# fxslava/tiny_mp2v_dec

Measured on AMD Instinct MI355X. Metric: decoded frames/sec + GB/s vs HBM roofline, 1080p 4:2:0 @1/2/4/8 GPU; bit-exact YUV, higher is better.
Workload: dtype u8

## Files before the change

include/mp2vg.h:

```cpp
#ifndef MP2VG_H
#define MP2VG_H

#include <stddef.h>
#include <stdint.h>

#ifdef __cplusplus
extern "C" {
#endif

#define MP2VG_ABI_VERSION 2

enum {
    MP2VG_OK = 0,
    MP2VG_E_INVALID = -1,
    MP2VG_E_UNSUPPORTED = -2,
    MP2VG_E_HIP = -3,
    MP2VG_E_NOMEM = -4,
    MP2VG_E_STATE = -5,
    MP2VG_E_BITSTREAM = -6
};

enum {
    MP2VG_MB_INTRA = 1u << 0,
    MP2VG_MB_FWD = 1u << 1,
    MP2VG_MB_BWD = 1u << 2,
    MP2VG_MB_FIELD_MC = 1u << 3,
    MP2VG_MB_DCT_FIELD = 1u << 4
};
#define MP2VG_MB_FS_BIT(r, s) (1u << (8 + 2 * (r) + (s)))

typedef struct mp2vg_mb {
    uint16_t x, y;
    uint16_t flags;
    uint16_t cbp;
    uint8_t  qscale;
    uint8_t  reserved;
    uint16_t ncoef;
    uint32_t coef_off;
    int16_t  mv[2][2][2];
} mp2vg_mb_t;

#define MP2VG_COEF_LEVEL(w) ((int16_t)((w) & 0xffffu))
#define MP2VG_COEF_POS(w) (((w) >> 16) & 63u)
#define MP2VG_COEF_BLOCK(w) (((w) >> 22) & 15u)
#define MP2VG_COEF_FIRST1S (1u << 29)
#define MP2VG_COEF_DC (1u << 30)
#define MP2VG_COEF_MBX(x) (((uint32_t)(x) & 7u) << 26)
#define MP2VG_COEF_PACK(level, pos, block, fl) \
    ((uint32_t)(uint16_t)(int16_t)(level) | ((uint32_t)(pos) << 16) | ((uint32_t)(block) << 22) | (uint32_t)(fl))

typedef struct mp2vg_picture {
    int32_t  dst_slot;
    int32_t  fwd_slot;
    int32_t  bwd_slot;
    int32_t  picture_coding_type;
    uint32_t mb_first;
    uint16_t mb_width, mb_height;
    uint8_t  alternate_scan;
    uint8_t  reserved0[3];
    int32_t  temporal_reference;
    uint8_t  W[4][64];
} mp2vg_picture_t;

typedef struct mp2vg_config {
    int32_t width, height;
    int32_t chroma_format;
    int32_t pictures_pool_size;
    int32_t num_threads;
    int32_t reordering;
    int32_t device;
    int32_t reserved;
} mp2vg_config_t;

#define MP2VG_DECODER_DEVICE_FRAMES 1
#define MP2VG_CTX_ONE_STREAM 2
#define MP2VG_DECODER_DEVICE_PARSE 4

typedef struct mp2vg_ctx mp2vg_ctx_t;

int  mp2vg_abi_version(void);
const char* mp2vg_status_string(int status);
const char* mp2vg_last_error(void);

int  mp2vg_create(const mp2vg_config_t* cfg, mp2vg_ctx_t** out);
int  mp2vg_destroy(mp2vg_ctx_t* ctx);
int  mp2vg_frame_geometry(const mp2vg_config_t* cfg, int32_t width[3], int32_t height[3],
                          int32_t stride[3], uint64_t* slot_bytes);
int  mp2vg_reserve_slots(mp2vg_ctx_t* ctx, int32_t nslots);

int  mp2vg_batch_upload(mp2vg_ctx_t* ctx, const mp2vg_picture_t* pics, int32_t npics,
                        const mp2vg_mb_t* mbs, uint64_t nmbs, const uint32_t* coefs,
                        uint64_t ncoefs);
int  mp2vg_batch_validate(const mp2vg_config_t* cfg, int32_t nslots, const mp2vg_picture_t* pics,
                          int32_t npics, const mp2vg_mb_t* mbs, uint64_t nmbs,
                          const uint32_t* coefs, uint64_t ncoefs, int32_t* nlaunches,
                          int32_t* launch_of_pic, int32_t* launch_mode, int32_t max_launches);
typedef struct mp2vg_plan {
    uint32_t* slices;
    int32_t*  launches;
    int32_t*  writes;
    int32_t*  ext_reads;
    int32_t*  post;
    int32_t*  foot;
    int32_t   max_slices, max_launches, max_writes, max_ext_reads, max_post, max_foot;
    int32_t   nslices, nlaunches, nwrites, next_reads, npost, nfoot;
    int32_t   nsets;
    int32_t   reserved;
} mp2vg_plan_t;
int  mp2vg_batch_plan(const mp2vg_config_t* cfg, int32_t nslots, const mp2vg_picture_t* pics,
                      int32_t npics, const mp2vg_mb_t* mbs, uint64_t nmbs,
                      const uint32_t* coefs, uint64_t ncoefs, mp2vg_plan_t* plan);
int  mp2vg_batch_decode(mp2vg_ctx_t* ctx);
int  mp2vg_synchronize(mp2vg_ctx_t* ctx);
int  mp2vg_last_launch_times(mp2vg_ctx_t* ctx, float* ms, int32_t max, int32_t* count);
int  mp2vg_last_batch_time(mp2vg_ctx_t* ctx, float* ms);
int  mp2vg_batch_times(mp2vg_ctx_t* ctx, int32_t back, float* batch_ms, float* launch_ms, int32_t max,
                       int32_t* count);
int  mp2vg_batches_span(mp2vg_ctx_t* ctx, int32_t back_first, int32_t back_last, float* ms);
int  mp2vg_download_slot(mp2vg_ctx_t* ctx, int32_t slot, uint8_t* dst_planes[3],
                         const int32_t dst_stride[3]);
int  mp2vg_copy_slot_packed(mp2vg_ctx_t* ctx, int32_t slot, void* dst, int32_t dst_on_device);
int  mp2vg_slot_device_ptr(mp2vg_ctx_t* ctx, int32_t slot, void** dptr);
int  mp2vg_invalidate_slot(mp2vg_ctx_t* ctx, int32_t slot);
int  mp2vg_pool_placement(mp2vg_ctx_t* ctx, float* ms, int32_t max, int32_t* n, int32_t* kept);
int  mp2vg_sink_device_ptr(mp2vg_ctx_t* ctx, void** dptr);
int  mp2vg_clock_probe(int32_t device, double* ghz);
int  mp2vg_cpu_budget(void);
int  mp2vg_pool_probe(mp2vg_ctx_t* ctx, int32_t rw, int32_t reps, double* gbps, int32_t max, int32_t* nblocks);
int  mp2vg_slot_digests(mp2vg_ctx_t* ctx, const int32_t* slots, int32_t n, uint64_t* out);

enum { MP2VG_EXPORT_RGB_PLANAR = 0 , MP2VG_EXPORT_RGB_PACKED = 1  };
enum { MP2VG_EXPORT_CHROMA_NEAREST = 0, MP2VG_EXPORT_CHROMA_LINEAR = 1 };
typedef struct mp2vg_export {
    int32_t layout, matrix, chroma;
    int32_t width, height;
    int32_t reserved[3];
} mp2vg_export_t;

int  mp2vg_export_coefficients(int32_t matrix, int32_t out[5]);
int  mp2vg_export_bytes(const mp2vg_config_t* cfg, const mp2vg_export_t* exp, int32_t n, uint64_t* bytes);
int  mp2vg_export_slots(mp2vg_ctx_t* ctx, const int32_t* slots, int32_t n, const mp2vg_export_t* exp,
                        void* dst_device, uint64_t dst_bytes);
int  mp2vg_export_planes(int32_t device, const uint8_t* const planes[3], const int32_t stride[3],
                         int32_t chroma_format, int32_t coded_w, int32_t coded_h, const mp2vg_export_t* exp,
                         void* dst_device, uint64_t dst_bytes);

enum { MP2VG_TENSOR_U8 = 0, MP2VG_TENSOR_F16 = 1, MP2VG_TENSOR_BF16 = 2, MP2VG_TENSOR_F32 = 3 };
enum { MP2VG_FIELD_PROGRESSIVE = 0, MP2VG_FIELD_TOP = 1, MP2VG_FIELD_BOTTOM = 2, MP2VG_FIELD_WEAVE = 3 };
#define MP2VG_TENSOR_MAX_TAPS 65
typedef struct mp2vg_tensor {
    int32_t layout, matrix, chroma;
    int32_t src_x, src_y, src_w, src_h;
    int32_t out_w, out_h;
    int32_t dtype;
    float   scale[3], bias[3];
    int32_t reserved[4];
} mp2vg_tensor_t;

int  mp2vg_tensor_weights(int32_t src, int32_t out, int32_t* first, int32_t* count, int32_t* weights,
                          int32_t max_taps);
int  mp2vg_tensor_bytes(const mp2vg_config_t* cfg, const mp2vg_tensor_t* t, int32_t n, uint64_t* bytes);
int  mp2vg_tensor_slots(mp2vg_ctx_t* ctx, const int32_t* slots, int32_t n, const mp2vg_tensor_t* t,
                        void* dst_device, uint64_t dst_bytes);
int  mp2vg_tensor_planes(int32_t device, const uint8_t* const planes[3], const int32_t stride[3],
                         int32_t chroma_format, int32_t coded_w, int32_t coded_h, const mp2vg_tensor_t* t,
                         void* dst_device, uint64_t dst_bytes);
int  mp2vg_tensor_slots_fields(mp2vg_ctx_t* ctx, const int32_t* slots, const int32_t* fields, int32_t n,
                               const mp2vg_tensor_t* t, void* dst_device, uint64_t dst_bytes);
int  mp2vg_tensor_planes_field(int32_t device, const uint8_t* const planes[3], const int32_t stride[3],
                               int32_t chroma_format, int32_t coded_w, int32_t coded_h, int32_t field,
                               const mp2vg_tensor_t* t, void* dst_device, uint64_t dst_bytes);

typedef struct mp2vg_sequence_header {
    uint32_t sequence_header_code, horizontal_size_value, vertical_size_value, aspect_ratio_information,
             frame_rate_code, bit_rate_value, vbv_buffer_size_value, constrained_parameters_flag,
             load_intra_quantiser_matrix;
    uint8_t  intra_quantiser_matrix[64];
    uint32_t load_non_intra_quantiser_matrix;
    uint8_t  non_intra_quantiser_matrix[64];
} mp2vg_sequence_header_t;
typedef struct mp2vg_sequence_extension {
    uint32_t extension_start_code, extension_start_code_identifier, profile_and_level_indication,
             progressive_sequence, chroma_format, horizontal_size_extension, vertical_size_extension,
             bit_rate_extension, vbv_buffer_size_extension, low_delay, frame_rate_extension_n,
             frame_rate_extension_d;
} mp2vg_sequence_extension_t;
typedef struct mp2vg_sequence_display_extension {
    uint32_t extension_start_code_identifier, video_format, colour_description, colour_primaries,
             transfer_characteristics, matrix_coefficients, display_horizontal_size, display_vertical_size;
} mp2vg_sequence_display_extension_t;
typedef struct mp2vg_sequence_scalable_extension {
    uint32_t extension_start_code_identifier, scalable_mode, layer_id, lower_layer_prediction_horizontal_size,
             lower_layer_prediction_vertical_size, horizontal_subsampling_factor_m,
             horizontal_subsampling_factor_n, vertical_subsampling_factor_m, vertical_subsampling_factor_n,
             picture_mux_enable, mux_to_progressive_sequence, picture_mux_order, picture_mux_factor;
} mp2vg_sequence_scalable_extension_t;
typedef struct mp2vg_group_of_pictures_header {
    uint32_t group_start_code, time_code, closed_gop, broken_link;
} mp2vg_group_of_pictures_header_t;
typedef struct mp2vg_stream_headers {
    int32_t have_sequence_display_extension;
    int32_t have_group_of_pictures_header;
    mp2vg_sequence_header_t sequence_header;
    mp2vg_sequence_extension_t sequence_extension;
    mp2vg_sequence_display_extension_t sequence_display_extension;
    mp2vg_group_of_pictures_header_t group_of_pictures_header;
} mp2vg_stream_headers_t;

int  mp2vg_export_matrix(const mp2vg_stream_headers_t* headers, int32_t* matrix);

typedef struct mp2vg_parsed mp2vg_parsed_t;

int  mp2vg_parse_es(const uint8_t* buf, uint64_t len, const mp2vg_config_t* cfg,
                    mp2vg_parsed_t** out);
int  mp2vg_parsed_counts(const mp2vg_parsed_t* p, int32_t* npics, uint64_t* nmbs,
                         uint64_t* ncoefs);
const mp2vg_picture_t* mp2vg_parsed_pictures(const mp2vg_parsed_t* p);
const mp2vg_mb_t*      mp2vg_parsed_mbs(const mp2vg_parsed_t* p);
const uint32_t*        mp2vg_parsed_coefs(const mp2vg_parsed_t* p);
int  mp2vg_parsed_display_order(const mp2vg_parsed_t* p, int32_t* order, int32_t n);
int  mp2vg_parsed_gop_index(const mp2vg_parsed_t* p, int32_t* gop, int32_t n);
enum { MP2VG_PIC_PROGRESSIVE_FRAME = 1, MP2VG_PIC_TOP_FIELD_FIRST = 2, MP2VG_PIC_REPEAT_FIRST_FIELD = 4 };
int  mp2vg_parsed_picture_flags(const mp2vg_parsed_t* p, uint32_t* flags, int32_t n);
int  mp2vg_parsed_stream_headers(const mp2vg_parsed_t* p, mp2vg_stream_headers_t* out);
int  mp2vg_parsed_shards(const mp2vg_parsed_t* p, int32_t* shard, int32_t n);
void mp2vg_parsed_free(mp2vg_parsed_t* p);

typedef struct mp2vg_scan mp2vg_scan_t;
int  mp2vg_scan_es(const uint8_t* buf, uint64_t len, const mp2vg_config_t* cfg, mp2vg_scan_t** out);
int  mp2vg_scan_counts(const mp2vg_scan_t* s, int32_t* npics, uint64_t* nslices);
const mp2vg_picture_t* mp2vg_scan_pictures(const mp2vg_scan_t* s);
int  mp2vg_scan_display_order(const mp2vg_scan_t* s, int32_t* order, int32_t n);
int  mp2vg_scan_gop_index(const mp2vg_scan_t* s, int32_t* gop, int32_t n);
int  mp2vg_scan_picture_flags(const mp2vg_scan_t* s, uint32_t* flags, int32_t n);
int  mp2vg_scan_shards(const mp2vg_scan_t* s, int32_t* shard, int32_t n);
int  mp2vg_scan_stream_headers(const mp2vg_scan_t* s, mp2vg_stream_headers_t* out);
void mp2vg_scan_free(mp2vg_scan_t* s);
int  mp2vg_scan_parse_host(const mp2vg_scan_t* s, int32_t first, int32_t npics, mp2vg_mb_t* mbs, uint64_t nmbs,
                           uint32_t* coefs, uint64_t ncoefs, uint64_t* nmbs_out, uint64_t* ncoefs_out);
int  mp2vg_batch_upload_es(mp2vg_ctx_t* ctx, const mp2vg_scan_t* scan, const mp2vg_picture_t* pics,
                           int32_t first, int32_t npics);
int  mp2vg_batch_record_counts(mp2vg_ctx_t* ctx, uint64_t* nmbs, uint64_t* ncoefs);
int  mp2vg_batch_download_records(mp2vg_ctx_t* ctx, mp2vg_mb_t* mbs, uint64_t nmbs, uint32_t* coefs,
                                  uint64_t ncoefs);
int  mp2vg_last_parse_times(mp2vg_ctx_t* ctx, float ms[3]);

enum {
    MP2VG_VLC_MBA = 0, MP2VG_VLC_MBTYPE_I = 1, MP2VG_VLC_MBTYPE_P = 2, MP2VG_VLC_MBTYPE_B = 3,
    MP2VG_VLC_CBP = 4, MP2VG_VLC_MOTION = 5, MP2VG_VLC_DC_LUMA = 6, MP2VG_VLC_DC_CHROMA = 7,
    MP2VG_VLC_COEF_B14 = 8, MP2VG_VLC_COEF_B15 = 9
};
int  mp2vg_vlc_decode(int32_t table, uint64_t bits, int32_t* value, int32_t* aux, int32_t* consumed);

typedef struct mp2vg_gen_params {
    int32_t width, height, chroma_format;
    int32_t n_gops;
    int32_t gop_n, gop_m;
    uint32_t seed;
    int32_t frame_pred_frame_dct;
    int32_t alternate_scan;
    int32_t q_scale_type;
    int32_t intra_dc_precision;
    int32_t coefs_min, coefs_max;
    int32_t intra_coefs_min, intra_coefs_max;
    int32_t big_level_permille;
    int32_t escape_permille;
    int32_t quant_permille;
    int32_t f_code;
    int32_t mix;
    int32_t leading_b;
    int32_t big_matrix_permille;
    int32_t top_field_first;
    int32_t reserved[4];
} mp2vg_gen_params_t;

void mp2vg_gen_default_params(mp2vg_gen_params_t* p);
int  mp2vg_generate_es(const mp2vg_gen_params_t* p, uint8_t** out, uint64_t* len);
void mp2vg_free(void* ptr);

typedef struct mp2vg_frame {
    uint8_t* planes[3];
    int32_t  width[3], height[3], stride[3];
    int32_t  picture_coding_type;
    int32_t  decode_index;
    int32_t  device;
} mp2vg_frame_t;
typedef void (*mp2vg_render_fn)(void* user, const mp2vg_frame_t* frame);
typedef struct mp2vg_decoder mp2vg_decoder_t;

int  mp2vg_decoder_create(const mp2vg_config_t* cfg, mp2vg_render_fn fn, void* user,
                          mp2vg_decoder_t** out);
int  mp2vg_decoder_create_multi(const mp2vg_config_t* cfg, const int32_t* devices, int32_t ndevices,
                                mp2vg_render_fn fn, void* user, mp2vg_decoder_t** out);
int  mp2vg_decoder_decode(mp2vg_decoder_t* dec, const uint8_t* buf, uint64_t len);
int  mp2vg_decoder_stream_headers(const mp2vg_decoder_t* dec, mp2vg_stream_headers_t* out);
int  mp2vg_decoder_lane_frames(const mp2vg_decoder_t* dec, int32_t* frames, int32_t n);
int  mp2vg_decoder_frames_allocated(const mp2vg_decoder_t* dec);
int  mp2vg_decoder_handoff_stats(const mp2vg_decoder_t* dec, int32_t* in_flight, int32_t* blocks, int32_t* landed,
                                 int32_t* changes);
int  mp2vg_decoder_destroy(mp2vg_decoder_t* dec);

#ifdef __cplusplus
}
#endif
#endif
```

tiny_mp2v_dec_amd/_lib.py:

```python
import ctypes
import os

import numpy as np

PKG = os.path.dirname(os.path.abspath(__file__))
LIB_PATH = os.environ.get("MP2VG_LIB") or os.path.join(PKG, "_build", "libmp2vg.so")

MB_DTYPE = np.dtype([("x", "<u2"), ("y", "<u2"), ("flags", "<u2"), ("cbp", "<u2"), ("qscale", "u1"),
                     ("reserved", "u1"), ("ncoef", "<u2"), ("coef_off", "<u4"), ("mv", "<i2", (2, 2, 2))])
assert MB_DTYPE.itemsize == 32
PIC_DTYPE = np.dtype([("dst_slot", "<i4"), ("fwd_slot", "<i4"), ("bwd_slot", "<i4"),
                      ("picture_coding_type", "<i4"), ("mb_first", "<u4"), ("mb_width", "<u2"),
                      ("mb_height", "<u2"), ("alternate_scan", "u1"), ("reserved0", "u1", (3,)),
                      ("temporal_reference", "<i4"), ("W", "u1", (4, 64))])
assert PIC_DTYPE.itemsize == 288

MB_INTRA, MB_FWD, MB_BWD, MB_FIELD_MC, MB_DCT_FIELD = 1, 2, 4, 8, 16
COEF_FIRST1S, COEF_DC = 1 << 29, 1 << 30


def mb_fs_bit(r, s):
    return 1 << (8 + 2 * r + s)


def coef_pack(level, pos, block, flags=0, mbx=0):
    return (np.uint32(np.int64(level) & 0xFFFF) | np.uint32(pos << 16) | np.uint32(block << 22) |
            np.uint32(flags) | np.uint32((int(mbx) & 7) << 26))


STATUS = {0: "ok", -1: "invalid argument", -2: "unsupported stream", -3: "HIP error", -4: "out of memory",
          -5: "call out of order", -6: "bitstream error"}


class Mp2vgError(RuntimeError):
    def __init__(self, status, what, detail=""):
        self.status = status
        super().__init__(f"{what}: {STATUS.get(status, status)} ({detail})")


class Config(ctypes.Structure):
    _fields_ = [("width", ctypes.c_int32), ("height", ctypes.c_int32), ("chroma_format", ctypes.c_int32),
                ("pictures_pool_size", ctypes.c_int32), ("num_threads", ctypes.c_int32),
                ("reordering", ctypes.c_int32), ("device", ctypes.c_int32), ("reserved", ctypes.c_int32)]


class GenParams(ctypes.Structure):
    _fields_ = [(n, ctypes.c_int32) for n in (
        "width", "height", "chroma_format", "n_gops", "gop_n", "gop_m")] + [("seed", ctypes.c_uint32)] + [
        (n, ctypes.c_int32) for n in (
            "frame_pred_frame_dct", "alternate_scan", "q_scale_type", "intra_dc_precision", "coefs_min",
            "coefs_max", "intra_coefs_min", "intra_coefs_max", "big_level_permille", "escape_permille",
            "quant_permille", "f_code", "mix", "leading_b", "big_matrix_permille", "top_field_first")] + [
        ("reserved", ctypes.c_int32 * 4)]


class Frame(ctypes.Structure):
    _fields_ = [("planes", ctypes.POINTER(ctypes.c_uint8) * 3), ("width", ctypes.c_int32 * 3),
                ("height", ctypes.c_int32 * 3), ("stride", ctypes.c_int32 * 3),
                ("picture_coding_type", ctypes.c_int32), ("decode_index", ctypes.c_int32),
                ("device", ctypes.c_int32)]


class SequenceHeader(ctypes.Structure):
    _fields_ = [(n, ctypes.c_uint32) for n in (
        "sequence_header_code", "horizontal_size_value", "vertical_size_value", "aspect_ratio_information",
        "frame_rate_code", "bit_rate_value", "vbv_buffer_size_value", "constrained_parameters_flag",
        "load_intra_quantiser_matrix")] + [("intra_quantiser_matrix", ctypes.c_uint8 * 64),
                                           ("load_non_intra_quantiser_matrix", ctypes.c_uint32),
                                           ("non_intra_quantiser_matrix", ctypes.c_uint8 * 64)]


class SequenceExtension(ctypes.Structure):
    _fields_ = [(n, ctypes.c_uint32) for n in (
        "extension_start_code", "extension_start_code_identifier", "profile_and_level_indication",
        "progressive_sequence", "chroma_format", "horizontal_size_extension", "vertical_size_extension",
        "bit_rate_extension", "vbv_buffer_size_extension", "low_delay", "frame_rate_extension_n",
        "frame_rate_extension_d")]


class SequenceDisplayExtension(ctypes.Structure):
    _fields_ = [(n, ctypes.c_uint32) for n in (
        "extension_start_code_identifier", "video_format", "colour_description", "colour_primaries",
        "transfer_characteristics", "matrix_coefficients", "display_horizontal_size", "display_vertical_size")]


class GopHeader(ctypes.Structure):
    _fields_ = [(n, ctypes.c_uint32) for n in ("group_start_code", "time_code", "closed_gop", "broken_link")]


class StreamHeaders(ctypes.Structure):
    _fields_ = [("have_sequence_display_extension", ctypes.c_int32),
                ("have_group_of_pictures_header", ctypes.c_int32),
                ("sequence_header", SequenceHeader), ("sequence_extension", SequenceExtension),
                ("sequence_display_extension", SequenceDisplayExtension),
                ("group_of_pictures_header", GopHeader)]


class Export(ctypes.Structure):
    _fields_ = [("layout", ctypes.c_int32), ("matrix", ctypes.c_int32), ("chroma", ctypes.c_int32),
                ("width", ctypes.c_int32), ("height", ctypes.c_int32), ("reserved", ctypes.c_int32 * 3)]


class Plan(ctypes.Structure):
    _fields_ = [("slices", ctypes.POINTER(ctypes.c_uint32))] + [
        (n, ctypes.POINTER(ctypes.c_int32)) for n in ("launches", "writes", "ext_reads", "post", "foot")] + [
        (n, ctypes.c_int32) for n in (
            "max_slices", "max_launches", "max_writes", "max_ext_reads", "max_post", "max_foot",
            "nslices", "nlaunches", "nwrites", "next_reads", "npost", "nfoot", "nsets", "reserved")]


EXPORT_RGB_PLANAR, EXPORT_RGB_PACKED = 0, 1
EXPORT_CHROMA_NEAREST, EXPORT_CHROMA_LINEAR = 0, 1

class Tensor(ctypes.Structure):
    _fields_ = [("layout", ctypes.c_int32), ("matrix", ctypes.c_int32), ("chroma", ctypes.c_int32),
                ("src_x", ctypes.c_int32), ("src_y", ctypes.c_int32), ("src_w", ctypes.c_int32),
                ("src_h", ctypes.c_int32), ("out_w", ctypes.c_int32), ("out_h", ctypes.c_int32),
                ("dtype", ctypes.c_int32), ("scale", ctypes.c_float * 3), ("bias", ctypes.c_float * 3),
                ("reserved", ctypes.c_int32 * 4)]


TENSOR_U8, TENSOR_F16, TENSOR_BF16, TENSOR_F32 = 0, 1, 2, 3
TENSOR_MAX_TAPS = 65
FIELD_PROGRESSIVE, FIELD_TOP, FIELD_BOTTOM, FIELD_WEAVE = 0, 1, 2, 3
FIELDS = {"progressive": FIELD_PROGRESSIVE, "top": FIELD_TOP, "bottom": FIELD_BOTTOM, "weave": FIELD_WEAVE}
PIC_PROGRESSIVE_FRAME, PIC_TOP_FIELD_FIRST, PIC_REPEAT_FIRST_FIELD = 1, 2, 4
TENSOR_DTYPES = {"uint8": (TENSOR_U8, 1), "float16": (TENSOR_F16, 2), "bfloat16": (TENSOR_BF16, 2),
                 "float32": (TENSOR_F32, 4)}

RENDER_FN = ctypes.CFUNCTYPE(None, ctypes.c_void_p, ctypes.POINTER(Frame))

EXPORTS = [
    "mp2vg_abi_version", "mp2vg_status_string", "mp2vg_last_error", "mp2vg_create", "mp2vg_destroy",
    "mp2vg_frame_geometry", "mp2vg_reserve_slots", "mp2vg_batch_upload", "mp2vg_batch_validate", "mp2vg_batch_plan", "mp2vg_batch_decode",
    "mp2vg_synchronize", "mp2vg_last_launch_times", "mp2vg_last_batch_time", "mp2vg_batch_times", "mp2vg_batches_span", "mp2vg_download_slot", "mp2vg_copy_slot_packed", "mp2vg_slot_device_ptr", "mp2vg_sink_device_ptr", "mp2vg_clock_probe", "mp2vg_pool_probe", "mp2vg_pool_placement", "mp2vg_cpu_budget", "mp2vg_invalidate_slot",
    "mp2vg_slot_digests", "mp2vg_parse_es", "mp2vg_parsed_counts", "mp2vg_parsed_pictures", "mp2vg_parsed_mbs",
    "mp2vg_parsed_coefs", "mp2vg_parsed_display_order", "mp2vg_parsed_gop_index", "mp2vg_parsed_stream_headers",
    "mp2vg_parsed_shards", "mp2vg_parsed_free", "mp2vg_vlc_decode",
    "mp2vg_gen_default_params", "mp2vg_generate_es", "mp2vg_free", "mp2vg_decoder_create",
    "mp2vg_decoder_create_multi", "mp2vg_decoder_decode", "mp2vg_decoder_stream_headers",
    "mp2vg_decoder_lane_frames", "mp2vg_decoder_frames_allocated", "mp2vg_decoder_handoff_stats",
    "mp2vg_decoder_destroy",
    "mp2vg_export_coefficients", "mp2vg_export_matrix", "mp2vg_export_bytes", "mp2vg_export_slots",
    "mp2vg_export_planes",
    "mp2vg_tensor_weights", "mp2vg_tensor_bytes", "mp2vg_tensor_slots", "mp2vg_tensor_planes",
    "mp2vg_tensor_slots_fields", "mp2vg_tensor_planes_field", "mp2vg_parsed_picture_flags", "mp2vg_scan_picture_flags",
    "mp2vg_scan_es", "mp2vg_scan_counts", "mp2vg_scan_pictures", "mp2vg_scan_display_order",
    "mp2vg_scan_gop_index", "mp2vg_scan_shards", "mp2vg_scan_stream_headers", "mp2vg_scan_free",
    "mp2vg_scan_parse_host", "mp2vg_batch_upload_es", "mp2vg_batch_record_counts",
    "mp2vg_batch_download_records", "mp2vg_last_parse_times",
]

_lib = None


def lib():
    global _lib
    if _lib is not None:
        return _lib
    if not os.path.exists(LIB_PATH):
        raise RuntimeError(f"native library {LIB_PATH} is missing: run `python tiny_mp2v_dec_amd/build.py` "
                           "(there is no CPU fallback for the reconstruct path)")
    L = ctypes.CDLL(LIB_PATH)
    P, I32, U64, VP = ctypes.POINTER, ctypes.c_int32, ctypes.c_uint64, ctypes.c_void_p
    sig = {
        "mp2vg_abi_version": ([], ctypes.c_int),
        "mp2vg_status_string": ([ctypes.c_int], ctypes.c_char_p),
        "mp2vg_last_error": ([], ctypes.c_char_p),
        "mp2vg_create": ([P(Config), P(VP)], ctypes.c_int),
        "mp2vg_destroy": ([VP], ctypes.c_int),
        "mp2vg_frame_geometry": ([P(Config), P(I32), P(I32), P(I32), P(U64)], ctypes.c_int),
        "mp2vg_reserve_slots": ([VP, I32], ctypes.c_int),
        "mp2vg_batch_upload": ([VP, VP, I32, VP, U64, VP, U64], ctypes.c_int),
        "mp2vg_batch_validate": ([P(Config), I32, VP, I32, VP, U64, VP, U64, P(I32), P(I32), P(I32), I32],
                                 ctypes.c_int),
        "mp2vg_batch_plan": ([P(Config), I32, VP, I32, VP, U64, VP, U64, P(Plan)], ctypes.c_int),
        "mp2vg_batch_decode": ([VP], ctypes.c_int),
        "mp2vg_synchronize": ([VP], ctypes.c_int),
        "mp2vg_last_launch_times": ([VP, P(ctypes.c_float), I32, P(I32)], ctypes.c_int),
        "mp2vg_last_batch_time": ([VP, P(ctypes.c_float)], ctypes.c_int),
        "mp2vg_batch_times": ([VP, I32, P(ctypes.c_float), P(ctypes.c_float), I32, P(I32)], ctypes.c_int),
        "mp2vg_batches_span": ([VP, I32, I32, P(ctypes.c_float)], ctypes.c_int),
        "mp2vg_download_slot": ([VP, I32, P(ctypes.c_void_p), P(I32)], ctypes.c_int),
        "mp2vg_copy_slot_packed": ([VP, I32, VP, I32], ctypes.c_int),
        "mp2vg_slot_device_ptr": ([VP, I32, P(VP)], ctypes.c_int),
        "mp2vg_sink_device_ptr": ([VP, P(VP)], ctypes.c_int),
        "mp2vg_clock_probe": ([I32, P(ctypes.c_double)], ctypes.c_int),
        "mp2vg_pool_probe": ([VP, I32, I32, P(ctypes.c_double), I32, P(I32)], ctypes.c_int),
        "mp2vg_pool_placement": ([VP, P(ctypes.c_float), I32, P(I32), P(I32)], ctypes.c_int),
        "mp2vg_cpu_budget": ([], ctypes.c_int),
        "mp2vg_invalidate_slot": ([VP, I32], ctypes.c_int),
        "mp2vg_slot_digests": ([VP, P(I32), I32, P(ctypes.c_uint64)], ctypes.c_int),
        "mp2vg_parse_es": ([VP, U64, P(Config), P(VP)], ctypes.c_int),
        "mp2vg_parsed_counts": ([VP, P(I32), P(U64), P(U64)], ctypes.c_int),
        "mp2vg_parsed_pictures": ([VP], VP),
        "mp2vg_parsed_mbs": ([VP], VP),
        "mp2vg_parsed_coefs": ([VP], VP),
        "mp2vg_parsed_display_order": ([VP, P(I32), I32], ctypes.c_int),
        "mp2vg_parsed_gop_index": ([VP, P(I32), I32], ctypes.c_int),
        "mp2vg_parsed_stream_headers": ([VP, P(StreamHeaders)], ctypes.c_int),
        "mp2vg_parsed_shards": ([VP, P(I32), I32], ctypes.c_int),
        "mp2vg_parsed_free": ([VP], None),
        "mp2vg_vlc_decode": ([I32, U64, P(I32), P(I32), P(I32)], ctypes.c_int),
        "mp2vg_gen_default_params": ([P(GenParams)], None),
        "mp2vg_generate_es": ([P(GenParams), P(VP), P(U64)], ctypes.c_int),
        "mp2vg_free": ([VP], None),
        "mp2vg_decoder_create": ([P(Config), RENDER_FN, VP, P(VP)], ctypes.c_int),
        "mp2vg_decoder_create_multi": ([P(Config), P(I32), I32, RENDER_FN, VP, P(VP)], ctypes.c_int),
        "mp2vg_decoder_decode": ([VP, VP, U64], ctypes.c_int),
        "mp2vg_decoder_stream_headers": ([VP, P(StreamHeaders)], ctypes.c_int),
        "mp2vg_decoder_lane_frames": ([VP, P(I32), I32], ctypes.c_int),
        "mp2vg_decoder_frames_allocated": ([VP], ctypes.c_int),
        "mp2vg_decoder_handoff_stats": ([VP, P(I32), P(I32), P(I32), P(I32)], ctypes.c_int),
        "mp2vg_decoder_destroy": ([VP], ctypes.c_int),
        "mp2vg_export_coefficients": ([I32, P(I32)], ctypes.c_int),
        "mp2vg_export_matrix": ([P(StreamHeaders), P(I32)], ctypes.c_int),
        "mp2vg_export_bytes": ([P(Config), P(Export), I32, P(U64)], ctypes.c_int),
        "mp2vg_export_slots": ([VP, P(I32), I32, P(Export), VP, U64], ctypes.c_int),
        "mp2vg_export_planes": ([I32, P(VP), P(I32), I32, I32, I32, P(Export), VP, U64], ctypes.c_int),
        "mp2vg_tensor_weights": ([I32, I32, P(I32), P(I32), P(I32), I32], ctypes.c_int),
        "mp2vg_tensor_bytes": ([P(Config), P(Tensor), I32, P(U64)], ctypes.c_int),
        "mp2vg_tensor_slots": ([VP, P(I32), I32, P(Tensor), VP, U64], ctypes.c_int),
        "mp2vg_tensor_planes": ([I32, P(VP), P(I32), I32, I32, I32, P(Tensor), VP, U64], ctypes.c_int),
        "mp2vg_tensor_slots_fields": ([VP, P(I32), P(I32), I32, P(Tensor), VP, U64], ctypes.c_int),
        "mp2vg_tensor_planes_field": ([I32, P(VP), P(I32), I32, I32, I32, I32, P(Tensor), VP, U64], ctypes.c_int),
        "mp2vg_parsed_picture_flags": ([VP, P(ctypes.c_uint32), I32], ctypes.c_int),
        "mp2vg_scan_picture_flags": ([VP, P(ctypes.c_uint32), I32], ctypes.c_int),
        "mp2vg_scan_es": ([VP, U64, P(Config), P(VP)], ctypes.c_int),
        "mp2vg_scan_counts": ([VP, P(I32), P(U64)], ctypes.c_int),
        "mp2vg_scan_pictures": ([VP], VP),
        "mp2vg_scan_display_order": ([VP, P(I32), I32], ctypes.c_int),
        "mp2vg_scan_gop_index": ([VP, P(I32), I32], ctypes.c_int),
        "mp2vg_scan_shards": ([VP, P(I32), I32], ctypes.c_int),
        "mp2vg_scan_stream_headers": ([VP, P(StreamHeaders)], ctypes.c_int),
        "mp2vg_scan_free": ([VP], None),
        "mp2vg_scan_parse_host": ([VP, I32, I32, VP, U64, VP, U64, P(U64), P(U64)], ctypes.c_int),
        "mp2vg_batch_upload_es": ([VP, VP, VP, I32, I32], ctypes.c_int),
        "mp2vg_batch_record_counts": ([VP, P(U64), P(U64)], ctypes.c_int),
        "mp2vg_batch_download_records": ([VP, VP, U64, VP, U64], ctypes.c_int),
        "mp2vg_last_parse_times": ([VP, P(ctypes.c_float)], ctypes.c_int),
    }
    for name, (args, res) in sig.items():
        fn = getattr(L, name)
        fn.argtypes = args
        fn.restype = res
    _lib = L
    return L


def check(status, what):
    if status != 0:
        detail = lib().mp2vg_last_error().decode(errors="replace")
        raise Mp2vgError(status, what, detail)
    return status


MP2VG_DECODER_DEVICE_FRAMES, MP2VG_CTX_ONE_STREAM = 1, 2
MP2VG_DECODER_DEVICE_PARSE = 4


def make_config(width, height, chroma_format, pool=10, threads=0, reordering=True, device=0, flags=0):
    return Config(width, height, chroma_format, pool, threads, 1 if reordering else 0, device, flags)


def make_export(layout="nchw", chroma="linear", matrix=1, size=None):
    layouts = {"nchw": EXPORT_RGB_PLANAR, "nhwc": EXPORT_RGB_PACKED}
    modes = {"nearest": EXPORT_CHROMA_NEAREST, "linear": EXPORT_CHROMA_LINEAR}
    if layout not in layouts:
        raise ValueError(f"layout {layout!r}: expected 'nchw' or 'nhwc'")
    if chroma not in modes:
        raise ValueError(f"chroma {chroma!r}: expected 'linear' or 'nearest'")
    w, h = (0, 0) if size is None else (int(size[0]), int(size[1]))
    return Export(layouts[layout], int(matrix), modes[chroma], w, h, (ctypes.c_int32 * 3)())


def export_shape(exp, n, coded_w, coded_h):
    w, h = exp.width or coded_w, exp.height or coded_h
    return (n, 3, h, w) if exp.layout == EXPORT_RGB_PLANAR else (n, h, w, 3)


def export_out(out, shape, device):
    import torch
    dev = torch.device("cuda", device)
    if out is None:
        return torch.empty(shape, dtype=torch.uint8, device=dev)
    if not isinstance(out, torch.Tensor) or out.device != dev or out.dtype != torch.uint8:
        raise ValueError(f"out must be a torch.uint8 tensor on {dev}")
    if tuple(out.shape) != tuple(shape) or not out.is_contiguous():
        raise ValueError(f"out must be contiguous with shape {tuple(shape)}, got {tuple(out.shape)}")
    return out


def tensor_dtype_name(dtype):
    name = str(dtype).replace("torch.", "")
    if name not in TENSOR_DTYPES:
        raise ValueError(f"dtype {dtype!r}: expected uint8, float16, bfloat16 or float32")
    return name


def make_tensor(size, crop=None, dtype="float16", mean=None, std=None, layout="nchw", chroma="linear", matrix=1):
    e = make_export(layout, chroma, matrix)
    name = tensor_dtype_name(dtype)
    if (mean is None) != (std is None):
        raise ValueError("mean and std go together")
    if name == "uint8":
        if mean is not None:
            raise ValueError("uint8 output takes no mean / std")
        scale, bias = [1.0] * 3, [0.0] * 3
    elif mean is None:
        scale, bias = [1.0 / 255.0] * 3, [0.0] * 3
    else:
        mean, std = [float(v) for v in mean], [float(v) for v in std]
        if len(mean) != 3 or len(std) != 3:
            raise ValueError("mean and std have one entry per channel")
        scale, bias = [1.0 / (255.0 * s) for s in std], [-m / s for m, s in zip(mean, std)]
    x, y, w, h = (0, 0, 0, 0) if crop is None else (int(v) for v in crop)
    return Tensor(e.layout, e.matrix, e.chroma, x, y, w, h, int(size[0]), int(size[1]), TENSOR_DTYPES[name][0],
                  (ctypes.c_float * 3)(*scale), (ctypes.c_float * 3)(*bias), (ctypes.c_int32 * 4)())


def field_mode(field):
    if isinstance(field, str):
        if field not in FIELDS:
            raise ValueError(f"field {field!r}: expected 'progressive', 'top', 'bottom' or 'weave'")
        return FIELDS[field]
    if int(field) not in FIELDS.values():
        raise ValueError(f"field {field!r}: expected 0..3 (MP2VG_FIELD_*)")
    return int(field)


def field_modes(fields, n):
    if fields is None:
        return None
    if isinstance(fields, (str, int, np.integer)):
        return np.full(n, field_mode(fields), np.int32)
    out = np.array([field_mode(f) for f in fields], np.int32)
    if len(out) != n:
        raise ValueError("fields must hold one mode per slot")
    return out


def tensor_shape(t, n):
    return (n, 3, t.out_h, t.out_w) if t.layout == EXPORT_RGB_PLANAR else (n, t.out_h, t.out_w, 3)


def tensor_out(out, shape, dtype, device):
    import torch
    dev, want = torch.device("cuda", device), getattr(torch, tensor_dtype_name(dtype))
    if out is None:
        return torch.empty(shape, dtype=want, device=dev)
    if not isinstance(out, torch.Tensor) or out.device != dev or out.dtype != want:
        raise ValueError(f"out must be a {want} tensor on {dev}")
    if tuple(out.shape) != tuple(shape) or not out.is_contiguous():
        raise ValueError(f"out must be contiguous with shape {tuple(shape)}, got {tuple(out.shape)}")
    return out


def tensor_weights(src, out):
    first, count = np.zeros(out, np.int32), np.zeros(out, np.int32)
    w = np.zeros((out, TENSOR_MAX_TAPS), np.int32)
    i32p = ctypes.POINTER(ctypes.c_int32)
    check(lib().mp2vg_tensor_weights(src, out, first.ctypes.data_as(i32p), count.ctypes.data_as(i32p),
                                     w.ctypes.data_as(i32p), TENSOR_MAX_TAPS), "tensor_weights")
    return first, count, w[:, :int(count.max())]


def geometry(width, height, chroma_format):
    c = make_config(width, height, chroma_format)
    w, h, s = (ctypes.c_int32 * 3)(), (ctypes.c_int32 * 3)(), (ctypes.c_int32 * 3)()
    sb = ctypes.c_uint64()
    check(lib().mp2vg_frame_geometry(ctypes.byref(c), w, h, s, ctypes.byref(sb)), "frame_geometry")
    return list(w), list(h), list(s), sb.value
```

tiny_mp2v_dec_amd/csrc/recon.hip:

```cpp
#include <hip/hip_runtime.h>

#include <cstdlib>
#include <stdint.h>
#include <stdlib.h>

#include "recon_kernel.h"

namespace mp2vg {

typedef short short2_t __attribute__((ext_vector_type(2)));

__device__ __forceinline__ short2_t adds2(short2_t a, short2_t b) { return __builtin_elementwise_add_sat(a, b); }
__device__ __forceinline__ short2_t subs2(short2_t a, short2_t b) { return __builtin_elementwise_sub_sat(a, b); }
__device__ __forceinline__ short2_t shl2(short2_t a, int n) {
    return __builtin_bit_cast(short2_t, __builtin_bit_cast(ushort2, a) << (unsigned short)n);
}
__device__ __forceinline__ short2_t mulhi2(short2_t a, int c) {
    const uint32_t u = __builtin_bit_cast(uint32_t, a);
    const int lo = (int)(short)(u & 0xffffu) * c, hi = ((int)u >> 16) * c;
    return __builtin_bit_cast(short2_t, __builtin_amdgcn_perm((uint32_t)hi, (uint32_t)lo, 0x07060302u));
}
__device__ __forceinline__ short2_t mulhi2_x2(short2_t a, int c) {
    const short2_t h = mulhi2(a, 2 * c);
    return __builtin_bit_cast(short2_t, __builtin_bit_cast(uint32_t, h) & 0xfffefffeu);
}

template <bool P1 = false>
__device__ __forceinline__ void idct_1d(short2_t s[8]) {
    const short2_t v15 = adds2(mulhi2_x2(s[0], 27145), shl2(s[0], 1));
    const short2_t v26 = P1 ? mulhi2(s[1], -5037 + 262144) : adds2(mulhi2(s[1], -5037), shl2(s[1], 2));
    const short2_t v21 = P1 ? mulhi2(s[2], -19954 + 262144) : adds2(mulhi2(s[2], -19954), shl2(s[2], 2));
    const short2_t v28 = P1 ? mulhi2_x2(s[3], -22089 + 131072) : adds2(mulhi2_x2(s[3], -22089), shl2(s[3], 2));
    const short2_t v16 = P1 ? mulhi2_x2(s[4], 27145 + 65536) : adds2(mulhi2_x2(s[4], 27145), shl2(s[4], 1));
    const short2_t v25 = P1 ? mulhi2(s[5], 14567 + 131072) : adds2(mulhi2(s[5], 14567), shl2(s[5], 1));
    const short2_t v22 = adds2(mulhi2_x2(s[6], 17391), s[6]);
    const short2_t v27 = mulhi2_x2(s[7], 25570);
    const short2_t v19 = subs2(v25, v28);
    const short2_t v20 = subs2(v26, v27);
    const short2_t v23 = adds2(v26, v27);
    const short2_t v24 = adds2(v25, v28);
    const short2_t v7 = adds2(v23, v24);
    const short2_t v11 = adds2(v21, v22);
    const short2_t v13 = subs2(v23, v24);
    const short2_t v17 = subs2(v21, v22);
    const short2_t v8 = adds2(v15, v16);
    const short2_t v9 = subs2(v15, v16);
    const short2_t v18 = mulhi2(subs2(v19, v20), 25079);
    const short2_t v12 = subs2(v18, P1 ? mulhi2(v19, 20090 + 65536) : adds2(v19, mulhi2(v19, 20090)));
    const short2_t v14 = subs2(subs2(v20, mulhi2(v20, 30068)), v18);
    const short2_t v6 = subs2(shl2(v14, 1), v7);
    const short2_t v5 = subs2(P1 ? mulhi2(v13, 27145 + 65536) : adds2(v13, mulhi2(v13, 27145)), v6);
    const short2_t v4 = adds2(v5, shl2(v12, 1));
    const short2_t v10 = subs2(P1 ? mulhi2(v17, 27145 + 65536) : adds2(v17, mulhi2(v17, 27145)), v11);
    const short2_t v0 = adds2(v8, v11);
    const short2_t v1 = adds2(v9, v10);
    const short2_t v2 = subs2(v9, v10);
    const short2_t v3 = subs2(v8, v11);
    s[0] = adds2(v0, v7);
    s[1] = adds2(v1, v6);
    s[2] = adds2(v2, v5);
    s[3] = subs2(v3, v4);
    s[4] = adds2(v3, v4);
    s[5] = subs2(v2, v5);
    s[6] = subs2(v1, v6);
    s[7] = subs2(v0, v7);
}

__device__ __forceinline__ void interleave(const uint4& a, const uint4& b, short2_t s[8]) {
    const uint32_t av[4] = {a.x, a.y, a.z, a.w}, bv[4] = {b.x, b.y, b.z, b.w};
#pragma unroll
    for (int i = 0; i < 4; i++) {
        s[2 * i] = __builtin_bit_cast(short2_t, __builtin_amdgcn_perm(bv[i], av[i], 0x05040100u));
        s[2 * i + 1] = __builtin_bit_cast(short2_t, __builtin_amdgcn_perm(bv[i], av[i], 0x07060302u));
    }
}

__constant__ uint8_t c_scan_raster[2][64] = {
    {0,  1,  8,  16, 9,  2,  3,  10, 17, 24, 32, 25, 18, 11, 4,  5,  12, 19, 26, 33, 40, 48,
     41, 34, 27, 20, 13, 6,  7,  14, 21, 28, 35, 42, 49, 56, 57, 50, 43, 36, 29, 22, 15, 23,
     30, 37, 44, 51, 58, 59, 52, 45, 38, 31, 39, 46, 53, 60, 61, 54, 47, 55, 62, 63},
    {0,  8,  16, 24, 1,  9,  2,  10, 17, 25, 32, 40, 48, 56, 57, 49, 41, 33, 26, 18, 3,  11,
     4,  12, 19, 27, 34, 42, 50, 58, 35, 43, 51, 59, 20, 28, 5,  13, 6,  14, 21, 29, 36, 44,
     52, 60, 37, 45, 53, 61, 22, 30, 7,  15, 23, 31, 38, 46, 54, 62, 39, 47, 55, 63}};

__device__ __forceinline__ void wave_sync() {
    __builtin_amdgcn_fence(__ATOMIC_RELEASE, "wavefront");
    __builtin_amdgcn_wave_barrier();
    __builtin_amdgcn_fence(__ATOMIC_ACQUIRE, "wavefront");
}

__device__ __forceinline__ uint32_t sat_pk_u8(short2_t v) {
    uint32_t r;
    asm("v_sat_pk_u8_i16 %0, %1" : "=v"(r) : "v"(__builtin_bit_cast(uint32_t, v)));
    return r;
}

__device__ __forceinline__ uint32_t avg4(uint32_t a, uint32_t b) { return __builtin_amdgcn_lerp(a, b, 0x01010101u); }

__device__ __forceinline__ uint32_t mul24_asm(uint32_t a, uint32_t b) {
    uint32_t r;
    asm("v_mul_u32_u24 %0, %1, %2" : "=v"(r) : "v"(a), "v"(b));
    return r;
}

template <int CF>
struct Fmt {
    static constexpr int NB = CF == 1 ? 6 : (CF == 2 ? 8 : 12);
    static constexpr int CW = CF == 3 ? 16 : 8;
    static constexpr int CH = CF == 1 ? 8 : 16;
};

template <int CF>
__device__ __forceinline__ void block_origin(int b, bool dctf, int& plane, int& x0, int& y0, int& ys) {
    ys = 1;
    if (b < 4) {
        plane = 0;
        x0 = (b & 1) * 8;
        if (dctf) {
            y0 = b >> 1;
            ys = 2;
        } else {
            y0 = (b >> 1) * 8;
        }
        return;
    }
    plane = (b & 1) ? 2 : 1;
    const int k = (b - 4) >> 1;
    x0 = k >= 2 ? 8 : 0;
    const bool lower = (k & 1);
    if (dctf && CF != 1) {
        y0 = lower ? 1 : 0;
        ys = 2;
    } else {
        y0 = lower ? 8 : 0;
    }
}

template <int CF>
__device__ __forceinline__ int left_block(int plane, int py, bool dctf) {
    const int lower = dctf ? (py & 1) : (py >> 3);
    if (plane == 0) return lower * 2;
    const int base = plane == 1 ? 4 : 5;
    if (CF == 1) return base;
    return base + 2 * lower;
}


constexpr int WAVES = 4;
constexpr int G = 4;
#ifndef MP2VG_I_WAVES
#define MP2VG_I_WAVES 4
#endif
#ifndef MP2VG_I_KBTAB
#define MP2VG_I_KBTAB 1
#endif
template <int MCM, int ABL>
constexpr int kernel_waves() { return (MCM == 0 || MCM == 4) && ABL == 0 ? MP2VG_I_WAVES : WAVES; }

template <int CF>
struct ResLayout {
    using F = Fmt<CF>;
    static constexpr int SIZE = 256 + 2 * F::CW * F::CH;
#ifndef MP2VG_RES_PAD
#define MP2VG_RES_PAD 0
#endif
    static constexpr int MBS = SIZE + MP2VG_RES_PAD;
    __device__ static constexpr int base(int plane) { return plane == 0 ? 0 : 256 + (plane - 1) * F::CW * F::CH; }
    __device__ static constexpr int width(int plane) { return plane == 0 ? 16 : F::CW; }
    __device__ static int pos(int x) { return (x & ~3) | ((x & 1) << 1) | ((x >> 1) & 1); }
};

template <class T>
__device__ __forceinline__ T gsel(const T (&v)[3], int plane) {
    return plane == 0 ? v[0] : (plane == 1 ? v[1] : v[2]);
}

#ifndef MP2VG_REC_NT
#define MP2VG_REC_NT 0
#endif
__device__ __forceinline__ uint32_t ld_rec(const uint32_t* p) {
    if (MP2VG_REC_NT) return __builtin_nontemporal_load(p);
    return *p;
}
__device__ __forceinline__ uint32_t rec_load(const uint32_t* __restrict__ mbrec, uint32_t g, uint32_t mb_last, int lane) {
    const uint32_t mb = min(g + (uint32_t)(lane & 3), mb_last);
    return ld_rec(&mbrec[(size_t)mb * 8 + ((lane >> 2) & 7)]);
}
__device__ __forceinline__ uint32_t rec_get(uint32_t rv, int f, int k) {
    return (uint32_t)__builtin_amdgcn_ds_bpermute((f * 4 + k) * 4, (int)rv);
}
template <int F, int K>
__device__ __forceinline__ uint32_t rec_uni(uint32_t rv) {
    return (uint32_t)__builtin_amdgcn_readlane((int)rv, F * 4 + K);
}

struct Group {
    uint32_t fl8;
    uint32_t qs8;
    uint32_t sb8;
    uint32_t cbp01, cbp23;
    int nslots, ncoef;
    uint32_t coef0;
};

__device__ __forceinline__ uint32_t pick8(uint32_t v, int k) { return __builtin_amdgcn_ubfe(v, (uint32_t)k * 8, 8); }
__device__ __forceinline__ uint32_t pick16(uint32_t lo, uint32_t hi, int k) {
    return __builtin_amdgcn_ubfe((k & 2) ? hi : lo, (uint32_t)(k & 1) * 16, 16);
}

template <int NB, int K>
__device__ __forceinline__ void group_mb(Group& S, uint32_t rv, int ng, int& sb, int& cr) {
    const uint32_t r1 = rec_uni<1, K>(rv), r2 = rec_uni<2, K>(rv);
    const bool live = K < ng;
    const uint32_t cbpk = live ? ((r1 >> 16) & ((1u << NB) - 1)) : 0u;
    S.fl8 |= (live ? (r1 & 0xff) : (uint32_t)MP2VG_MB_INTRA) << (8 * K);
    S.qs8 |= (r2 & 0xff) << (8 * K);
    S.sb8 |= (uint32_t)sb << (8 * K);
    if (K == 0) S.cbp01 = cbpk;
    if (K == 1) S.cbp01 |= cbpk << 16;
    if (K == 2) S.cbp23 = cbpk;
    if (K == 3) S.cbp23 |= cbpk << 16;
    sb += __builtin_popcount(cbpk);
    cr += live ? (int)(r2 >> 16) : 0;
}

template <int NB>
__device__ __forceinline__ Group group_state(uint32_t rv, int ng) {
    Group S;
    S.fl8 = S.qs8 = S.sb8 = 0;
    int sb = 0, cr = 0;
    group_mb<NB, 0>(S, rv, ng, sb, cr);
    group_mb<NB, 1>(S, rv, ng, sb, cr);
    group_mb<NB, 2>(S, rv, ng, sb, cr);
    group_mb<NB, 3>(S, rv, ng, sb, cr);
    S.nslots = sb;
    S.ncoef = cr;
    S.coef0 = rec_uni<3, 0>(rv);
    return S;
}

template <int CF>
struct Passes {
    static constexpr int N = CF == 1 ? 2 : 3;
};
template <int CF, int J>
__device__ __forceinline__ void pass_row(int lane, int& k, int& plane, int& py) {
    k = lane & 3;
    py = lane >> 2;
    if (J == 0) {
        plane = 0;
    } else if (CF == 1) {
        plane = 1 + (lane >> 5);
        py = (lane & 31) >> 2;
    } else {
        plane = J;
    }
}

template <int W>
__device__ __forceinline__ uint32_t tile_off(uint32_t x, uint32_t y, uint32_t ncol) {
    if (W == 16) return (mul24_asm(y >> 2, ncol) + (x >> 4)) * 128u + (y & 3u) * 32u + (x & 12u);
    return (mul24_asm(y >> 3, ncol) + (x >> 3)) * 128u + (y & 7u) * 16u + (x & 4u);
}
template <int W>
__device__ __forceinline__ uint32_t tile_row(uint32_t mx, uint32_t y, uint32_t ncol) {
    if (W == 16) return (mul24_asm(y >> 2, ncol) + mx) * 128u + (y & 3u) * 32u;
    return (mul24_asm(y >> 3, ncol) + mx) * 128u + (y & 7u) * 16u;
}

template <int NW>
struct Tap {
    static constexpr int ND = NW + 1;
    uint32_t a[ND], b[ND];
    uint32_t ctl;
};

typedef uint32_t u3v __attribute__((ext_vector_type(3)));
typedef uint32_t u4v __attribute__((ext_vector_type(4)));
constexpr uint32_t kNoTap = 0xFFFFFF00u;
__device__ __forceinline__ __amdgpu_buffer_rsrc_t slot_rsrc(const uint8_t* base, uint32_t bytes) {
    return __builtin_amdgcn_make_buffer_rsrc((void*)base, (short)0, (int)bytes, 0x00020000);
}
template <int NW, int ABL = 0>
__device__ __forceinline__ void load_row(uint32_t (&d)[NW + 1], __amdgpu_buffer_rsrc_t r, uint32_t off) {
    if (NW == 4) {
        const u4v v = __builtin_amdgcn_raw_buffer_load_b128(r, (int)off, 0, 0);
        d[0] = v.x; d[1] = v.y; d[2] = v.z; d[3] = v.w;
        d[4] = __builtin_amdgcn_raw_buffer_load_b32(r, (ABL & 128) ? (int)kNoTap : (int)(off + 16), 0, 0);
    } else if (NW == 2) {
        const u3v v = __builtin_amdgcn_raw_buffer_load_b96(r, (int)off, 0, 0);
        d[0] = v.x; d[1] = v.y; d[2] = v.z;
    } else {
#pragma unroll
        for (int i = 0; i < NW + 1; i++) d[i] = __builtin_amdgcn_raw_buffer_load_b32(r, (int)(off + 4 * i), 0, 0);
    }
}

#ifndef MP2VG_CHROMA_TILES
#define MP2VG_CHROMA_TILES 1
#endif
constexpr bool kChromaTiles = MP2VG_CHROMA_TILES;

__device__ __forceinline__ uint32_t mad24s_asm(uint32_t a, uint32_t b_uniform, uint32_t c) {
    uint32_t r;
    asm("v_mad_u32_u24 %0, %1, %2, %3" : "=v"(r) : "v"(a), "s"(b_uniform), "v"(c));
    return r;
}

// ... 77 lines not shown
    for (int d = 0; d < NW; d++) {
        const uint32_t r0 = avg4(A[d], __builtin_amdgcn_alignbyte(A[d + 1], A[d], hx));
        const uint32_t r1 = avg4(C[d], __builtin_amdgcn_alignbyte(C[d + 1], C[d], hx));
        p[d] = avg4(r0, r1);
    }
}

template <int MCM, int NW, int ABL = 0>
__device__ __forceinline__ void predict(Tap<NW>& tf, Tap<NW>& tb, int lane, uint32_t (&p)[NW]) {
    if (ABL & 64) {
#pragma unroll
        for (int d = 0; d < NW; d++) p[d] = tf.a[d] ^ tf.b[d] ^ (MCM == 2 ? tb.a[d] ^ tb.b[d] : 0u);
        return;
    }
    if (!(MP2VG_ROW2_LOAD && MCM == 2)) {
        tap_rows<NW>(tf, lane);
        if (MCM == 2) tap_rows<NW>(tb, lane);
    }
    const bool uf = tf.ctl & 16, ub = MCM == 2 && (tb.ctl & 16);
    uint32_t pf[NW], pb[NW];
#pragma unroll
    for (int d = 0; d < NW; d++) pf[d] = pb[d] = 0;
    if (uf) tap_finish<NW>(tf, pf);
    if (MCM == 2 && ub) tap_finish<NW>(tb, pb);
#pragma unroll
    for (int d = 0; d < NW; d++) p[d] = (uf && ub) ? avg4(pf[d], pb[d]) : (uf ? pf[d] : pb[d]);
}

struct LaneRec {
    uint32_t r0, r1, mvf, mvb;
};
__device__ __forceinline__ LaneRec lane_rec(uint32_t rv, int lane) {
    LaneRec L;
    const int k = lane & 3;
    L.r0 = rec_get(rv, 0, k);
    L.r1 = rec_get(rv, 1, k);
    const int r = (L.r1 & MP2VG_MB_FIELD_MC) ? ((lane >> 2) & 1) : 0;
    L.mvf = rec_get(rv, 4 + 2 * r, k);
    L.mvb = rec_get(rv, 5 + 2 * r, k);
    return L;
}

template <int CF, int MCM, int J, int NW, int ABL = 0>
__device__ __forceinline__ void issue_pass(const LaneRec& L, bool live, int lane, const Geo& geo,
                                           __amdgpu_buffer_rsrc_t ref_fwd, __amdgpu_buffer_rsrc_t ref_bwd,
                                           Tap<NW>& tf, Tap<NW>& tb, int dir = 0) {
    using F = Fmt<CF>;
    int k, plane, py;
    pass_row<CF, J>(lane, k, plane, py);
    const uint32_t fl = L.r1 & 0xffff;
    const bool none = !live || (fl & MP2VG_MB_INTRA);
    const bool bwd = fl & MP2VG_MB_BWD;
    const bool fwd = !none && (MCM == 1 || (fl & MP2VG_MB_FWD) || !bwd);
    const bool field = fl & MP2VG_MB_FIELD_MC;
    const int pw = plane == 0 ? 16 : F::CW;
    const int phm = plane == 0 ? 16 : F::CH;
    const int gx = (int)(L.r0 & 0xffff) * pw;
    const int mbyb = (int)(L.r0 >> 16) * phm;
    const int r = field ? (py & 1) : 0;
    const int stride = J == 0 ? geo.stride[0] : geo.stride[1];
    const int ph = J == 0 ? geo.ph[0] : geo.ph[1];
    constexpr bool TL = J == 0 || kChromaTiles;
    const uint32_t off = (TL ? 2u : 1u) * (uint32_t)gsel(geo.plane_off, plane);
    const uint32_t mv1 = (MCM == 1 && dir) ? L.mvb : L.mvf;
    const int fsh = 8 + 2 * r + (MCM == 1 ? dir : 0);
    constexpr bool R2 = MP2VG_ROW2_LOAD && MCM == 2;
    tap_issue<CF, NW, ABL, TL, R2>(tf, fwd, ref_fwd, off, mv1, plane, gx, py, phm, mbyb, field, (fl >> fsh) & 1, stride, ph);
    if (MCM == 2)
        tap_issue<CF, NW, ABL, TL, R2>(tb, !none && bwd, ref_bwd, off, L.mvb, plane, gx, py, phm, mbyb, field,
                                       (fl >> (9 + 2 * r)) & 1, stride, ph);
}

__device__ __forceinline__ void row_store16(uint8_t* d, uint32_t a, uint32_t b, uint32_t c, uint32_t e) {
    *(uint4*)d = make_uint4(a, b, c, e);
}
__device__ __forceinline__ void row_store8(uint8_t* d, uint32_t a, uint32_t b) { *(uint2*)d = make_uint2(a, b); }

#ifndef MP2VG_ROW_POL
#define MP2VG_ROW_POL 16
#endif
#ifndef MP2VG_TILE_POL
#define MP2VG_TILE_POL 2
#endif
template <int POL>
__device__ __forceinline__ void pol_store16(__amdgpu_buffer_rsrc_t r, uint32_t off, uint4 v) {
    __builtin_amdgcn_raw_buffer_store_b128(u4v{v.x, v.y, v.z, v.w}, r, (int)off, 0, POL);
}
template <int POL>
__device__ __forceinline__ void pol_store8(__amdgpu_buffer_rsrc_t r, uint32_t off, uint2 v) {
    typedef uint32_t u2v __attribute__((ext_vector_type(2)));
    __builtin_amdgcn_raw_buffer_store_b64(u2v{v.x, v.y}, r, (int)off, 0, POL);
}


template <int CF, int J, int NW, int ABL>
__device__ __forceinline__ void store_pass(uint32_t r0, uint32_t r1, bool live, int lane, const Geo& geo, uint8_t* wsink,
                                           uint8_t* dst_slot, __amdgpu_buffer_rsrc_t dst_rsrc, bool tiles,
                                           const short* s_res_wave, const uint32_t (&p)[NW]) {
    using F = Fmt<CF>;
    using RL = ResLayout<CF>;
    int k, plane, py;
    pass_row<CF, J>(lane, k, plane, py);
    const uint32_t fl = r1 & 0xffff, cbpk = r1 >> 16;
    const int lb = left_block<CF>(plane, py, fl & MP2VG_MB_DCT_FIELD);
    const int rb = (plane == 0) ? lb + 1 : lb + 4;
    const bool cl = cbpk & (1u << lb);
    const bool cr = NW == 4 && (cbpk & (1u << rb));
    uint32_t out[4] = {0, 0, 0, 0};
#pragma unroll
    for (int d = 0; d < NW; d++) out[d] = p[d];
    if (cl || cr) {
        const short* res = s_res_wave + k * RL::MBS + RL::base(plane) + py * RL::width(plane);
        uint32_t rv[8];
        const uint4 q0 = *(const uint4*)&res[0];
        rv[0] = q0.x; rv[1] = q0.y; rv[2] = q0.z; rv[3] = q0.w;
        if (NW == 4) {
            const uint4 q1 = *(const uint4*)&res[8];
            rv[4] = q1.x; rv[5] = q1.y; rv[6] = q1.z; rv[7] = q1.w;
        }
#pragma unroll
        for (int d = 0; d < NW; d++) {
            if (!(d < 2 ? cl : cr)) continue;
            const uint32_t lo = __builtin_amdgcn_perm(0u, out[d], 0x0c020c00u);
            const uint32_t hi = __builtin_amdgcn_perm(0u, out[d], 0x0c030c01u);
            const short2_t a = __builtin_bit_cast(short2_t, lo) + __builtin_bit_cast(short2_t, rv[2 * d]);
            const short2_t c = __builtin_bit_cast(short2_t, hi) + __builtin_bit_cast(short2_t, rv[2 * d + 1]);
            out[d] = __builtin_amdgcn_perm(sat_pk_u8(c), sat_pk_u8(a), 0x05010400u);
        }
    }
    const int pw = plane == 0 ? 16 : F::CW;
    const int phm = plane == 0 ? 16 : F::CH;
    const uint32_t doff = gsel(geo.plane_off, plane) + mul24_asm((r0 >> 16) * phm + py, (uint32_t)gsel(geo.stride, plane)) +
                          (r0 & 0xffff) * (uint32_t)pw;
    uint8_t* dst = dst_slot + doff;
    dst = live ? dst : wsink;
    if (ABL & 8192)
        dst = dst_slot + ((((r0 & 0xffff) + (r0 >> 16) * 128u) * 3u + (uint32_t)J) * 1024u + (uint32_t)lane * 16u) %
                             (uint32_t)(geo.plane_off[1] - 1024);
    if (tiles) {
        uint8_t* img = (uint8_t*)(s_res_wave + k * RL::MBS + RL::base(plane) + py * RL::width(plane));
        if (NW == 4)
            *(uint4*)img = make_uint4(out[0], out[1], out[2], out[3]);
        else
            *(uint2*)img = make_uint2(out[0], out[1]);
    }
    if (ABL & 8) {
        asm volatile("" ::"v"(out[0]), "v"(out[1]), "v"(out[2]), "v"(out[3]), "v"(dst));
    } else if (ABL & 4096) {
        asm volatile("" ::"v"(out[0]), "v"(out[1]), "v"(out[2]), "v"(out[3]));
        *(uint32_t*)dst = out[0] ^ out[1] ^ (NW == 4 ? out[2] ^ out[3] : 0u);
    } else if (MP2VG_ROW_POL != 0) {
        if (NW == 4)
            pol_store16<MP2VG_ROW_POL>(dst_rsrc, live ? doff : kNoTap, make_uint4(out[0], out[1], out[2], out[3]));
        else
            pol_store8<MP2VG_ROW_POL>(dst_rsrc, live ? doff : kNoTap, make_uint2(out[0], out[1]));
    } else if (NW == 4) {
        row_store16(dst, out[0], out[1], out[2], out[3]);
    } else {
        row_store8(dst, out[0], out[1]);
    }
}

template <int CF, int J, int NW>
__device__ __forceinline__ void store_pass_put8(uint32_t r0, bool live, int lane, const Geo& geo, uint8_t* wsink,
                                                uint8_t* dst_slot, __amdgpu_buffer_rsrc_t dst_rsrc,
                                                const uint8_t* res8_wave) {
    using F = Fmt<CF>;
    using RL = ResLayout<CF>;
    int k, plane, py;
    pass_row<CF, J>(lane, k, plane, py);
    const uint8_t* row = &res8_wave[k * RL::SIZE + RL::base(plane) + py * RL::width(plane)];
    const int pw = plane == 0 ? 16 : F::CW;
    const int phm = plane == 0 ? 16 : F::CH;
    const uint32_t doff = gsel(geo.plane_off, plane) + mul24_asm((r0 >> 16) * phm + py, (uint32_t)gsel(geo.stride, plane)) +
                          (r0 & 0xffff) * (uint32_t)pw;
    uint8_t* dst = live ? dst_slot + doff : wsink;
    if (NW == 4) {
        const uint4 q = *(const uint4*)row;
        const uint4 o = make_uint4(__builtin_amdgcn_perm(q.x, q.x, 0x03010200u), __builtin_amdgcn_perm(q.y, q.y, 0x03010200u),
                                   __builtin_amdgcn_perm(q.z, q.z, 0x03010200u), __builtin_amdgcn_perm(q.w, q.w, 0x03010200u));
        if (MP2VG_ROW_POL != 0)
            pol_store16<MP2VG_ROW_POL>(dst_rsrc, live ? doff : kNoTap, o);
        else
            row_store16(dst, o.x, o.y, o.z, o.w);
    } else {
        const uint2 q = *(const uint2*)row;
        const uint2 o = make_uint2(__builtin_amdgcn_perm(q.x, q.x, 0x03010200u), __builtin_amdgcn_perm(q.y, q.y, 0x03010200u));
        if (MP2VG_ROW_POL != 0)
            pol_store8<MP2VG_ROW_POL>(dst_rsrc, live ? doff : kNoTap, o);
        else
            row_store8(dst, o.x, o.y);
    }
}

template <int CF, bool NAT>
__device__ __forceinline__ const uint8_t* img_row(const uint8_t* img, int k, int plane, int py) {
    using RL = ResLayout<CF>;
    return &img[(NAT ? 2 : 1) * (k * (NAT ? RL::MBS : RL::SIZE) + RL::base(plane) + py * RL::width(plane))];
}
__device__ __forceinline__ uint32_t unswz(uint32_t v, bool nat) { return nat ? v : __builtin_amdgcn_perm(v, v, 0x03010200u); }
template <int CF, bool NAT>
__device__ __forceinline__ uint4 img_row16(const uint8_t* img, int k, int plane, int py) {
    const uint4 q = *(const uint4*)img_row<CF, NAT>(img, k, plane, py);
    return make_uint4(unswz(q.x, NAT), unswz(q.y, NAT), unswz(q.z, NAT), unswz(q.w, NAT));
}
template <int CF, bool NAT>
__device__ __forceinline__ uint2 img_row8(const uint8_t* img, int k, int plane, int py) {
    const uint2 q = *(const uint2*)img_row<CF, NAT>(img, k, plane, py);
    return make_uint2(unswz(q.x, NAT), unswz(q.y, NAT));
}
template <int CF, bool NAT, int ABL = 0>
__device__ __forceinline__ void tile_group(uint32_t mx0, uint32_t mby, int lane, const Geo& geo, uint8_t* wsink,
                                           uint8_t* dst_tiles, __amdgpu_buffer_rsrc_t tile_rsrc, const uint8_t* res8) {
    using F = Fmt<CF>;
    constexpr bool POL = MP2VG_TILE_POL != 0;
    for (int plane = 0; plane < (CF == 3 && kChromaTiles ? 3 : 1); plane++) {
        uint8_t* tp = dst_tiles + 2u * gsel(geo.plane_off, plane);
        const uint32_t ncol = (uint32_t)gsel(geo.stride, plane) >> 4;
#pragma nounroll
        for (int i = 0; i < 2; i++) {
            const int u = lane + 64 * i;
            int j, r, h;
            if (u < 96) {
                j = u >> 5, r = ((u >> 3) & 3) * 4 + ((u & 7) >> 1), h = u & 1;
            } else {
                const int side = (u - 96) >> 4;
                r = u & 15, h = side, j = side ? -1 : 3;
            }
            const uint4 v = img_row16<CF, NAT>(res8, j + h, plane, r);
            const bool none = j < 0 && mx0 == 0;
            const uint32_t o = tile_row<16>(mx0 + (uint32_t)j, mby * 16u + (uint32_t)r, ncol) + (uint32_t)h * 16u;
            if (POL)
                pol_store16<MP2VG_TILE_POL>(tile_rsrc, none ? kNoTap : 2u * gsel(geo.plane_off, plane) + o, v);
            else
                *(uint4*)(none ? wsink : ((ABL & 65536) ? dst_tiles + (o & 0xFFF0u) : tp + o)) = v;
        }
    }
    if constexpr (CF != 3 && kChromaTiles) {
        constexpr int RPM = F::CH;
        constexpr int N16 = 2 * 3 * RPM, N8 = 2 * 2 * RPM;
        const uint32_t ncol = (uint32_t)geo.stride[1] >> 3;
#pragma nounroll
        for (int i = 0; i < (N16 + 63) / 64; i++) {
            const int u = lane + 64 * i;
            const int plane = 1 + (u >= 3 * RPM ? 1 : 0), rem = u - (plane - 1) * 3 * RPM;
            const int j = rem / RPM, r = rem % RPM;
            const uint2 a = img_row8<CF, NAT>(res8, j, plane, r), b = img_row8<CF, NAT>(res8, min(j + 1, 3), plane, r);
            const uint32_t o = tile_row<8>(mx0 + (uint32_t)j, mby * (uint32_t)RPM + (uint32_t)r, ncol);
            if (POL) {
                pol_store16<MP2VG_TILE_POL>(tile_rsrc, u < N16 ? 2u * gsel(geo.plane_off, plane) + o : kNoTap,
                                            make_uint4(a.x, a.y, b.x, b.y));
            } else {
                uint8_t* d = (ABL & 65536) ? dst_tiles + (o & 0xFFF0u) : dst_tiles + 2u * gsel(geo.plane_off, plane) + o;
                *(uint4*)(u < N16 ? d : wsink) = make_uint4(a.x, a.y, b.x, b.y);
            }
        }
#pragma nounroll
        for (int i = 0; i < (N8 + 63) / 64; i++) {
            const int u = lane + 64 * i;
            const int plane = 1 + (u >= 2 * RPM ? 1 : 0), rem = u - (plane - 1) * 2 * RPM;
            const int side = rem / RPM, r = rem % RPM;
            const int j = side ? -1 : 3, h = side;
            const uint2 v = img_row8<CF, NAT>(res8, side ? 0 : 3, plane, r);
            const uint32_t o = tile_row<8>(mx0 + (uint32_t)j, mby * (uint32_t)RPM + (uint32_t)r, ncol) + (uint32_t)h * 8u;
            const bool none = u >= N8 || (side && mx0 == 0);
            if (POL) {
                pol_store8<MP2VG_TILE_POL>(tile_rsrc, none ? kNoTap : 2u * gsel(geo.plane_off, plane) + o, v);
            } else {
                uint8_t* d = (ABL & 65536) ? dst_tiles + (o & 0xFFF8u) : dst_tiles + 2u * gsel(geo.plane_off, plane) + o;
                *(uint2*)(none ? wsink : d) = v;
            }
        }
    }
}

constexpr int kAblCompact = 16 | 32768 | 65536;
template <int MCM, int ABL>
constexpr bool compact_layout() { return (MCM == 0 || MCM == 4) && (ABL & ~kAblCompact) == 0; }
constexpr int lds_sets(int cf, bool c8) { return c8 ? 1 : (cf == 3 ? 2 : 4); }
template <int CF, int MCM, int ABL>
constexpr uint32_t slices_per_wg(uint32_t mates) {
    return !compact_layout<MCM, ABL>() && kernel_waves<MCM, ABL>() == 4 && (mates == 2 || mates == 4) &&
                   mates <= (uint32_t)lds_sets(CF, false)
               ? mates
               : 1u;
}
constexpr int BLKS = 72;
template <int CF, bool C8 = false, int NWV = WAVES>
struct Lds {
    static constexpr bool COMPACT = C8;
    static constexpr bool X64 = C8;
    static constexpr int NBUF = 1;
    static constexpr int NWAVES = NWV;
    static constexpr int STEP = NWV * G;
    static constexpr int MAXS = G * Fmt<CF>::NB;
    static constexpr int BLK = X64 ? 64 : BLKS;
    short blk[NWV * NBUF][MAXS][BLK];
    short res[NWV][C8 ? G * ResLayout<CF>::SIZE / 2 : G * ResLayout<CF>::MBS];
    uint8_t map[NWV * NBUF][MAXS];
    uint32_t dq[NWV][64];
    static constexpr int NH = lds_sets(CF, C8);
    uint8_t W[4 * NH][64];
    static constexpr bool WB = C8;
    uint8_t scan[64 * NH];
    uint8_t Wb[WB && CF != 1 ? Fmt<CF>::NB : 0][64];
    uint32_t kbtab[WB ? 64 : 0];
    __device__ static int bofs(int slot, int idx) { return slot * BLK + (X64 ? (idx ^ ((slot & 7) << 3)) : idx); }
};

template <int MCM, int NB, class LT>
__device__ __forceinline__ int slot_kb(const LT& L, int wave, int slot, int buf = 0) {
    if constexpr (MCM == 0) {
        static_assert(NB == 6 || NB == 8 || NB == 12, "blocks per MB");
        const int k = NB == 8 ? slot >> 3 : (int)(__umul24((uint32_t)slot, 43u) >> (NB == 6 ? 8 : 9));
        return (k << 4) | (slot - k * NB);
    } else {
        return L.map[wave * LT::NBUF + buf][slot];
    }
}

typedef __attribute__((address_space(3))) short2_t lds_short2_t;
typedef __attribute__((address_space(3))) u4v lds_uint4_t;
__device__ __forceinline__ uint4 ld16(const lds_uint4_t* p) {
    const u4v v = *p;
    return make_uint4(v.x, v.y, v.z, v.w);
}
__device__ __forceinline__ void zero16(lds_uint4_t* p) { *p = u4v{0u, 0u, 0u, 0u}; }
template <class LT>
__device__ __forceinline__ void pass1_store(short* bw, int slot, int v, const short2_t (&s)[8]) {
    if constexpr (LT::X64) {
        const uint32_t b0 = (uint32_t)(uintptr_t)(lds_short2_t*)(bw + LT::bofs(slot, v));
#pragma unroll
        for (int x = 0; x < 8; x++) *(lds_short2_t*)(uintptr_t)(b0 ^ (uint32_t)(x << 4)) = s[x];
    } else {
#pragma unroll
        for (int x = 0; x < 8; x++) *(short2_t*)&bw[LT::bofs(slot, x * 8 + v)] = s[x];
    }
}

typedef __attribute__((address_space(3))) uint16_t lds_u16_t;

template <class LT>
__device__ __forceinline__ void slot_chunks(short* bw, int slot, int ca, int cb, lds_uint4_t*& pa, lds_uint4_t*& pb) {
    if constexpr (LT::X64) {
        const uint32_t b0 = (uint32_t)(uintptr_t)(lds_short2_t*)(bw + LT::bofs(slot, 0));
        pa = (lds_uint4_t*)(uintptr_t)(b0 ^ (uint32_t)(ca << 4));
        pb = (lds_uint4_t*)(uintptr_t)(b0 ^ (uint32_t)(cb << 4));
    } else {
        const uint32_t b0 = (uint32_t)(uintptr_t)(lds_short2_t*)(bw + slot * LT::BLK);
        pa = (lds_uint4_t*)(uintptr_t)(b0 + (uint32_t)(ca << 4));
        pb = (lds_uint4_t*)(uintptr_t)(b0 + (uint32_t)(cb << 4));
    }
}
__device__ __forceinline__ void put8_rows(uint32_t a0, uint32_t step, const short2_t (&s)[8]) {
#pragma unroll
    for (int y = 0; y < 8; y++) *(lds_u16_t*)(uintptr_t)(a0 + (uint32_t)y * step) = (uint16_t)sat_pk_u8(s[y] >> (short)6);
}

struct SliceCtx {
    const uint32_t* mbrec;
    const uint32_t* coefs;
    uint8_t* dst_slot;
    uint8_t* dst_tiles;
    __amdgpu_buffer_rsrc_t dst_rsrc, tile_rsrc;
    bool tiles;
    int dir;
    uint8_t* wsink;
    __amdgpu_buffer_rsrc_t ref_fwd, ref_bwd;
    __amdgpu_buffer_rsrc_t cref_fwd, cref_bwd;
    __amdgpu_buffer_rsrc_t coef_rsrc;
    uint32_t mb_begin, mb_end;
    uint32_t wpos, step;
    int half;
};

template <int CF>
__device__ __forceinline__ uint32_t dq_entry(const Group& S, int lane) {
    constexpr int NB = Fmt<CF>::NB;
    const int k = lane >> 4, bb = lane & 15;
    const uint32_t cbpk = pick16(S.cbp01, S.cbp23, k);
    const bool coded = bb < NB && ((cbpk >> bb) & 1);
    const uint32_t slot = pick8(S.sb8, k) + (uint32_t)__builtin_popcount(cbpk & ((1u << bb) - 1));
    const uint32_t intra = pick8(S.fl8, k) & MP2VG_MB_INTRA;
    const uint32_t wsel = (bb < 6 ? 0u : 2u) + (intra ? 0u : 1u);
    return (slot & 0xff) | (pick8(S.qs8, k) << 8) | (wsel << 16) | (intra << 18) | ((uint32_t)coded << 19);
}

__device__ __forceinline__ int mul24i_asm(int a, int b) {
    int r;
    asm("v_mul_i32_i24 %0, %1, %2" : "=v"(r) : "v"(a), "v"(b));
    return r;
}

template <class LT, bool INTRA_ONLY = false, int NB = 6>
__device__ __forceinline__ void dequant_word(LT& L, int wave, uint32_t w, uint32_t qs8, bool live = true, int h = 0,
                                             int buf = 0) {
    if constexpr (INTRA_ONLY) {
        const uint32_t k = (w >> 26) & 3u, b = (w >> 22) & 15u;
        const int slot = (int)(k * NB + b);
        const int i = (w >> 16) & 63;
        const int level = (short)(w & 0xffff);
        const int Wi = NB == 6 ? L.W[4 * h][i]
                               : (LT::WB ? ((const uint8_t*)L.Wb)[(w >> 16) & 0x3ffu] : L.W[4 * h + (b < 6 ? 0 : 2)][i]);
        uint32_t kb = 0;
        if constexpr (LT::WB && MP2VG_I_KBTAB) kb = L.kbtab[(w >> 22) & 63u];
        const uint32_t qsk = (LT::WB && MP2VG_I_KBTAB) ? __builtin_amdgcn_ubfe(qs8, kb, 8) : pick8(qs8, (int)k);
        const uint32_t wq = __umul24((uint32_t)Wi, qsk);
        const int p = mul24i_asm(level, (int)wq);
        const int val = (p + ((p >> 31) & 15)) >> 4;
        const int v = min(max((int)(short)val, -2048), 2047);
        short o;
        if constexpr (LT::WB) {
            const uint32_t dcm = (uint32_t)__builtin_amdgcn_sbfe((int)w, 30, 1);
            uint32_t ov;
            asm("v_bfi_b32 %0, %1, %2, %3" : "=v"(ov) : "v"(dcm), "v"(w), "v"((uint32_t)v));
            o = (short)ov;
        } else {
            o = (w & MP2VG_COEF_DC) ? (short)level : (short)v;
        }
        if constexpr (LT::WB) {
            const uint32_t a = MP2VG_I_KBTAB
                                   ? (uint32_t)(uintptr_t)(lds_short2_t*)L.blk[wave] + ((kb >> 8) ^ (uint32_t)L.scan[64 * h + i])
                                   : (uint32_t)(uintptr_t)(lds_short2_t*)L.blk[wave] + ((uint32_t)slot << 7) +
                                         ((((uint32_t)slot << 4) & 0x70u) ^ (uint32_t)L.scan[64 * h + i]);
            const uint32_t d = (uint32_t)(uintptr_t)(lds_short2_t*)L.res[wave];
            *(__attribute__((address_space(3))) short*)(uintptr_t)(live ? a : d) = o;
        } else {
            short* const dst = live ? &((short*)L.blk[wave])[LT::bofs(slot, L.scan[64 * h + i])] : (short*)L.res[wave];
            *dst = o;
        }
        return;
    }
    const uint32_t e = L.dq[wave][(w >> 22) & 63u];
    const int slot = (int)(e & 0xff);
    const bool intra = INTRA_ONLY || ((e >> 18) & 1);
    const int qs = (int)((e >> 8) & 0xff);
    const int i = (w >> 16) & 63;
    const int level = (short)(w & 0xffff);
    const bool dc = w & MP2VG_COEF_DC;
    const bool s1 = !INTRA_ONLY && (w & MP2VG_COEF_FIRST1S);
    const int Wi = L.W[4 * h + ((e >> 16) & 3)][i];
    const int sign = level < 0 ? -1 : 0;
    const int mag = level < 0 ? -level : level;
    const uint32_t wq = __umul24((uint32_t)Wi, (uint32_t)qs);
    int val = intra ? (int)mul24_asm((uint32_t)mag, wq) >> 4 : (int)mul24_asm((uint32_t)(2 * mag + 1), wq) >> 5;
    val = (val ^ sign) - sign;
    const int t = (short)val;
    short v = (short)min(max(t, -2048), 2047);
    if (!INTRA_ONLY) {
        const short t1 = (short)((int)(3u * wq) >> 5);
        v = s1 ? (short)((t1 ^ sign) - sign) : v;
    }
    v = dc ? (short)level : v;
    ((short*)L.blk[wave * LT::NBUF + buf])[LT::bofs(slot, L.scan[64 * h + i])] = v;
}

template <int NW>
__device__ __forceinline__ void touch(const Tap<NW>& t) {
#pragma unroll
    for (int i = 0; i <= NW; i++) asm volatile("" ::"v"(t.a[i]), "v"(t.b[i]));
}

struct Stamps {
    uint64_t t, acc[7];
};
template <int ABL>
__device__ __forceinline__ void stamp(Stamps& st, int i) {
    if (!(ABL & 16)) return;
    uint64_t t;
    __builtin_amdgcn_sched_barrier(0);
    asm volatile("s_memtime %0 ; stage stamp %1\n\ts_waitcnt lgkmcnt(0)" : "=s"(t) : "i"(i) : "memory");
    __builtin_amdgcn_sched_barrier(0);
    if (i >= 0) st.acc[i] += t - st.t;
    st.t = t;
}

template <int MCM, int NCW>
__device__ __forceinline__ void prefetch_words(uint32_t (&cw)[NCW], const SliceCtx& c, uint32_t coef0, int ncoef,
                                               int lane) {
    if (MCM != 0) {
#pragma unroll
        for (int j = 0; j < NCW; j++) cw[j] = ld_rec(&c.coefs[coef0 + 64 * j + lane]);
    } else {
        const uint32_t off = (coef0 + (uint32_t)lane) * 4u;
#pragma unroll
        for (int j = 0; j < NCW; j++)
            cw[j] = __builtin_amdgcn_raw_buffer_load_b32(c.coef_rsrc, 64 * j < ncoef ? (int)(off + 256u * j) : (int)kNoTap,
                                                         0, MP2VG_REC_NT ? 2 : 0);
    }
}

template <int CF, int MCM, int ABL, class LT, bool TILES = true>
__device__ __forceinline__ void run_slice(const SliceCtx& c, const Geo& geo, LT& L, int lane, int wave) {
    using F = Fmt<CF>;
    using RL = ResLayout<CF>;
    constexpr int NB = F::NB;
    const uint32_t STEP = c.step;
    constexpr int NWC = F::CW / 4;
    constexpr bool UNI = LT::COMPACT && CF == 1;
    const uint32_t mb_end = c.mb_end, mb_last = c.mb_end - 1;
    uint32_t g = c.mb_begin + c.wpos * G;
    if (g >= mb_end) return;
    const int kl = lane & 3;

    Tap<4> t0f, t0b;
    Tap<NWC> t1f, t1b;
    Tap<NWC> t2f, t2b;
    Group S;
    constexpr int NCW = MCM == 0 ? (CF == 3 ? 24 : (CF == 2 ? 12 : 8)) : 2;
    uint32_t gr0, gr1, rvN, cw[NCW];
    bool glive;
    {
        const uint32_t rv = rec_load(c.mbrec, g, mb_last, lane);
        const int ng = (int)min(mb_end - g, (uint32_t)G);
        glive = kl < ng;
        const LaneRec R = lane_rec(rv, lane);
        if (MCM) issue_pass<CF, MCM, 0, 4, ABL>(R, glive, lane, geo, c.ref_fwd, c.ref_bwd, t0f, t0b, c.dir);
        S = group_state<NB>(rv, ng);
        gr0 = R.r0;
        gr1 = R.r1;
        __builtin_amdgcn_sched_barrier(0);
        rvN = rec_load(c.mbrec, g + STEP < mb_end ? g + STEP : g, mb_last, lane);
        prefetch_words<MCM, NCW>(cw, c, S.coef0, S.ncoef, lane);
        __builtin_amdgcn_sched_barrier(0);
        if (MCM) {
            issue_pass<CF, MCM, 1, NWC, ABL>(R, glive, lane, geo, c.cref_fwd, c.cref_bwd, t1f, t1b, c.dir);
            if (CF != 1) issue_pass<CF, MCM, 2, NWC, ABL>(R, glive, lane, geo, c.cref_fwd, c.cref_bwd, t2f, t2b, c.dir);
        }
        __builtin_amdgcn_sched_barrier(0);
        if (!(ABL & 8)) {
#pragma unroll
            for (int j = 0; j < Passes<CF>::N; j++) ((uint32_t*)c.wsink)[j * 4] = 0u;
        }
    }

    Stamps st;
#pragma unroll
    for (int i = 0; i < 7; i++) st.acc[i] = 0;
    stamp<ABL>(st, -1);
    for (; g < mb_end; g += STEP) {
        stamp<ABL>(st, 6);
        uint32_t p0[4] = {0, 0, 0, 0}, p1[NWC], p2[NWC];
#pragma unroll
        for (int d = 0; d < NWC; d++) p1[d] = p2[d] = 0;
        if (MCM) {
            touch(t0f), touch(t1f);
            if (MCM == 2) touch(t0b), touch(t1b);
            if (CF != 1) touch(t2f);
            if (CF != 1 && MCM == 2) touch(t2b);
            predict<MCM, 4, ABL>(t0f, t0b, lane, p0);
            predict<MCM, NWC, ABL>(t1f, t1b, lane, p1);
            if (CF != 1) predict<MCM, NWC, ABL>(t2f, t2b, lane, p2);
        }

        stamp<ABL>(st, 0);
        const uint32_t gn = g + STEP < mb_end ? g + STEP : g;
        const int ngN = (int)min(mb_end - gn, (uint32_t)G);
        const bool gliveN = kl < ngN;
        const LaneRec R = lane_rec(rvN, lane);
        if (MCM) issue_pass<CF, MCM, 0, 4, ABL>(R, gliveN, lane, geo, c.ref_fwd, c.ref_bwd, t0f, t0b, c.dir);
        const Group SN = group_state<NB>(rvN, ngN);
        __builtin_amdgcn_sched_barrier(0);
        rvN = rec_load(c.mbrec, g + 2 * STEP < mb_end ? g + 2 * STEP : g, mb_last, lane);

        stamp<ABL>(st, 1);
        if constexpr (MCM != 0) {
            const uint32_t e = dq_entry<CF>(S, lane);
            L.dq[wave][lane] = e;
            if (e & (1u << 19)) L.map[wave][e & 0xff] = (uint8_t)lane;
            wave_sync();
        }
        if (!(ABL & 4)) {
            if constexpr (MCM == 0) {
#pragma unroll
                for (int j = 0; j < NCW; j++) {
                    if (64 * j >= S.ncoef) break;
                    dequant_word<LT, true, NB>(L, wave, cw[j], S.qs8, 64 * j + lane < S.ncoef, c.half);
                }
            } else {
#pragma unroll
                for (int j = 0; j < NCW; j++)
                    if (64 * j + lane < S.ncoef) dequant_word<LT, false, NB>(L, wave, cw[j], S.qs8, true, c.half);
            }
            constexpr int XW = MCM == 0 ? 8 : 2;
            if (S.ncoef > 64 * NCW) {
                for (int base = 64 * NCW; base < S.ncoef; base += 64 * XW) {
                    uint32_t xw[XW];
#pragma unroll
                    for (int j = 0; j < XW; j++) {
                        const int wi = base + 64 * j + lane;
                        xw[j] = wi < S.ncoef ? ld_rec(&c.coefs[S.coef0 + wi]) : 0u;
                    }
#pragma unroll
                    for (int j = 0; j < XW; j++)
                        if (base + 64 * j + lane < S.ncoef) dequant_word<LT, MCM == 0, NB>(L, wave, xw[j], S.qs8, true, c.half);
                }
                __builtin_amdgcn_s_waitcnt(0x0f70);
            }
        }
        __builtin_amdgcn_sched_barrier(0);
        prefetch_words<MCM, NCW>(cw, c, SN.coef0, SN.ncoef, lane);
        __builtin_amdgcn_sched_barrier(0);
        wave_sync();

        stamp<ABL>(st, 2);
        bool odd = false;
        if constexpr ((ABL & (131072 | 262144)) != 0) odd = ((g - c.mb_begin) / STEP) & 1;
        if constexpr (!UNI) {
            for (int t = lane; t < (((ABL & 1) || ((ABL & 262144) && odd)) ? 0 : S.nslots * 4); t += 64) {
                const int slot = t >> 2, v = (t & 3) * 2;
                short* const bw = (short*)L.blk[wave];
                lds_uint4_t *pa, *pb;
                slot_chunks<LT>(bw, slot, v, v + 1, pa, pb);
                uint4 ra = ld16(pa);
                uint4 rb = ld16(pb);
                const int k = slot_kb<MCM, NB>(L, wave, slot) >> 4;
                const bool intra = MCM == 0 || (pick8(S.fl8, k) & MP2VG_MB_INTRA);
                uint32_t par = (ra.x ^ ra.y ^ ra.z ^ ra.w ^ rb.x ^ rb.y ^ rb.z ^ rb.w) & 0x00010001u;
                if (v == 0 && intra) par ^= ra.x & 1u;
                par = (par ^ (par >> 16)) & 1u;
                par ^= (uint32_t)__builtin_amdgcn_ds_swizzle((int)par, 0x041F);
                par ^= (uint32_t)__builtin_amdgcn_ds_swizzle((int)par, 0x081F);
                if (v == 6) rb.w ^= (par ^ 1u) << 16;
                short2_t s[8] = {__builtin_bit_cast(short2_t, ra.x), __builtin_bit_cast(short2_t, ra.y),
                                 __builtin_bit_cast(short2_t, ra.z), __builtin_bit_cast(short2_t, ra.w),
                                 __builtin_bit_cast(short2_t, rb.x), __builtin_bit_cast(short2_t, rb.y),
                                 __builtin_bit_cast(short2_t, rb.z), __builtin_bit_cast(short2_t, rb.w)};
                idct_1d<true>(s);
                pass1_store<LT>(bw, slot, v, s);
            }
            wave_sync();
            __builtin_amdgcn_sched_barrier(0);
            if (MCM) {
                issue_pass<CF, MCM, 1, NWC, ABL>(R, gliveN, lane, geo, c.cref_fwd, c.cref_bwd, t1f, t1b, c.dir);
                if (CF != 1) issue_pass<CF, MCM, 2, NWC, ABL>(R, gliveN, lane, geo, c.cref_fwd, c.cref_bwd, t2f, t2b, c.dir);
            }
            __builtin_amdgcn_sched_barrier(0);
            stamp<ABL>(st, 3);
            for (int t = lane; t < (((ABL & 1) || ((ABL & (131072 | 262144)) && odd)) ? 0 : S.nslots * 4); t += 64) {
                const int slot = t >> 2, xq = t & 3;
                const int x = (xq & 1) | ((xq & 2) << 1);
                short* const bw = (short*)L.blk[wave];
                lds_uint4_t *pa, *pb;
                slot_chunks<LT>(bw, slot, x, x + 2, pa, pb);
                const uint4 ra = ld16(pa);
                const uint4 rb = ld16(pb);
                zero16(pa);
                zero16(pb);
                short2_t s[8];
                interleave(ra, rb, s);
                idct_1d(s);
                const int kb = slot_kb<MCM, NB>(L, wave, slot);
                const int k = kb >> 4, bb = kb & 15;
                const bool dctf = pick8(S.fl8, k) & MP2VG_MB_DCT_FIELD;
                int plane, x0, y0, ys;
                block_origin<CF>(bb, dctf, plane, x0, y0, ys);
                const int rw = RL::width(plane);
                const int xp = RL::pos(x0 + x);
                if constexpr (LT::COMPACT) {
                    const uint32_t a0 = (uint32_t)(uintptr_t)(lds_u16_t*)((uint8_t*)L.res[wave] + RL::base(plane)) +
                                        mul24_asm((uint32_t)k, (uint32_t)RL::SIZE) + (uint32_t)(y0 * rw + xp);
                    put8_rows(a0, (uint32_t)(ys * rw), s);
                } else {
                    const uint32_t a0 = (uint32_t)(uintptr_t)(lds_short2_t*)(&L.res[wave][RL::base(plane)]) +
                                        2u * (mul24_asm((uint32_t)k, (uint32_t)RL::MBS) + (uint32_t)(y0 * rw + xp));
                    const uint32_t step = 2u * (uint32_t)(ys * rw);
#pragma unroll
                    for (int y = 0; y < 8; y++) *(lds_short2_t*)(uintptr_t)(a0 + (uint32_t)y * step) = s[y] >> (short)6;
                }
            }
            wave_sync();
        } else {
            const int n4 = S.nslots * 4;
            const int p2b = n4 > 64 ? n4 : 64;
            short* const bw = (short*)L.blk[wave];
            for (int base = 0; base < ((ABL & 1) ? 0 : p2b + n4); base += 64) {
                const int t = base + lane;
                const bool p1 = t < n4;
                const int u = p1 ? t : t - p2b;
                if (p1 || (t >= p2b && u < n4)) {
                    const int slot = u >> 2, q = u & 3;
                    const int v = q * 2;
                    const int x = (q & 1) | ((q & 2) << 1);
                    lds_uint4_t *pa, *pb;
                    slot_chunks<LT>(bw, slot, p1 ? v : x, p1 ? v + 1 : x + 2, pa, pb);
                    uint4 ra = ld16(pa);
                    uint4 rb = ld16(pb);
                    short2_t sv[8];
                    if (p1) {
                        uint32_t par = (ra.x ^ ra.y ^ ra.z ^ ra.w ^ rb.x ^ rb.y ^ rb.z ^ rb.w) & 0x00010001u;
                        if (v == 0) par ^= ra.x & 1u;
                        par = (par ^ (par >> 16)) & 1u;
                        par ^= (uint32_t)__builtin_amdgcn_ds_swizzle((int)par, 0x041F);
                        par ^= (uint32_t)__builtin_amdgcn_ds_swizzle((int)par, 0x081F);
                        if (v == 6) rb.w ^= (par ^ 1u) << 16;
                        sv[0] = __builtin_bit_cast(short2_t, ra.x), sv[1] = __builtin_bit_cast(short2_t, ra.y);
                        sv[2] = __builtin_bit_cast(short2_t, ra.z), sv[3] = __builtin_bit_cast(short2_t, ra.w);
                        sv[4] = __builtin_bit_cast(short2_t, rb.x), sv[5] = __builtin_bit_cast(short2_t, rb.y);
                        sv[6] = __builtin_bit_cast(short2_t, rb.z), sv[7] = __builtin_bit_cast(short2_t, rb.w);
                    } else {
                        zero16(pa);
                        zero16(pb);
                        interleave(ra, rb, sv);
                    }
                    if (base + 64 <= n4)
                        idct_1d<true>(sv);
                    else
                        idct_1d(sv);
                    if (p1) {
                        pass1_store<LT>(bw, slot, v, sv);
                    } else {
                        const int kb = slot_kb<MCM, NB>(L, wave, slot);
                        const int k = kb >> 4, bb = kb & 15;
                        const bool dctf = pick8(S.fl8, k) & MP2VG_MB_DCT_FIELD;
                        int plane, x0, y0, ys;
                        block_origin<CF>(bb, dctf, plane, x0, y0, ys);
                        const int rw = RL::width(plane);
                        const int xp = RL::pos(x0 + x);
                        const uint32_t a0 = (uint32_t)(uintptr_t)(lds_u16_t*)((uint8_t*)L.res[wave] + RL::base(plane)) +
                                            mul24_asm((uint32_t)k, (uint32_t)RL::SIZE) + (uint32_t)(y0 * rw + xp);
                        put8_rows(a0, (uint32_t)(ys * rw), sv);
                    }
                }
                wave_sync();
            }
            stamp<ABL>(st, 3);
        }

        stamp<ABL>(st, 4);
        if constexpr (LT::COMPACT) {
            const uint8_t* res8 = (const uint8_t*)L.res[wave];
            store_pass_put8<CF, 0, 4>(gr0, glive, lane, geo, c.wsink, c.dst_slot, c.dst_rsrc, res8);
            store_pass_put8<CF, 1, NWC>(gr0, glive, lane, geo, c.wsink, c.dst_slot, c.dst_rsrc, res8);
            if (CF != 1) store_pass_put8<CF, 2, NWC>(gr0, glive, lane, geo, c.wsink, c.dst_slot, c.dst_rsrc, res8);
            if (TILES && c.tiles) {
                const uint32_t r00 = (uint32_t)__builtin_amdgcn_readfirstlane((int)gr0);
                tile_group<CF, false, ABL>(r00 & 0xffff, r00 >> 16, lane, geo, c.wsink, c.dst_tiles, c.tile_rsrc, res8);
            }
        } else {
            store_pass<CF, 0, 4, ABL>(gr0, gr1, glive, lane, geo, c.wsink, c.dst_slot, c.dst_rsrc, MCM != 2 && c.tiles, L.res[wave], p0);
            store_pass<CF, 1, NWC, ABL>(gr0, gr1, glive, lane, geo, c.wsink, c.dst_slot, c.dst_rsrc, MCM != 2 && c.tiles, L.res[wave], p1);
            if (CF != 1) store_pass<CF, 2, NWC, ABL>(gr0, gr1, glive, lane, geo, c.wsink, c.dst_slot, c.dst_rsrc, MCM != 2 && c.tiles, L.res[wave], p2);
            if (MCM != 2 && c.tiles) {
                wave_sync();
                const uint32_t r00 = (uint32_t)__builtin_amdgcn_readfirstlane((int)gr0);
                tile_group<CF, true, ABL>(r00 & 0xffff, r00 >> 16, lane, geo, c.wsink, c.dst_tiles, c.tile_rsrc,
                                          (const uint8_t*)L.res[wave]);
            }
        }
        wave_sync();

        stamp<ABL>(st, 5);
        S = SN;
        gr0 = R.r0;
        gr1 = R.r1;
        glive = gliveN;
    }
    if ((ABL & 16) && lane == 0) {
        unsigned long long* out = (unsigned long long*)(geo.sink + 1024) + 8 * MCM;
#pragma unroll
        for (int i = 0; i < 7; i++) atomicAdd(&out[i], (unsigned long long)st.acc[i]);
        atomicAdd(&out[7], 1ull);
    }
}

template <int CF, int MCM, int ABL = 0>
__global__ __launch_bounds__((64 * kernel_waves<MCM, ABL>())) __attribute__((amdgpu_waves_per_eu((MCM == 0 || MCM == 4) && (ABL & ~kAblCompact) == 0 ? (CF == 3 ? 4 : 6) : (CF == 3 ? 3 : 4)))) void recon_kernel(const mp2vg_picture_t* __restrict__ pics,
                                                    const uint32_t* __restrict__ mbrec,
                                                    const uint32_t* __restrict__ coefs,
                                                    const SliceDesc* __restrict__ slices,
                                                    const Geo geo,
                                                    const uint32_t slice_base, const uint32_t nslices,
                                                    const uint32_t mates) {
    using LT = Lds<CF, compact_layout<MCM, ABL>(), kernel_waves<MCM, ABL>()>;
    __shared__ __attribute__((aligned(128))) LT L;
    const int tid = threadIdx.x;
    const int lane = tid & 63;
    const int wave = __builtin_amdgcn_readfirstlane(tid >> 6);
    static_assert(slices_per_wg<CF, MCM, ABL>(4) <= (uint32_t)LT::NH, "one matrix set per slice");
    const uint32_t spw = slices_per_wg<CF, MCM, ABL>(mates);
    const bool two = spw > 1;
    const uint32_t wps = 4u / spw;
    const uint32_t nunits = (nslices + spw - 1) / spw;
    const uint32_t b = blockIdx.x, q8 = nunits / 8, r8 = nunits % 8, xcd = b % 8;
    const uint32_t unit = xcd * q8 + min(xcd, r8) + b / 8;
    const int half = two ? (int)((uint32_t)wave / wps) : 0;
    const uint32_t si = spw * unit + (uint32_t)half;
    const bool have = si < nslices;
    const SliceDesc sd = slices[slice_base + min(si, nslices - 1)];
    const mp2vg_picture_t* pic = pics + sd.pic;
    const int alt = pic->alternate_scan & 1;

    if ((uint32_t)wave % wps == 0 && (two || tid < 64)) {
        ((uint32_t*)L.W)[64 * half + lane] = ((const uint32_t*)pic->W)[lane];
        const int r = c_scan_raster[alt][lane];
        const int pos = (r >> 4) * 16 + (r & 7) * 2 + ((r >> 3) & 1);
        L.scan[64 * half + lane] = (uint8_t)(LT::WB ? 2 * pos : pos);
        if constexpr (LT::WB && MP2VG_I_KBTAB) {
            const int k = lane >> 4, bb = lane & 15;
            const uint32_t slot = (uint32_t)(k * Fmt<CF>::NB + (bb < Fmt<CF>::NB ? bb : 0));
            L.kbtab[lane] = (((slot << 7) | ((slot << 4) & 0x70u)) << 8) | ((uint32_t)k * 8u);
        }
        if constexpr (LT::WB && CF != 1) {
#pragma unroll
            for (int bb = 0; bb < Fmt<CF>::NB; bb++) L.Wb[bb][lane] = pic->W[bb < 6 ? 0 : 2][lane];
        }
    }
    for (int i = lane; i < LT::NBUF * LT::MAXS * LT::BLK / 2; i += 64) ((uint32_t*)L.blk[wave * LT::NBUF])[i] = 0;
    __syncthreads();
    if (!have) return;

    SliceCtx c;
    c.mbrec = mbrec;
    c.coefs = coefs;
    c.dst_slot = (uint8_t*)geo.ftab[pic->dst_slot];
    c.wsink = geo.sink + 2048 + ((b * LT::NWAVES + wave) & 1023) * 64;
    c.dst_tiles = (uint8_t*)geo.ttab[pic->dst_slot];
    c.dst_rsrc = slot_rsrc(c.dst_slot, (uint32_t)geo.slot_bytes);
    c.tile_rsrc = slot_rsrc(c.dst_tiles, (uint32_t)(2 * geo.slot_bytes));
    c.tiles = sd.reserved & 1u;
    const bool one_dir = sd.reserved & 2u;
    c.dir = (sd.reserved >> 2) & 1u;
    const int fs0 = pic->fwd_slot < 0 ? pic->dst_slot : pic->fwd_slot;
    const int bs = pic->bwd_slot < 0 ? pic->dst_slot : pic->bwd_slot;
    const int fs = c.dir ? bs : fs0;
    c.ref_fwd = slot_rsrc((const uint8_t*)geo.ttab[fs], (uint32_t)(2 * geo.slot_bytes));
    c.ref_bwd = slot_rsrc((const uint8_t*)geo.ttab[bs], (uint32_t)(2 * geo.slot_bytes));
    if (kChromaTiles) {
        c.cref_fwd = c.ref_fwd, c.cref_bwd = c.ref_bwd;
    } else {
        c.cref_fwd = slot_rsrc((const uint8_t*)geo.ftab[fs], (uint32_t)geo.slot_bytes);
        c.cref_bwd = slot_rsrc((const uint8_t*)geo.ftab[bs], (uint32_t)geo.slot_bytes);
    }
    c.coef_rsrc = __builtin_amdgcn_make_buffer_rsrc((void*)coefs, (short)0, (int)kNoTap, 0x00020000);
    c.mb_begin = sd.mb_begin;
    c.mb_end = sd.mb_begin + sd.mb_count;
    c.half = half;
    c.wpos = two ? (uint32_t)wave % wps : (uint32_t)wave;
    c.step = (two ? wps : (uint32_t)LT::NWAVES) * G;
    if constexpr (MCM == 4) {
        run_slice<CF, 0, ABL, LT, false>(c, geo, L, lane, wave);
    } else if constexpr (MCM < 3) {
        run_slice<CF, (ABL & 2) ? 0 : MCM, ABL, LT>(c, geo, L, lane, wave);
    } else {
        const int pct = pic->picture_coding_type;
        if (pct == 3 && !one_dir)
            run_slice<CF, (ABL & 2) ? 0 : 2, ABL, LT>(c, geo, L, lane, wave);
        else if (pct == 2 || one_dir)
            run_slice<CF, (ABL & 2) ? 0 : 1, ABL, LT>(c, geo, L, lane, wave);
        else
            run_slice<CF, 0, ABL, LT>(c, geo, L, lane, wave);
    }
}
__device__ __forceinline__ uint64_t mix64(uint64_t z) {
    z = (z ^ (z >> 30)) * 0xBF58476D1CE4E5B9ull;
    z = (z ^ (z >> 27)) * 0x94D049BB133111EBull;
    return z ^ (z >> 31);
}

__global__ void digest_kernel(const uint64_t* __restrict__ ftab, const int32_t* __restrict__ slots,
                              uint64_t o0, uint64_t o1, uint64_t o2, int s0, int s1, int w0, int w1, int h0, int h1,
                              unsigned long long* __restrict__ out) {
    const int si = blockIdx.y;
    const uint8_t* base = (const uint8_t*)ftab[slots[si]];
    const int rows = h0 + 2 * h1;
    uint64_t acc = 0;
    for (int row = blockIdx.x; row < rows; row += gridDim.x) {
        const uint8_t* p;
        int w;
        if (row < h0) {
            p = base + o0 + (uint64_t)row * s0;
            w = w0;
        } else if (row < h0 + h1) {
            p = base + o1 + (uint64_t)(row - h0) * s1;
            w = w1;
        } else {
            p = base + o2 + (uint64_t)(row - h0 - h1) * s1;
            w = w1;
        }
        for (int x = threadIdx.x * 4; x < w; x += blockDim.x * 4) {
            const uint32_t d = *(const uint32_t*)(p + x);
            acc += mix64(mix64(((uint64_t)row << 32) | (uint64_t)x) ^ (uint64_t)d);
        }
    }
    for (int off = 32; off > 0; off >>= 1) acc += __shfl_xor(acc, off);
    if ((threadIdx.x & 63) == 0) atomicAdd(&out[si], (unsigned long long)acc);
}

template <int CF, int MCM, int ABL>
static void launch_one(const KArgs& a, const Geo& g, hipStream_t stream) {
    const uint32_t spw = slices_per_wg<CF, MCM, ABL>(a.mates);
    hipLaunchKernelGGL((recon_kernel<CF, MCM, ABL>), dim3((a.nslices + spw - 1) / spw),
                       dim3(64 * kernel_waves<MCM, ABL>()), 0, stream, a.pics, (const uint32_t*)a.mbs, a.coefs,
                       a.slices, g, a.slice_base, a.nslices, spw);
}

template <int CF, int ABL>
static hipError_t launch_mcm(int mcm, const KArgs& a, const Geo& g, hipStream_t stream) {
    switch (mcm) {
    case 0: launch_one<CF, 0, ABL>(a, g, stream); break;
    case 1: launch_one<CF, 1, ABL>(a, g, stream); break;
    case 2: launch_one<CF, 2, ABL>(a, g, stream); break;
    case 3: launch_one<CF, 3, ABL>(a, g, stream); break;
    case 4: launch_one<CF, 4, ABL>(a, g, stream); break;
    default: return hipErrorInvalidValue;
    }
    return hipGetLastError();
}

hipError_t launch_recon(int cf, int mcm, const KArgs& a, hipStream_t stream) {
    Geo g;
    g.sink = a.sink;
    g.slot_bytes = a.slot_bytes;
    g.ftab = a.ftab;
    g.ttab = a.ttab;
    for (int i = 0; i < 3; i++) {
        g.plane_off[i] = (uint32_t)a.plane_off[i];
        g.stride[i] = a.stride[i];
        g.ph[i] = a.ph[i];
    }
    static const int ablate = getenv("MP2VG_ABLATE") ? atoi(getenv("MP2VG_ABLATE")) : 0;
#ifndef MP2VG_DEV_ABLATIONS
    if (ablate) return hipErrorNotSupported;
#else
    if (cf == 3 && ablate == 16) return launch_mcm<3, 16>(mcm, a, g, stream);
    if (cf == 1 && ablate) {
        switch (ablate) {
        case 1: return launch_mcm<1, 1>(mcm, a, g, stream);
        case 2: return launch_mcm<1, 2>(mcm, a, g, stream);
        case 4: return launch_mcm<1, 4>(mcm, a, g, stream);
        case 8: return launch_mcm<1, 8>(mcm, a, g, stream);
        case 15: return launch_mcm<1, 15>(mcm, a, g, stream);
        case 16: return launch_mcm<1, 16>(mcm, a, g, stream);
        case 32: return launch_mcm<1, 32>(mcm, a, g, stream);
        case 64: return launch_mcm<1, 64>(mcm, a, g, stream);
        case 96: return launch_mcm<1, 96>(mcm, a, g, stream);
        case 128: return launch_mcm<1, 128>(mcm, a, g, stream);
        case 512: return launch_mcm<1, 512>(mcm, a, g, stream);
        case 2048: return launch_mcm<1, 2048>(mcm, a, g, stream);
        case 2056: return launch_mcm<1, 2056>(mcm, a, g, stream);
        case 4096: return launch_mcm<1, 4096>(mcm, a, g, stream);
        case 8192: return launch_mcm<1, 8192>(mcm, a, g, stream);
        case 32768: return launch_mcm<1, 32768>(mcm, a, g, stream);
        case 65536: return launch_mcm<1, 65536>(mcm, a, g, stream);
        case 131072: return launch_mcm<1, 131072>(mcm, a, g, stream);
        case 262144: return launch_mcm<1, 262144>(mcm, a, g, stream);
        default: return hipErrorInvalidValue;
        }
    }
#endif
    switch (cf) {
    case 1: return launch_mcm<1, 0>(mcm, a, g, stream);
    case 2: return launch_mcm<2, 0>(mcm, a, g, stream);
    case 3: return launch_mcm<3, 0>(mcm, a, g, stream);
    default: return hipErrorInvalidValue;
    }
}

__global__ void __launch_bounds__(256) tile_convert_kernel(const Geo geo, int cw, const int32_t* __restrict__ list,
                                                           int32_t slot0) {
    const int32_t slot = list ? list[blockIdx.y] : slot0;
    const uint8_t* frame = (const uint8_t*)geo.ftab[slot];
    uint8_t* tiles = (uint8_t*)geo.ttab[slot];
#pragma unroll
    for (int plane = 0; plane < 3; plane++) {
        const int w = plane == 0 ? 16 : cw;
        const int R = w == 16 ? 4 : 8, RB = 128 / R;
        const uint32_t ncol = (uint32_t)geo.stride[plane] / w;
        const uint32_t n = (uint32_t)geo.ph[plane] / R * ncol * 8;
        for (uint32_t i = blockIdx.x * 256 + threadIdx.x; i < n; i += gridDim.x * 256) {
            const uint32_t line = i >> 3, c = i & 7;
            const uint32_t band = line / ncol, t = line % ncol;
            const uint32_t r = c / (RB / 16), o = (c % (RB / 16)) * 16;
            const uint8_t* src = frame + geo.plane_off[plane] + (size_t)(band * R + r) * geo.stride[plane] + t * w + o;
            const uint2 lo = *(const uint2*)src, hi = *(const uint2*)(src + 8);
            *(uint4*)(tiles + 2 * (size_t)geo.plane_off[plane] + (size_t)line * 128 + c * 16) =
                make_uint4(lo.x, lo.y, hi.x, hi.y);
        }
    }
}

hipError_t launch_tile_convert(const KArgs& a, int cf, const int32_t* d_list, int n, int32_t slot0, hipStream_t stream) {
    Geo g;
    g.ftab = a.ftab;
    g.ttab = a.ttab;
    for (int i = 0; i < 3; i++) {
        g.plane_off[i] = (uint32_t)a.plane_off[i];
        g.stride[i] = a.stride[i];
        g.ph[i] = a.ph[i];
    }
    const int cw = cf == 3 ? 16 : 8;
    hipLaunchKernelGGL(tile_convert_kernel, dim3(128, d_list ? n : 1), dim3(256), 0, stream, g, cw, d_list, slot0);
    return hipGetLastError();
}

__global__ void __launch_bounds__(256) frame_copy_kernel(FrameCopy fc, uint64_t bytes) {
    typedef uint32_t u4v_t __attribute__((ext_vector_type(4)));
    const int f = blockIdx.y;
    const uint8_t* __restrict__ src = fc.src[f];
    uint8_t* __restrict__ dst = fc.dst[f];
    const uint64_t n16 = bytes >> 4, step = (uint64_t)gridDim.x * 256;
    for (uint64_t i = (uint64_t)blockIdx.x * 256 + threadIdx.x; i < n16; i += step)
        ((u4v_t*)dst)[i] = ((const u4v_t*)src)[i];
    if (blockIdx.x == 0)
        for (uint64_t i = (n16 << 4) + threadIdx.x; i < bytes; i += 256) dst[i] = src[i];
}

hipError_t launch_frame_copy(const FrameCopy& fc, int n, uint64_t bytes, hipStream_t stream) {
    if (n < 1 || n > kFrameCopyMax) return hipErrorInvalidValue;
    for (int i = 0; i < n; i++)
        if (((uintptr_t)fc.src[i] | (uintptr_t)fc.dst[i]) & 15) return hipErrorInvalidValue;
    static const int wgs = getenv("MP2VG_DL_WGS") ? std::max(1, atoi(getenv("MP2VG_DL_WGS"))) : 64;
    dim3 block(256), grid(n < wgs ? wgs / n : 1, n);
    hipLaunchKernelGGL(frame_copy_kernel, grid, block, 0, stream, fc, bytes);
    return hipGetLastError();
}

__global__ void __launch_bounds__(256) clock_probe_kernel(unsigned long long* __restrict__ out, int iters) {
    uint32_t a = threadIdx.x, b = a * 2654435761u, c2 = a ^ 0x9e3779b9u, d = ~a;
    uint64_t t0, r0, t1, r1;
    asm volatile("s_memtime %0\n s_memrealtime %1\n s_waitcnt lgkmcnt(0)" : "=s"(t0), "=s"(r0)::"memory");
    for (int i = 0; i < iters; i++) {
        asm volatile("v_add_u32 %0, %0, %1\n v_xor_b32 %1, %1, %2\n v_add_u32 %2, %2, %3\n v_xor_b32 %3, %3, %0"
                     : "+v"(a), "+v"(b), "+v"(c2), "+v"(d));
    }
    asm volatile("s_memtime %0\n s_memrealtime %1\n s_waitcnt lgkmcnt(0)" : "=s"(t1), "=s"(r1)::"memory");
    if ((a ^ b ^ c2 ^ d) == 0x12345678u) out[2] = 1;
    if ((threadIdx.x & 63) == 0) {
        atomicAdd(&out[0], (unsigned long long)(t1 - t0));
        atomicAdd(&out[1], (unsigned long long)(r1 - r0));
    }
}

hipError_t launch_clock_probe(unsigned long long* d_out, int iters, int blocks, hipStream_t stream) {
    hipLaunchKernelGGL(clock_probe_kernel, dim3(blocks), dim3(256), 0, stream, d_out, iters);
    return hipGetLastError();
}

template <bool RW>
__global__ void __launch_bounds__(256) block_probe_kernel(u4v* __restrict__ p, size_t n, uint32_t zero, int reps,
                                                          u4v* __restrict__ sink) {
    u4v acc = {0, 0, 0, 0};
    for (int r = 0; r < reps; r++)
        for (size_t i = (size_t)blockIdx.x * 256 + threadIdx.x; i < n; i += (size_t)gridDim.x * 256) {
            u4v v = p[i];
            if (RW) {
                v.x ^= zero;
                p[i] = v;
            } else {
                acc ^= v;
            }
        }
    if (!RW && (acc.x ^ acc.y ^ acc.z ^ acc.w) == ~zero) sink[threadIdx.x] = acc;
}

template <bool LOCK, bool RW = false>
__global__ void __launch_bounds__(256) pool_scatter_kernel(const uint64_t* __restrict__ tab, int nslots,
                                                           uint32_t fkb, uint32_t tkb, int iters,
                                                           u4v* __restrict__ sink, uint32_t zero) {
    const uint32_t wave = blockIdx.x * 4 + (threadIdx.x >> 6), lane = threadIdx.x & 63;
    u4v acc = {0, 0, 0, 0};
    uint32_t h = wave * 2654435761u + 12345u;
    for (int i = 0; i < iters; i++) {
        uint32_t slot, tile, kb;
        if (LOCK) {
            slot = wave % nslots;
            tile = wave / nslots & 1;
            kb = (uint32_t)i * 4 % (tile ? tkb : fkb);
        } else {
            h ^= h << 13, h ^= h >> 17, h ^= h << 5;
            slot = h % nslots;
            tile = h >> 31;
            const uint32_t g = h * 0x9e3779b1u;
            kb = (g >> 8) % (tile ? tkb : fkb);
        }
        u4v* p = (u4v*)(tab[tile * nslots + slot] + (uint64_t)kb * 1024) + lane;
        u4v v = *p;
        if (RW) {
            v.x ^= zero;
            *p = v;
        } else {
            acc ^= v;
        }
    }
    if ((acc.x ^ acc.y ^ acc.z ^ acc.w) == ~zero) sink[threadIdx.x] = acc;
}

__global__ void __launch_bounds__(256) block_random_kernel(const uint8_t* __restrict__ base, uint32_t kbs, int iters,
                                                           u4v* __restrict__ sink, uint32_t zero) {
    const uint32_t wave = blockIdx.x * 4 + (threadIdx.x >> 6), lane = threadIdx.x & 63;
    u4v acc = {0, 0, 0, 0};
    uint32_t h = wave * 2654435761u + 777u;
    for (int i = 0; i < iters; i++) {
        h ^= h << 13, h ^= h >> 17, h ^= h << 5;
        const uint32_t kb = (h * 0x9e3779b1u >> 8) % kbs;
        acc ^= *((const u4v*)(base + (uint64_t)kb * 1024) + lane);
    }
    if ((acc.x ^ acc.y ^ acc.z ^ acc.w) == ~zero) sink[threadIdx.x] = acc;
}

hipError_t launch_block_random(const void* base, size_t bytes, int waves, int iters, void* sink, hipStream_t stream) {
    hipLaunchKernelGGL(block_random_kernel, dim3(waves / 4), dim3(256), 0, stream, (const uint8_t*)base,
                       (uint32_t)(bytes >> 10), iters, (u4v*)sink, 0u);
    return hipGetLastError();
}

hipError_t launch_pool_scatter(const uint64_t* tab, int nslots, uint32_t fkb, uint32_t tkb, int lock, int waves,
                               int iters, void* sink, hipStream_t stream) {
    if (lock >= 2)
        hipLaunchKernelGGL((lock == 2 ? pool_scatter_kernel<true, true> : pool_scatter_kernel<false, true>),
                           dim3(waves / 4), dim3(256), 0, stream, tab, nslots, fkb, tkb, iters, (u4v*)sink, 0u);
    else if (lock)
        hipLaunchKernelGGL(pool_scatter_kernel<true>, dim3(waves / 4), dim3(256), 0, stream, tab, nslots, fkb, tkb,
                           iters, (u4v*)sink, 0u);
    else
        hipLaunchKernelGGL(pool_scatter_kernel<false>, dim3(waves / 4), dim3(256), 0, stream, tab, nslots, fkb, tkb,
                           iters, (u4v*)sink, 0u);
    return hipGetLastError();
}

hipError_t launch_block_probe(void* p, size_t bytes, int rw, int reps, void* sink, hipStream_t stream) {
    const size_t n = bytes / 16;
    if (rw)
        hipLaunchKernelGGL(block_probe_kernel<true>, dim3(2048), dim3(256), 0, stream, (u4v*)p, n, 0u, reps, (u4v*)sink);
    else
        hipLaunchKernelGGL(block_probe_kernel<false>, dim3(2048), dim3(256), 0, stream, (u4v*)p, n, 0u, reps, (u4v*)sink);
    return hipGetLastError();
}

hipError_t launch_digest(const uint64_t* ftab, const int32_t* d_slots, int n,
                         const uint64_t off[3], const int32_t stride[3], const int32_t w[3],
                         const int32_t h[3], unsigned long long* d_out, hipStream_t stream) {
    dim3 block(256), grid(64, n);
    hipLaunchKernelGGL(digest_kernel, grid, block, 0, stream, ftab, d_slots, off[0], off[1], off[2],
                       stride[0], stride[1], w[0], w[1], h[0], h[1], d_out);
    return hipGetLastError();
}

}
```

tiny_mp2v_dec_amd/csrc/recon_kernel.h:

```cpp
#pragma once
#include <hip/hip_runtime.h>
#include <stdint.h>

#include "../../include/mp2vg.h"

namespace mp2vg {

struct SliceDesc {
    uint32_t pic;
    uint32_t mb_begin;
    uint32_t mb_count;
    uint32_t reserved;
};

struct Launch {
    uint32_t begin, end;
    int mcm;
    int mates = 0;
    int level;
    int set;
};

struct Geo {
    uint8_t* sink;
    uint64_t slot_bytes;
    const uint64_t* ftab;
    const uint64_t* ttab;
    uint32_t plane_off[3];
    int32_t stride[3];
    int32_t ph[3];
};

struct KArgs {
    const mp2vg_picture_t* pics;
    const mp2vg_mb_t* mbs;
    const uint32_t* coefs;
    const SliceDesc* slices;
    uint8_t* sink;
    uint64_t slot_bytes;
    const uint64_t *ftab, *ttab;
    uint64_t plane_off[3];
    int32_t stride[3];
    int32_t ph[3];
    uint32_t slice_base;
    uint32_t nslices;
    uint32_t mates = 0;
};

constexpr int kFrameCopyMax = 32;
struct FrameCopy {
    const uint8_t* src[kFrameCopyMax];
    uint8_t* dst[kFrameCopyMax];
};
hipError_t launch_frame_copy(const FrameCopy& fc, int n, uint64_t bytes, hipStream_t stream);

}
```

tiny_mp2v_dec_amd/csrc/runtime.cpp:

```cpp
#include <hip/hip_runtime.h>

#include <algorithm>
#include <cmath>
#include <cstdio>
#include <cstring>
#include <string>
#include <vector>
#include <atomic>
#include <thread>

#include "export_kernel.h"
#include "hipchk.h"
#include "parse_kernel.h"
#include "recon_kernel.h"
#include "syntax.h"
#include "tensor_kernel.h"

namespace mp2vg {
hipError_t launch_recon(int cf, int mcm, const KArgs& a, hipStream_t stream);
hipError_t launch_tile_convert(const KArgs& a, int cf, const int32_t* d_list, int n, int32_t slot0, hipStream_t stream);
hipError_t launch_clock_probe(unsigned long long* d_out, int iters, int blocks, hipStream_t stream);
hipError_t launch_block_probe(void* p, size_t bytes, int rw, int reps, void* sink, hipStream_t stream);
hipError_t launch_block_random(const void* base, size_t bytes, int waves, int iters, void* sink, hipStream_t stream);
hipError_t launch_pool_scatter(const uint64_t* tab, int nslots, uint32_t fkb, uint32_t tkb, int lock, int waves,
                               int iters, void* sink, hipStream_t stream);
hipError_t launch_digest(const uint64_t* ftab, const int32_t* d_slots, int n,
                         const uint64_t off[3], const int32_t stride[3], const int32_t w[3],
                         const int32_t h[3], unsigned long long* d_out, hipStream_t stream);
}

using namespace mp2vg;


static constexpr size_t kPoolPad = 4096 + 65536;
static constexpr size_t kSinkOff = 2048;
static constexpr size_t kCoefPad = 256;
static constexpr size_t kStageBytes = 32u << 20;
static constexpr size_t kMbPad = 16;
static int default_streams(const mp2vg_config_t* cfg) {
    if (cfg->reserved & MP2VG_CTX_ONE_STREAM) return 1;
    const char* e = getenv("MP2VG_STREAMS");
    return e ? std::max(1, atoi(e)) : 2;
}
static const char* dev_env(const char* name) {
#ifdef MP2VG_DEV_ABLATIONS
    return getenv(name);
#else
    (void)name;
    return nullptr;
#endif
}
static void pool_block_free(uint8_t* p, size_t bytes, uint64_t vmm);
static void free_held_pools(mp2vg_ctx_t* c);
static size_t slot_pad() {
    const char* e = dev_env("MP2VG_SLOT_PAD");
    return e ? (size_t)std::max(0, atoi(e)) & ~(size_t)255 : 0;
}
static size_t tile_pad() {
    const char* e = dev_env("MP2VG_TILE_PAD");
    return e ? (size_t)std::max(0, atoi(e)) & ~(size_t)255 : 0;
}
static int set_coupling() {
    const char* e = dev_env("MP2VG_SET_COUPLE");
    return e ? atoi(e) : 0;
}

struct TilePlan {
    std::vector<std::pair<int32_t, int32_t>> ext_reads;
    std::vector<std::pair<int32_t, uint8_t>> writes;
    std::vector<std::pair<int32_t, int32_t>> post;
};

struct Bank {
    mp2vg_picture_t* d_pics = nullptr;
    size_t cap_pics = 0;
    mp2vg_mb_t* d_mbs = nullptr;
    size_t cap_mbs = 0;
    uint32_t* d_coefs = nullptr;
    size_t cap_coefs = 0;
    SliceDesc* d_slices = nullptr;
    size_t cap_slices = 0;
    int32_t* d_post = nullptr;
    size_t cap_post = 0;
    uint8_t* h_small = nullptr;
    size_t cap_small = 0;
    std::vector<std::pair<int32_t, int32_t>> post_of;
    std::vector<Launch> launches;
    std::vector<std::vector<int32_t>> foot;
    TilePlan tiles;
    int32_t npics = 0;
    uint64_t nmbs = 0, ncoefs = 0;
    hipEvent_t uploaded = nullptr;
    hipEvent_t consumed = nullptr;
    bool decoded = false;
};

struct PoolSet;
struct mp2vg_ctx {
    mp2vg_config_t cfg{};
    Geom g{};
    hipStream_t stream = nullptr;
    hipStream_t ustream = nullptr;
    std::vector<hipStream_t> sstreams;
    std::vector<hipEvent_t> sev;
    std::vector<hipEvent_t> lev;
    std::vector<std::vector<uint8_t>> last_foot;
    uint8_t* d_pool = nullptr;
    int32_t nslots = 0;
    size_t slot_stride = 0;
    uint8_t* d_tiles = nullptr;
    std::vector<uint64_t> fptr, tptr;
    std::vector<uint8_t*> chunks;
    std::vector<size_t> chunk_bytes;
    std::vector<uint64_t> chunk_vmm;
    uint64_t* d_tab = nullptr;
    uint8_t* d_sink = nullptr;
    std::vector<uint8_t> tiles_ok;
    size_t tile_stride = 0;
    int nstreams = 2;
    int ncu = 0;

    Bank bank[2];
    int cur = -1;
    bool batch_ready = false;

    struct BatchEv {
        hipEvent_t b[2] = {nullptr, nullptr};
        std::vector<hipEvent_t> s;
        int ns = 0;
        std::vector<hipEvent_t> l;
        int nl = 0;
    };
    static constexpr int kHist = 64;
    BatchEv hist[kHist];
    uint64_t seq = 0;
    hipEvent_t up_ev[2] = {nullptr, nullptr};
    bool launch_timing = true;
    bool placed = false;
    std::vector<float> place_ms;
    int place_kept = -1;
    std::vector<PoolSet*> place_held;

    void* h_stage = nullptr;
    int32_t* d_dslots = nullptr;
    unsigned long long* d_digest = nullptr;
    size_t cap_digest = 0;

    struct ExportStage {
        int32_t* h = nullptr;
        int32_t* d = nullptr;
        size_t cap = 0;
        hipEvent_t done = nullptr;
    };
    static constexpr int kExportRing = 4;
    ExportStage estage[kExportRing];
    uint32_t eseq = 0;
    hipEvent_t export_ev = nullptr;
    std::vector<uint32_t> swaited;
    uint32_t export_synced = 0;

    void* es = nullptr;
    void (*es_free)(void*) = nullptr;
};

template <class T>
static int grow(T*& p, size_t& cap, size_t n) {
    if (n <= cap) return MP2VG_OK;
    if (p) HIPCHK(hipFree(p));
    p = nullptr;
    size_t c = std::max(n, cap * 3 / 2);
    HIPCHK(hipMalloc((void**)&p, c * sizeof(T)));
    cap = c;
    return MP2VG_OK;
}

static int upload(mp2vg_ctx_t* ctx, void* dst, const void* src, size_t bytes, bool pinned) {
    if (pinned) {
        if (bytes) HIPCHK(hipMemcpyAsync(dst, src, bytes, hipMemcpyHostToDevice, ctx->ustream));
        return MP2VG_OK;
    }
    const uint8_t* s = (const uint8_t*)src;
    uint8_t* d = (uint8_t*)dst;
    const size_t half = kStageBytes / 2;
    for (int i = 0; bytes; i++) {
        const size_t n = std::min(bytes, half);
        uint8_t* st = (uint8_t*)ctx->h_stage + (i & 1) * half;
        if (i >= 2) HIPCHK(hipEventSynchronize(ctx->up_ev[i & 1]));
        memcpy(st, s, n);
        HIPCHK(hipMemcpyAsync(d, st, n, hipMemcpyHostToDevice, ctx->ustream));
        HIPCHK(hipEventRecord(ctx->up_ev[i & 1], ctx->ustream));
        s += n;
        d += n;
        bytes -= n;
    }
    HIPCHK(hipStreamSynchronize(ctx->ustream));
    return MP2VG_OK;
}

extern "C" int mp2vg_create(const mp2vg_config_t* cfg, mp2vg_ctx_t** out) {
    if (!cfg || !out) return MP2VG_E_INVALID;
    *out = nullptr;
    if (mp2vg_frame_geometry(cfg, nullptr, nullptr, nullptr, nullptr) != MP2VG_OK) return MP2VG_E_INVALID;
    int ndev = 0;
    HIPCHK(hipGetDeviceCount(&ndev));
    if (cfg->device < 0 || cfg->device >= ndev) {
        set_error("no such HIP device");
        return MP2VG_E_HIP;
    }
    HIPCHK(hipSetDevice(cfg->device));
    if (const char* qw = dev_env("MP2VG_QUEUE_WARM")) {
        static bool warmed = false;
        if (!warmed) {
            warmed = true;
            void* buf = nullptr;
            if (hipMalloc(&buf, 4096) == hipSuccess)
                for (int i = 0; i < atoi(qw); i++) {
                    hipStream_t st;
                    if (hipStreamCreateWithFlags(&st, hipStreamNonBlocking) == hipSuccess)
                        (void)hipMemsetAsync(buf, 0, 4096, st);
                }
            (void)hipDeviceSynchronize();
        }
    }
    mp2vg_ctx_t* c = new mp2vg_ctx_t();
    c->cfg = *cfg;
    c->g.init(cfg->width, cfg->height, cfg->chroma_format);
    c->slot_stride = c->g.slot_bytes + slot_pad();
    c->tile_stride = ((2 * c->g.slot_bytes + 255) & ~(size_t)255) + tile_pad();
    c->nstreams = default_streams(cfg);
    if (hipDeviceGetAttribute(&c->ncu, hipDeviceAttributeMultiprocessorCount, cfg->device) != hipSuccess) c->ncu = 0;
    bool ok = true;
    for (Bank& b : c->bank)
        ok = ok && hipEventCreateWithFlags(&b.uploaded, hipEventDisableTiming | hipEventBlockingSync) == hipSuccess &&
             hipEventCreateWithFlags(&b.consumed, hipEventDisableTiming) == hipSuccess;
    if (!ok || hipStreamCreateWithFlags(&c->stream, hipStreamNonBlocking) != hipSuccess ||
        hipStreamCreateWithFlags(&c->ustream, hipStreamNonBlocking) != hipSuccess ||
        hipEventCreateWithFlags(&c->up_ev[0], hipEventDisableTiming) != hipSuccess ||
        hipEventCreateWithFlags(&c->up_ev[1], hipEventDisableTiming) != hipSuccess ||
        hipHostMalloc(&c->h_stage, kStageBytes, hipHostMallocDefault) != hipSuccess) {
        set_error("stream / pinned staging allocation failed");
        mp2vg_destroy(c);
        return MP2VG_E_HIP;
    }
    int rc = mp2vg_reserve_slots(c, std::max(1, cfg->pictures_pool_size));
    if (rc != MP2VG_OK) {
        mp2vg_destroy(c);
        return rc;
    }
    *out = c;
    return MP2VG_OK;
}

extern "C" int mp2vg_destroy(mp2vg_ctx_t* c) {
    if (!c) return MP2VG_E_INVALID;
    hipSetDevice(c->cfg.device);
    if (c->stream) hipStreamSynchronize(c->stream);
    if (c->ustream) hipStreamSynchronize(c->ustream);
    if (c->es && c->es_free) c->es_free(c->es);
    for (auto& h : c->hist) {
        for (auto e : h.l) hipEventDestroy(e);
        for (auto e : h.s)
            if (e) hipEventDestroy(e);
        for (auto e : h.b)
            if (e) hipEventDestroy(e);
    }
    for (auto e : c->up_ev)
        if (e) hipEventDestroy(e);

    hipFree(c->d_pool);
    hipFree(c->d_tiles);
    for (size_t i = 0; i < c->chunks.size(); i++) pool_block_free(c->chunks[i], c->chunk_bytes[i], c->chunk_vmm[i]);
    free_held_pools(c);
    hipFree(c->d_tab);
    hipFree(c->d_sink);
    for (Bank& b : c->bank) {
        hipFree(b.d_pics);
        hipFree(b.d_mbs);
        hipFree(b.d_coefs);
        hipFree(b.d_slices);
        hipFree(b.d_post);
        if (b.h_small) hipHostFree(b.h_small);
        if (b.uploaded) hipEventDestroy(b.uploaded);
        if (b.consumed) hipEventDestroy(b.consumed);
    }
    hipFree(c->d_dslots);
    hipFree(c->d_digest);
    for (auto& e : c->estage) {
        if (e.h) hipHostFree(e.h);
        hipFree(e.d);
        if (e.done) hipEventDestroy(e.done);
    }
    if (c->export_ev) hipEventDestroy(c->export_ev);
    if (c->h_stage) hipHostFree(c->h_stage);
    for (auto st : c->sstreams) hipStreamSynchronize(st);
    for (auto e : c->sev) hipEventDestroy(e);
    for (auto e : c->lev) hipEventDestroy(e);
    for (auto st : c->sstreams) hipStreamDestroy(st);
    if (c->ustream) hipStreamDestroy(c->ustream);
    if (c->stream) hipStreamDestroy(c->stream);
    delete c;
    return MP2VG_OK;
}

static int finish_reserve(mp2vg_ctx_t* c, int32_t nslots) {
    hipFree(c->d_tab);
    c->d_tab = nullptr;
    HIPCHK(hipMalloc((void**)&c->d_tab, sizeof(uint64_t) * 2 * nslots));
    HIPCHK(hipMemcpyAsync(c->d_tab, c->fptr.data(), sizeof(uint64_t) * nslots, hipMemcpyHostToDevice, c->stream));
    HIPCHK(hipMemcpyAsync(c->d_tab + nslots, c->tptr.data(), sizeof(uint64_t) * nslots, hipMemcpyHostToDevice,
                          c->stream));
    HIPCHK(hipStreamSynchronize(c->stream));
    c->tiles_ok.resize(nslots, 1);
    c->nslots = nslots;
    c->last_foot.clear();
    return MP2VG_OK;
}

static hipError_t pool_block_alloc(int device, size_t bytes, uint8_t** p, size_t* got, uint64_t* vmm) {
    *vmm = 0;
    size_t sz = bytes;
    const char* pw = dev_env("MP2VG_POOL_POW2");
    const char* vm = dev_env("MP2VG_POOL_VMM");
    if ((pw && atoi(pw)) || vm) {
        sz = 1;
        while (sz < bytes) sz <<= 1;
    }
    *got = sz;
    if (!vm) return hipMalloc((void**)p, sz);
    hipMemAllocationProp prop = {};
    prop.type = hipMemAllocationTypePinned;
    prop.location.type = hipMemLocationTypeDevice;
    prop.location.id = device;
    size_t gran = 0;
    hipError_t e = hipMemGetAllocationGranularity(&gran, &prop, hipMemAllocationGranularityRecommended);
    if (e != hipSuccess) return e;
    sz = (sz + gran - 1) / gran * gran;
    *got = sz;
    const size_t align = atoi(vm) > 0 ? (size_t)atoi(vm) << 20 : sz;
    hipMemGenericAllocationHandle_t h;
    if ((e = hipMemCreate(&h, sz, &prop, 0)) != hipSuccess) return e;
    void* va = nullptr;
    if ((e = hipMemAddressReserve(&va, sz, align, nullptr, 0)) != hipSuccess) {
        hipMemRelease(h);
        return e;
    }
    if ((e = hipMemMap(va, sz, 0, h, 0)) != hipSuccess) {
        hipMemAddressFree(va, sz);
        hipMemRelease(h);
        return e;
    }
    hipMemAccessDesc acc = {};
    acc.location = prop.location;
    acc.flags = hipMemAccessFlagsProtReadWrite;
    if ((e = hipMemSetAccess(va, sz, &acc, 1)) != hipSuccess) {
        hipMemUnmap(va, sz);
        hipMemAddressFree(va, sz);
        hipMemRelease(h);
        return e;
    }
    *p = (uint8_t*)va;
    *vmm = (uint64_t)(uintptr_t)h;
    return hipSuccess;
}

static void pool_block_free(uint8_t* p, size_t bytes, uint64_t vmm) {
    if (!vmm) {
        hipFree(p);
        return;
    }
    hipMemUnmap(p, bytes);
    hipMemAddressFree(p, bytes);
    hipMemRelease((hipMemGenericAllocationHandle_t)(uintptr_t)vmm);
}

extern "C" int mp2vg_reserve_slots(mp2vg_ctx_t* c, int32_t nslots) {
    if (!c || nslots <= 0) return MP2VG_E_INVALID;
    HIPCHK(hipSetDevice(c->cfg.device));
    if (nslots <= c->nslots) return MP2VG_OK;
    HIPCHK(hipStreamSynchronize(c->stream));
    if (!c->d_sink) {
        HIPCHK(hipMalloc((void**)&c->d_sink, kPoolPad));
        HIPCHK(hipMemsetAsync(c->d_sink, 0, kPoolPad, c->stream));
    }
    static const int chunk = getenv("MP2VG_POOL_CHUNK") ? std::max(0, atoi(getenv("MP2VG_POOL_CHUNK"))) : 16;
    if (chunk > 0) {
        std::vector<uint8_t*> blocks;
        std::vector<size_t> bsz;
        std::vector<uint64_t> fp, tp, vh;
        auto fail = [&](hipError_t e) {
            for (size_t i = 0; i < blocks.size(); i++) pool_block_free(blocks[i], bsz[i], vh[i]);
            set_error(std::string("hipMalloc (frame pool block): ") + hipGetErrorString(e));
            return MP2VG_E_HIP;
        };
        for (int s0 = c->nslots; s0 < nslots; s0 += chunk) {
            const int k = std::min(chunk, nslots - s0);
            uint8_t *f = nullptr, *t = nullptr;
            size_t got = 0;
            uint64_t h = 0;
            hipError_t e = pool_block_alloc(c->cfg.device, c->slot_stride * k + kPoolPad, &f, &got, &h);
            if (e != hipSuccess) return fail(e);
            blocks.push_back(f);
            bsz.push_back(got);
            vh.push_back(h);
            if ((e = pool_block_alloc(c->cfg.device, c->tile_stride * k, &t, &got, &h)) != hipSuccess) return fail(e);
            blocks.push_back(t);
            bsz.push_back(got);
            vh.push_back(h);
            if ((e = hipMemsetAsync(f, 0, c->slot_stride * k + kPoolPad, c->stream)) != hipSuccess ||
                (e = hipMemsetAsync(t, 0, c->tile_stride * k, c->stream)) != hipSuccess)
                return fail(e);
            for (int i = 0; i < k; i++) {
                fp.push_back((uint64_t)(uintptr_t)(f + (size_t)i * c->slot_stride));
                tp.push_back((uint64_t)(uintptr_t)(t + (size_t)i * c->tile_stride));
            }
        }
        c->chunks.insert(c->chunks.end(), blocks.begin(), blocks.end());
        c->chunk_bytes.insert(c->chunk_bytes.end(), bsz.begin(), bsz.end());
        c->chunk_vmm.insert(c->chunk_vmm.end(), vh.begin(), vh.end());
        c->fptr.insert(c->fptr.end(), fp.begin(), fp.end());
        c->tptr.insert(c->tptr.end(), tp.begin(), tp.end());
        return finish_reserve(c, nslots);
    }
    uint8_t* p = nullptr;
    uint8_t* t = nullptr;
    size_t bytes = c->slot_stride * nslots + kPoolPad;
    const size_t tbytes = c->tile_stride * nslots;
#ifdef MP2VG_DEV_ABLATIONS
    static const int pool_alloc = getenv("MP2VG_POOL_ALLOC") ? atoi(getenv("MP2VG_POOL_ALLOC")) : 0;
    if (pool_alloc == 1 && hipExtMallocWithFlags((void**)&p, bytes, hipDeviceMallocContiguous) != hipSuccess) {
        (void)hipGetLastError();
        p = nullptr;
    }
    static uint8_t* ballast = nullptr;
    static const size_t ballast_mb = getenv("MP2VG_BALLAST_MB") ? (size_t)atoll(getenv("MP2VG_BALLAST_MB")) : 0;
    if (pool_alloc == 5 && !ballast &&
        hipMalloc((void**)&ballast, ballast_mb ? ballast_mb << 20 : bytes + tbytes) != hipSuccess)
        (void)hipGetLastError(), ballast = nullptr;
#endif
    if (!p) HIPCHK(hipMalloc((void**)&p, bytes));
    if (hipMalloc((void**)&t, tbytes) != hipSuccess) {
        hipFree(p);
        set_error("out of device memory for the anchor tiles");
        return MP2VG_E_HIP;
    }
    HIPCHK(hipMemsetAsync(p, 0, bytes, c->stream));
    HIPCHK(hipMemsetAsync(t, 0, tbytes, c->stream));
    if (c->d_pool) {
        HIPCHK(hipMemcpyAsync(p, c->d_pool, c->slot_stride * c->nslots, hipMemcpyDeviceToDevice, c->stream));
        HIPCHK(hipMemcpyAsync(t, c->d_tiles, c->tile_stride * c->nslots, hipMemcpyDeviceToDevice, c->stream));
        HIPCHK(hipStreamSynchronize(c->stream));
        HIPCHK(hipFree(c->d_pool));
        HIPCHK(hipFree(c->d_tiles));
    }
    HIPCHK(hipStreamSynchronize(c->stream));
    c->d_pool = p;
    c->d_tiles = t;
    c->fptr.resize(nslots);
    c->tptr.resize(nslots);
    for (int i = 0; i < nslots; i++) {
        c->fptr[i] = (uint64_t)(uintptr_t)(p + (size_t)i * c->slot_stride);
        c->tptr[i] = (uint64_t)(uintptr_t)(t + (size_t)i * c->tile_stride);
    }
    return finish_reserve(c, nslots);
}

static int plan_from_uses(mp2vg_ctx_t* c, const mp2vg_picture_t* pics, int32_t npics, const uint8_t* uses_of,
                          const char* const* err, std::vector<SliceDesc>& slices, std::vector<Launch>& launches,
                          std::vector<std::vector<int32_t>>* foot, TilePlan* tplan);

static int plan_batch(mp2vg_ctx_t* c, const mp2vg_picture_t* pics, int32_t npics, const mp2vg_mb_t* mbs,
                      uint64_t nmbs, const uint32_t* coefs, uint64_t ncoefs, std::vector<SliceDesc>& slices,
                      std::vector<Launch>& launches, std::vector<std::vector<int32_t>>* foot = nullptr,
                      bool trusted = false, TilePlan* tplan = nullptr) {
    const int mbw = c->cfg.width / 16, mbh = c->cfg.height / 16;
    const int nb = c->g.nblocks;
    if (ncoefs + kCoefPad >= (1ull << 30)) {
        set_error("batch with 2^30 or more coefficient words (4 GB): split it");
        return MP2VG_E_INVALID;
    }
    std::vector<uint8_t> uses_of(2 * (size_t)npics, 0);
    std::vector<const char*> err(npics, nullptr);
    auto bad_type = [&](int p) { return pics[p].picture_coding_type < 1 || pics[p].picture_coding_type > 3; };
    auto uses_only = [&](int p) -> const char* {
        const mp2vg_picture_t& P = pics[p];
        if (bad_type(p)) return "picture_coding_type is not 1 (I), 2 (P) or 3 (B)";
        if (P.mb_width != mbw || P.mb_height != mbh) return "picture size differs from the context geometry";
        if (P.dst_slot < 0 || P.dst_slot >= c->nslots || P.fwd_slot >= c->nslots || P.bwd_slot >= c->nslots)
            return "frame slot out of range (mp2vg_reserve_slots)";
        const uint64_t nm = (uint64_t)mbw * mbh;
        if ((uint64_t)P.mb_first + nm > nmbs) return "picture MB range outside the batch";
        bool uses[2] = {false, false};
        for (uint64_t k = 0; k < nm; k++) {
            const mp2vg_mb_t& m = mbs[P.mb_first + k];
            if ((uint64_t)m.coef_off + m.ncoef > ncoefs) return "MB coefficient range outside the batch";
            const uint16_t f = m.flags;
            if (!(f & MP2VG_MB_INTRA)) {
                uses[0] |= (f & MP2VG_MB_FWD) || !(f & MP2VG_MB_BWD);
                uses[1] |= (f & MP2VG_MB_BWD) != 0;
            }
        }
        uses_of[2 * (size_t)p] = uses[0];
        uses_of[2 * (size_t)p + 1] = uses[1];
        return nullptr;
    };
    auto validate = [&](int p) -> const char* {
        if (trusted) return uses_only(p);
        const mp2vg_picture_t& P = pics[p];
        if (bad_type(p)) return "picture_coding_type is not 1 (I), 2 (P) or 3 (B)";
        if (P.mb_width != mbw || P.mb_height != mbh) return "picture size differs from the context geometry";
        if (P.dst_slot < 0 || P.dst_slot >= c->nslots || P.fwd_slot >= c->nslots || P.bwd_slot >= c->nslots)
            return "frame slot out of range (mp2vg_reserve_slots)";
        const uint64_t nm = (uint64_t)mbw * mbh;
        if ((uint64_t)P.mb_first + nm > nmbs) return "picture MB range outside the batch";
        bool uses[2] = {false, false};
        for (uint64_t k = 0; k < nm; k++) {
            const mp2vg_mb_t& m = mbs[P.mb_first + k];
            if (m.x != k % mbw || m.y != k / mbw) return "MB records not in raster order";
            if ((uint64_t)m.coef_off + m.ncoef > ncoefs) return "MB coefficient range outside the batch";
            const uint32_t tag = MP2VG_COEF_MBX(m.x);
            const uint32_t first = MP2VG_COEF_DC | MP2VG_COEF_FIRST1S;
            uint32_t bad = 0, blocks = 0, pos0 = 0;
            const uint32_t* w = coefs + m.coef_off;
            for (uint32_t j = 0; j < m.ncoef; j++) {
                bad |= (w[j] & 0x9C000000u) ^ tag;
                blocks |= 1u << MP2VG_COEF_BLOCK(w[j]);
                pos0 |= (w[j] & first) ? MP2VG_COEF_POS(w[j]) : 0u;
            }
            if (bad) return "coefficient word bits 26-28 are not the MB column mod 8 (or bit 31 is set)";
            if (pos0) return "DC or '1s' coefficient word with a nonzero scan position";
            if (blocks & ~(uint32_t)m.cbp) return "coefficient word of a block the MB's cbp does not code";
            if (k % mbw != 0) {
                const mp2vg_mb_t& pm = mbs[P.mb_first + k - 1];
                if ((uint64_t)pm.coef_off + pm.ncoef != m.coef_off)
                    return "coefficient words of a macroblock row are not contiguous";
            }
            if (m.cbp >> nb) return "cbp names a block the chroma format does not have";
            if (nb == 12 && (m.flags & MP2VG_MB_DCT_FIELD) && m.cbp)
                return "4:4:4 field-DCT macroblock (reference block 10/11 placement is unsupported)";
            if ((m.flags & MP2VG_MB_INTRA) && m.cbp != (1u << nb) - 1)
                return "intra macroblock whose cbp does not code every block";
            if (P.picture_coding_type == 1 && !(m.flags & MP2VG_MB_INTRA)) return "non-intra macroblock in an I picture";
            if (!(m.flags & MP2VG_MB_INTRA)) {
                const bool dir[2] = {(m.flags & MP2VG_MB_FWD) || !(m.flags & MP2VG_MB_BWD), (m.flags & MP2VG_MB_BWD) != 0};
                uses[0] |= dir[0];
                uses[1] |= dir[1];
                const bool field = m.flags & MP2VG_MB_FIELD_MC;
                for (int r = 0; r < (field ? 2 : 1); r++)
                    for (int s = 0; s < 2; s++)
                        if (dir[s] && !mc_reads_inside(c->g, m.x, m.y, m.mv[r][s][0], m.mv[r][s][1], field,
                                                       (m.flags & MP2VG_MB_FS_BIT(r, s)) ? 1 : 0, r))
                            return "motion vector reads outside the reference planes";
            }
        }
        uses_of[2 * (size_t)p] = uses[0];
        uses_of[2 * (size_t)p + 1] = uses[1];
        return nullptr;
    };
    parallel_for(npics, 16, [&](int p) { err[p] = validate(p); });
    return plan_from_uses(c, pics, npics, uses_of.data(), err.data(), slices, launches, foot, tplan);
}

static int plan_from_uses(mp2vg_ctx_t* c, const mp2vg_picture_t* pics, int32_t npics, const uint8_t* uses_of,
                          const char* const* err, std::vector<SliceDesc>& slices, std::vector<Launch>& launches,
                          std::vector<std::vector<int32_t>>* foot, TilePlan* tplan) {
    const int mbw = c->cfg.width / 16, mbh = c->cfg.height / 16;
    std::vector<int> level(npics, 0);
    std::vector<int> last_write(c->nslots, -1), max_read(c->nslots, -1);
    int maxlevel = -1;
    for (int p = 0; p < npics; p++) {
        const mp2vg_picture_t& P = pics[p];
        if (err && err[p]) {
            set_error(err[p]);
            return MP2VG_E_INVALID;
        }
        const bool uses[2] = {uses_of[2 * (size_t)p] != 0, uses_of[2 * (size_t)p + 1] != 0};
        if (P.picture_coding_type == 2 && uses[1]) {
            set_error("backward prediction in a P picture");
            return MP2VG_E_INVALID;
        }
        if ((uses[0] && P.fwd_slot < 0) || (uses[1] && P.bwd_slot < 0)) {
            set_error("picture predicts from a missing reference slot");
            return MP2VG_E_INVALID;
        }
        int lv = 0;
        if (uses[0]) lv = std::max(lv, last_write[P.fwd_slot] + 1);
        if (uses[1]) lv = std::max(lv, last_write[P.bwd_slot] + 1);
        lv = std::max(lv, last_write[P.dst_slot] + 1);
        lv = std::max(lv, max_read[P.dst_slot] + 1);
        if ((uses[0] && P.fwd_slot == P.dst_slot) || (uses[1] && P.bwd_slot == P.dst_slot)) {
            set_error("picture predicts from its own slot");
            return MP2VG_E_INVALID;
        }
        level[p] = lv;
        if (uses[0]) max_read[P.fwd_slot] = std::max(max_read[P.fwd_slot], lv);
        if (uses[1]) max_read[P.bwd_slot] = std::max(max_read[P.bwd_slot], lv);
        last_write[P.dst_slot] = lv;
        max_read[P.dst_slot] = -1;
        maxlevel = std::max(maxlevel, lv);
    }
    const int nsets = std::max(1, std::min(c->nstreams, npics));
    std::vector<int> parent(npics);
    for (int p = 0; p < npics; p++) parent[p] = p;
    auto find = [&](int x) {
        while (parent[x] != x) x = parent[x] = parent[parent[x]];
        return x;
    };
    {
        std::vector<int> owner(c->nslots, -1);
        for (int p = 0; p < npics; p++) {
            const mp2vg_picture_t& P = pics[p];
            const int sl[3] = {P.dst_slot, uses_of[2 * (size_t)p] ? P.fwd_slot : -1,
                               uses_of[2 * (size_t)p + 1] ? P.bwd_slot : -1};
            for (int s : sl) {
                if (s < 0) continue;
                if (owner[s] < 0) owner[s] = p;
                else parent[find(p)] = find(owner[s]);
            }
        }
    }
    std::vector<int> set_of(npics, 0), root_set(npics, -1);
    std::vector<size_t> load(nsets, 0);
    for (int p = 0; p < npics; p++) {
        const int r = find(p);
        if (root_set[r] < 0) root_set[r] = (int)(std::min_element(load.begin(), load.end()) - load.begin());
        set_of[p] = root_set[r];
        load[set_of[p]]++;
    }
    if (foot) {
        foot->assign(nsets, {});
        std::vector<int8_t> seen((size_t)c->nslots * nsets, 0);
        for (int p = 0; p < npics; p++) {
            const mp2vg_picture_t& P = pics[p];
            const int sl[3] = {P.dst_slot, uses_of[2 * (size_t)p] ? P.fwd_slot : -1,
                               uses_of[2 * (size_t)p + 1] ? P.bwd_slot : -1};
            for (int x : sl)
                if (x >= 0 && !seen[(size_t)set_of[p] * c->nslots + x]) {
                    seen[(size_t)set_of[p] * c->nslots + x] = 1;
                    (*foot)[set_of[p]].push_back(x);
                }
        }
    }
    std::vector<uint8_t> need(npics, 0);
    {
        std::vector<int> writer(c->nslots, -1);
        std::vector<uint8_t> ext(c->nslots, 0);
        for (int p = 0; p < npics; p++) {
            const mp2vg_picture_t& P = pics[p];
            const int rs[2] = {uses_of[2 * (size_t)p] ? P.fwd_slot : -1, uses_of[2 * (size_t)p + 1] ? P.bwd_slot : -1};
            for (int s : rs) {
                if (s < 0) continue;
                if (writer[s] >= 0) {
                    need[writer[s]] = 1;
                } else if (!ext[s]) {
                    ext[s] = 1;
                    if (tplan) tplan->ext_reads.push_back({s, set_of[p]});
                }
            }
            writer[P.dst_slot] = p;
        }
        for (int p = npics - 1, anchors = 0; p >= 0 && anchors < 2; p--)
            if (pics[p].picture_coding_type != 3) need[p] = 1, anchors++;
        if (tplan)
            for (int p = 0; p < npics; p++) tplan->writes.push_back({pics[p].dst_slot, need[p]});
    }
    slices.clear();
    launches.clear();
    static const int rows_pb = dev_env("MP2VG_SLICE_ROWS") ? std::max(1, atoi(dev_env("MP2VG_SLICE_ROWS"))) : 2;
    static const int mates = !dev_env("MP2VG_MATES") ? 2 : atoi(dev_env("MP2VG_MATES")) == 4 ? 4 : (atoi(dev_env("MP2VG_MATES")) ? 2 : 0);
    static const bool pair_order = !dev_env("MP2VG_PAIR_ORDER") || atoi(dev_env("MP2VG_PAIR_ORDER")) != 0;
    static const int rows_i_env = dev_env("MP2VG_SLICE_ROWS_I") ? std::max(1, atoi(dev_env("MP2VG_SLICE_ROWS_I"))) : 0;
    const int rows_i = rows_i_env ? rows_i_env : (c->g.cf == 3 ? 2 : 1);
    static const int i_split = dev_env("MP2VG_I_SPLIT") ? std::max(1, atoi(dev_env("MP2VG_I_SPLIT"))) : 1;
    static const int i_mbs = dev_env("MP2VG_I_SLICE_MBS") ? std::max(0, atoi(dev_env("MP2VG_I_SLICE_MBS"))) : 0;
    auto i_slice_groups = [&](size_t npic_launch) -> int {
        const int s0 = rows_i * mbw / 4;
        if (rows_i_env || i_mbs || i_split > 1 || mbw % 4) return s0;
        const double cap = (double)(c->ncu > 0 ? c->ncu : 256) * (c->g.cf == 3 ? 4 : 6) / std::max(1, nsets);
        const double gtot = (double)npic_launch * (mbw / 4) * mbh;
        auto waste = [&](int sg) {
            const double r = std::ceil(gtot / sg) / cap;
            return std::ceil(r) - r;
        };
        int best = s0;
        for (int sg = s0 + 1; sg <= s0 + s0 / 4; sg++)
            if (waste(sg) < waste(best)) best = sg;
        return waste(s0) - waste(best) >= 0.1 ? best : s0;
    };
    for (int set = 0; set < nsets; set++)
    for (int q = 0; q <= maxlevel; q++) {
        std::vector<int> lp;
        for (int p = 0; p < npics; p++)
            if (level[p] == q && set_of[p] == set) lp.push_back(p);
        if (lp.empty()) continue;
        Launch l;
        l.begin = (uint32_t)slices.size();
        static const bool route = !dev_env("MP2VG_ONE_DIR_B") || atoi(dev_env("MP2VG_ONE_DIR_B")) != 0;
        auto one_dir = [&](int p) {
            return route && pics[p].picture_coding_type == 3 && !(uses_of[2 * (size_t)p] && uses_of[2 * (size_t)p + 1]);
        };
        int types = 0;
        for (int p : lp) {
            const int pct = pics[p].picture_coding_type;
            types |= 1 << (pct == 1 ? 0 : (pct == 2 || one_dir(p) ? 1 : 2));
        }
        auto reads = [&](int p, int s) { return s >= 0 && (pics[p].fwd_slot == s || pics[p].bwd_slot == s); };
        auto sflags = [&](int p) -> uint32_t {
            const bool b = pics[p].picture_coding_type == 3;
            const bool bwd_only = !uses_of[2 * (size_t)p] && uses_of[2 * (size_t)p + 1];
            return (uint32_t)(need[p] && !b) | (one_dir(p) ? 2u : 0u) | (one_dir(p) && bwd_only ? 4u : 0u);
        };
        size_t i = 0;
        while (i < lp.size()) {
            size_t j = i + 1;
            while (j < lp.size() && j - i < 4) {
                bool share = false;
                for (size_t k = i; k < j && !share; k++)
                    share = reads(lp[j], pics[lp[k]].fwd_slot) || reads(lp[j], pics[lp[k]].bwd_slot);
                if (!share) break;
                j++;
            }
            const int slice_rows = (mbw % 4 != 0) ? 1 : (types == 1 ? rows_i : (mates ? 1 : rows_pb));
            auto push = [&](size_t k, int r) {
                slices.push_back({(uint32_t)lp[k], pics[lp[k]].mb_first + (uint32_t)(r * mbw),
                                  (uint32_t)(std::min(slice_rows, mbh - r) * mbw), sflags(lp[k])});
            };
            const bool paired = pair_order && mates == 2 && types != 1 && mbw % 4 == 0;
            if (paired && (j - i) % 2 == 1 && j - i > 1) {
                size_t o = j - 1;
                for (size_t k = i; k < j; k++)
                    if (pics[lp[k]].picture_coding_type == 2 || one_dir(lp[k])) o = k;
                for (int r = 0; r < mbh; r += 2) {
                    for (int rr = r; rr < std::min(r + 2, mbh); rr++)
                        for (size_t k = i; k < j; k++)
                            if (k != o) push(k, rr);
                    for (int rr = r; rr < std::min(r + 2, mbh); rr++) push(o, rr);
                }
            } else if (types == 1 && mbw % 4 == 0 &&
                       ((i_mbs > 0 && i_mbs % 4 == 0) || i_slice_groups(lp.size()) != rows_i * mbw / 4)) {
                const int cut = i_mbs > 0 ? i_mbs : 4 * i_slice_groups(lp.size());
                const int total = mbw * mbh;
                for (int m0 = 0; m0 < total; m0 += cut)
                    for (size_t k = i; k < j; k++)
                        slices.push_back({(uint32_t)lp[k], pics[lp[k]].mb_first + (uint32_t)m0,
                                          (uint32_t)std::min(cut, total - m0), sflags(lp[k])});
            } else if (types == 1 && slice_rows == 1 && i_split > 1 && (mbw / i_split) % 4 == 0 && mbw % i_split == 0) {
                const int pw = mbw / i_split;
                for (int r = 0; r < mbh; r++)
                    for (size_t k = i; k < j; k++)
                        for (int q = 0; q < i_split; q++)
                            slices.push_back({(uint32_t)lp[k], pics[lp[k]].mb_first + (uint32_t)(r * mbw + q * pw),
                                              (uint32_t)pw, sflags(lp[k])});
            } else {
                for (int r = 0; r < mbh; r += slice_rows)
                    for (size_t k = i; k < j; k++) push(k, r);
            }
            i = j;
        }
        l.end = (uint32_t)slices.size();
        l.mcm = types == 1 ? 0 : (types == 2 ? 1 : (types == 4 ? 2 : 3));
        static const int tilefree = dev_env("MP2VG_I_TILEFREE") ? atoi(dev_env("MP2VG_I_TILEFREE")) : 0;
        int nneed = 0;
        for (int p : lp) nneed += need[p];
        if (types == 1 && (tilefree == 2 || (tilefree && c->g.cf != 3 && nneed * 4 <= (int)lp.size()))) {
            l.mcm = 4;
            for (uint32_t k = l.begin; k < l.end; k++) slices[k].reserved = 0;
        }
        l.level = q;
        l.set = set;
        l.mates = (mates && types != 1 && l.mcm != 0 && l.mcm != 4 && mbw % 4 == 0) ? (c->g.cf == 3 ? std::min(mates, 2) : mates) : 0;
        if (tplan)
            for (int p : lp)
                if (need[p] && (pics[p].picture_coding_type == 3 || l.mcm == 4))
                    tplan->post.push_back({(int32_t)launches.size(), pics[p].dst_slot});
        launches.push_back(l);
    }
    return MP2VG_OK;
}

static int batch_upload(mp2vg_ctx_t* c, const mp2vg_picture_t* pics, int32_t npics, const mp2vg_mb_t* mbs,
                        uint64_t nmbs, const uint32_t* coefs, uint64_t ncoefs, bool pinned, bool async,
                        bool trusted = false) {
    if (!c || !pics || npics <= 0 || !mbs || (!coefs && ncoefs)) return MP2VG_E_INVALID;
    HIPCHK(hipSetDevice(c->cfg.device));
    c->batch_ready = false;
    std::vector<SliceDesc> slices;
    std::vector<Launch> lb;
    std::vector<std::vector<int32_t>> foot;
    TilePlan tplan;
    double tp = now_ms();
    int rc = plan_batch(c, pics, npics, mbs, nmbs, coefs, ncoefs, slices, lb, &foot, trusted, &tplan);
    if (rc != MP2VG_OK) return rc;
    tp = trace_phase("upload: plan", tp);
    const int k = (c->cur + 1) & 1;
    Bank& b = c->bank[k];
    if (b.decoded) HIPCHK(hipEventSynchronize(b.consumed));
    if ((rc = grow(b.d_pics, b.cap_pics, (size_t)npics)) != MP2VG_OK) return rc;
    if ((rc = grow(b.d_mbs, b.cap_mbs, (size_t)nmbs + kMbPad)) != MP2VG_OK) return rc;
    if ((rc = grow(b.d_coefs, b.cap_coefs, (size_t)ncoefs + kCoefPad)) != MP2VG_OK) return rc;
    if ((rc = grow(b.d_slices, b.cap_slices, slices.size())) != MP2VG_OK) return rc;
    std::vector<int32_t> ps;
    std::vector<std::pair<int32_t, int32_t>> post_of(lb.size(), {0, 0});
    for (size_t i = 0; i < lb.size(); i++) {
        post_of[i].first = (int32_t)ps.size();
        for (const auto& pc : tplan.post)
            if (pc.first == (int32_t)i) ps.push_back(pc.second);
        post_of[i].second = (int32_t)ps.size();
    }
    if (!ps.empty() && (rc = grow(b.d_post, b.cap_post, ps.size())) != MP2VG_OK) return rc;
    const size_t pic_bytes = sizeof(mp2vg_picture_t) * npics, sl_bytes = sizeof(SliceDesc) * slices.size(),
                 ps_bytes = sizeof(int32_t) * ps.size();
    if (async) {
        HIPCHK(hipEventSynchronize(b.uploaded));
        const size_t o1 = (pic_bytes + 255) & ~(size_t)255, o2 = o1 + ((sl_bytes + 255) & ~(size_t)255);
        const size_t need = o2 + ps_bytes;
        if (need > b.cap_small) {
            if (b.h_small) HIPCHK(hipHostFree(b.h_small));
            b.h_small = nullptr;
            b.cap_small = 0;
            const size_t cap = std::max(need, (size_t)1 << 20);
            HIPCHK(hipHostMalloc((void**)&b.h_small, cap, hipHostMallocDefault));
            b.cap_small = cap;
        }
        memcpy(b.h_small, pics, pic_bytes);
        memcpy(b.h_small + o1, slices.data(), sl_bytes);
        if (ps_bytes) memcpy(b.h_small + o2, ps.data(), ps_bytes);
        HIPCHK(hipMemcpyAsync(b.d_pics, b.h_small, pic_bytes, hipMemcpyHostToDevice, c->ustream));
        HIPCHK(hipMemcpyAsync(b.d_slices, b.h_small + o1, sl_bytes, hipMemcpyHostToDevice, c->ustream));
        if (ps_bytes) HIPCHK(hipMemcpyAsync(b.d_post, b.h_small + o2, ps_bytes, hipMemcpyHostToDevice, c->ustream));
    } else {
        if ((rc = upload(c, b.d_pics, pics, pic_bytes, false)) != MP2VG_OK) return rc;
        if ((rc = upload(c, b.d_slices, slices.data(), sl_bytes, false)) != MP2VG_OK) return rc;
        if (ps_bytes && (rc = upload(c, b.d_post, ps.data(), ps_bytes, false)) != MP2VG_OK) return rc;
    }
    if ((rc = upload(c, b.d_mbs, mbs, sizeof(mp2vg_mb_t) * nmbs, pinned)) != MP2VG_OK) return rc;
    if (ncoefs && (rc = upload(c, b.d_coefs, coefs, sizeof(uint32_t) * ncoefs, pinned)) != MP2VG_OK) return rc;
    HIPCHK(hipEventRecord(b.uploaded, c->ustream));
    if (!async) HIPCHK(hipStreamSynchronize(c->ustream));
    trace_phase("upload: copy", tp);
    b.launches = std::move(lb);
    b.foot = std::move(foot);
    b.post_of = std::move(post_of);
    b.tiles = std::move(tplan);
    b.npics = npics;
    b.nmbs = nmbs;
    b.ncoefs = ncoefs;
    c->cur = k;
    c->batch_ready = true;
    return MP2VG_OK;
}

namespace mp2vg {
int es_begin(mp2vg_ctx_t* c, const mp2vg_picture_t* pics, int32_t npics, uint64_t nmbs, EsBank* out) {
    HIPCHK(hipSetDevice(c->cfg.device));
    c->batch_ready = false;
    const int mbw = c->cfg.width / 16, mbh = c->cfg.height / 16;
    for (int p = 0; p < npics; p++) {
        const mp2vg_picture_t& P = pics[p];
        const char* e = nullptr;
        if (P.picture_coding_type < 1 || P.picture_coding_type > 3) e = "picture_coding_type is not 1 (I), 2 (P) or 3 (B)";
        else if (P.mb_width != mbw || P.mb_height != mbh) e = "picture size differs from the context geometry";
        else if (P.dst_slot < 0 || P.dst_slot >= c->nslots || P.fwd_slot >= c->nslots || P.bwd_slot >= c->nslots)
            e = "frame slot out of range (mp2vg_reserve_slots)";
        else if ((uint64_t)P.mb_first + (uint64_t)mbw * mbh > nmbs) e = "picture MB range outside the batch";
        if (e) {
            set_error(e);
            return MP2VG_E_INVALID;
        }
    }
    Bank& b = c->bank[(c->cur + 1) & 1];
    if (b.decoded) HIPCHK(hipEventSynchronize(b.consumed));
    int rc;
    if ((rc = grow(b.d_pics, b.cap_pics, (size_t)npics)) != MP2VG_OK) return rc;
    if ((rc = grow(b.d_mbs, b.cap_mbs, (size_t)nmbs + kMbPad)) != MP2VG_OK) return rc;
    out->device = c->cfg.device;
    out->stream = c->ustream;
    out->d_mbs = b.d_mbs;
    out->state = &c->es;
    out->state_free = &c->es_free;
    return MP2VG_OK;
}
int es_coefs(mp2vg_ctx_t* c, uint64_t ncoefs, uint32_t** d_coefs) {
    if (ncoefs + kCoefPad >= (1ull << 30)) {
        set_error("batch with 2^30 or more coefficient words (4 GB): split it");
        return MP2VG_E_INVALID;
    }
    Bank& b = c->bank[(c->cur + 1) & 1];
    const int rc = grow(b.d_coefs, b.cap_coefs, (size_t)ncoefs + kCoefPad);
    *d_coefs = b.d_coefs;
    return rc;
}
int es_commit(mp2vg_ctx_t* c, const mp2vg_picture_t* pics, int32_t npics, uint64_t nmbs, uint64_t ncoefs,
              const uint8_t* uses_of) {
    std::vector<SliceDesc> slices;
    std::vector<Launch> lb;
    std::vector<std::vector<int32_t>> foot;
    TilePlan tplan;
    int rc = plan_from_uses(c, pics, npics, uses_of, nullptr, slices, lb, &foot, &tplan);
    if (rc != MP2VG_OK) return rc;
    const int k = (c->cur + 1) & 1;
    Bank& b = c->bank[k];
    if ((rc = grow(b.d_slices, b.cap_slices, slices.size())) != MP2VG_OK) return rc;
    std::vector<int32_t> ps;
    std::vector<std::pair<int32_t, int32_t>> post_of(lb.size(), {0, 0});
    for (size_t i = 0; i < lb.size(); i++) {
        post_of[i].first = (int32_t)ps.size();
        for (const auto& pc : tplan.post)
            if (pc.first == (int32_t)i) ps.push_back(pc.second);
        post_of[i].second = (int32_t)ps.size();
    }
    if (!ps.empty() && (rc = grow(b.d_post, b.cap_post, ps.size())) != MP2VG_OK) return rc;
    if ((rc = upload(c, b.d_pics, pics, sizeof(mp2vg_picture_t) * npics, false)) != MP2VG_OK) return rc;
    if ((rc = upload(c, b.d_slices, slices.data(), sizeof(SliceDesc) * slices.size(), false)) != MP2VG_OK) return rc;
    if (!ps.empty() && (rc = upload(c, b.d_post, ps.data(), sizeof(int32_t) * ps.size(), false)) != MP2VG_OK) return rc;
    HIPCHK(hipEventRecord(b.uploaded, c->ustream));
    HIPCHK(hipStreamSynchronize(c->ustream));
    b.launches = std::move(lb);
    b.foot = std::move(foot);
    b.post_of = std::move(post_of);
    b.tiles = std::move(tplan);
    b.npics = npics;
    b.nmbs = nmbs;
    b.ncoefs = ncoefs;
    c->cur = k;
    c->batch_ready = true;
    return MP2VG_OK;
}
void* ctx_es_state(mp2vg_ctx_t* c) { return c->es; }
const mp2vg_config_t* ctx_config(const mp2vg_ctx_t* c) { return &c->cfg; }
}

extern "C" int mp2vg_batch_record_counts(mp2vg_ctx_t* c, uint64_t* nmbs, uint64_t* ncoefs) {
    if (!c) return MP2VG_E_INVALID;
    if (!c->batch_ready) {
        set_error("no batch uploaded");
        return MP2VG_E_STATE;
    }
    if (nmbs) *nmbs = c->bank[c->cur].nmbs;
    if (ncoefs) *ncoefs = c->bank[c->cur].ncoefs;
    return MP2VG_OK;
}

extern "C" int mp2vg_batch_download_records(mp2vg_ctx_t* c, mp2vg_mb_t* mbs, uint64_t nmbs, uint32_t* coefs,
                                            uint64_t ncoefs) {
    if (!c || !mbs || (!coefs && ncoefs)) return MP2VG_E_INVALID;
    if (!c->batch_ready) {
        set_error("no batch uploaded");
        return MP2VG_E_STATE;
    }
    const Bank& b = c->bank[c->cur];
    if (nmbs != b.nmbs || ncoefs != b.ncoefs) {
        set_error("record array sizes differ from the resident batch (mp2vg_batch_record_counts)");
        return MP2VG_E_INVALID;
    }
    HIPCHK(hipSetDevice(c->cfg.device));
    HIPCHK(hipEventSynchronize(b.uploaded));
    HIPCHK(hipMemcpy(mbs, b.d_mbs, sizeof(mp2vg_mb_t) * nmbs, hipMemcpyDeviceToHost));
    if (ncoefs) HIPCHK(hipMemcpy(coefs, b.d_coefs, sizeof(uint32_t) * ncoefs, hipMemcpyDeviceToHost));
    return MP2VG_OK;
}

static void init_shell(mp2vg_ctx_t& shell, const mp2vg_config_t* cfg, int32_t nslots) {
    shell.cfg = *cfg;
    shell.g.init(cfg->width, cfg->height, cfg->chroma_format);
    shell.nslots = nslots;
    shell.nstreams = default_streams(cfg);
}

extern "C" int mp2vg_batch_plan(const mp2vg_config_t* cfg, int32_t nslots, const mp2vg_picture_t* pics,
                                int32_t npics, const mp2vg_mb_t* mbs, uint64_t nmbs, const uint32_t* coefs,
                                uint64_t ncoefs, mp2vg_plan_t* out) {
    if (!cfg || nslots <= 0 || !pics || npics <= 0 || !mbs || (!coefs && ncoefs) || !out) return MP2VG_E_INVALID;
    if (mp2vg_frame_geometry(cfg, nullptr, nullptr, nullptr, nullptr) != MP2VG_OK) return MP2VG_E_INVALID;
    mp2vg_ctx_t shell;
    init_shell(shell, cfg, nslots);
    std::vector<SliceDesc> slices;
    std::vector<Launch> lb;
    std::vector<std::vector<int32_t>> foot;
    TilePlan tplan;
    const int rc = plan_batch(&shell, pics, npics, mbs, nmbs, coefs, ncoefs, slices, lb, &foot, false, &tplan);
    if (rc != MP2VG_OK) return rc;
    auto room = [](const void* p, int32_t i, int32_t max) { return p && i < max; };
    out->nslices = (int32_t)slices.size();
    for (int32_t i = 0; i < out->nslices && room(out->slices, i, out->max_slices); i++) {
        const uint32_t w[4] = {slices[i].pic, slices[i].mb_begin, slices[i].mb_count, slices[i].reserved};
        memcpy(out->slices + 4 * (size_t)i, w, sizeof w);
    }
    out->nlaunches = (int32_t)lb.size();
    for (int32_t i = 0; i < out->nlaunches && room(out->launches, i, out->max_launches); i++) {
        const int32_t w[6] = {(int32_t)lb[i].begin, (int32_t)lb[i].end, lb[i].mcm, lb[i].level, lb[i].set, lb[i].mates};
        memcpy(out->launches + 6 * (size_t)i, w, sizeof w);
    }
    auto pairs = [&](const std::vector<std::pair<int32_t, int32_t>>& v, int32_t* dst, int32_t max, int32_t* n) {
        *n = (int32_t)v.size();
        for (int32_t i = 0; i < *n && room(dst, i, max); i++) dst[2 * (size_t)i] = v[i].first, dst[2 * (size_t)i + 1] = v[i].second;
    };
    std::vector<std::pair<int32_t, int32_t>> wr, ft;
    for (const auto& w : tplan.writes) wr.push_back({w.first, (int32_t)w.second});
    for (size_t s = 0; s < foot.size(); s++)
        for (int32_t x : foot[s]) ft.push_back({(int32_t)s, x});
    pairs(wr, out->writes, out->max_writes, &out->nwrites);
    pairs(tplan.ext_reads, out->ext_reads, out->max_ext_reads, &out->next_reads);
    pairs(tplan.post, out->post, out->max_post, &out->npost);
    pairs(ft, out->foot, out->max_foot, &out->nfoot);
    out->nsets = (int32_t)foot.size();
    return MP2VG_OK;
}

extern "C" int mp2vg_batch_validate(const mp2vg_config_t* cfg, int32_t nslots, const mp2vg_picture_t* pics,
                                    int32_t npics, const mp2vg_mb_t* mbs, uint64_t nmbs, const uint32_t* coefs,
                                    uint64_t ncoefs, int32_t* nlaunches, int32_t* launch_of_pic,
                                    int32_t* launch_mode, int32_t max_launches) {
    if (!cfg || nslots <= 0 || !pics || npics <= 0 || !mbs || (!coefs && ncoefs)) return MP2VG_E_INVALID;
    if (mp2vg_frame_geometry(cfg, nullptr, nullptr, nullptr, nullptr) != MP2VG_OK) return MP2VG_E_INVALID;
    mp2vg_ctx_t shell;
    init_shell(shell, cfg, nslots);
    std::vector<SliceDesc> slices;
    std::vector<Launch> lb;
    const int rc = plan_batch(&shell, pics, npics, mbs, nmbs, coefs, ncoefs, slices, lb);
    if (rc != MP2VG_OK) return rc;
    if (nlaunches) *nlaunches = (int32_t)lb.size();
    for (size_t i = 0; i < lb.size(); i++) {
        if (launch_mode && (int32_t)i < max_launches) launch_mode[i] = lb[i].mcm;
        for (uint32_t k = lb[i].begin; launch_of_pic && k < lb[i].end; k++) launch_of_pic[slices[k].pic] = (int32_t)i;
    }
    return MP2VG_OK;
}

extern "C" int mp2vg_batch_upload(mp2vg_ctx_t* c, const mp2vg_picture_t* pics, int32_t npics,
                                  const mp2vg_mb_t* mbs, uint64_t nmbs, const uint32_t* coefs,
                                  uint64_t ncoefs) {
    return batch_upload(c, pics, npics, mbs, nmbs, coefs, ncoefs, false, false);
}

namespace mp2vg {
int batch_upload_pinned(mp2vg_ctx_t* c, const mp2vg_picture_t* pics, int32_t npics, const mp2vg_mb_t* mbs,
                        uint64_t nmbs, const uint32_t* coefs, uint64_t ncoefs) {
    return batch_upload(c, pics, npics, mbs, nmbs, coefs, ncoefs, true, true, true);
}
int ctx_next_bank(const mp2vg_ctx_t* c) { return (c->cur + 1) & 1; }
int ctx_wait_upload(mp2vg_ctx_t* c, int bank) {
    HIPCHK(hipEventSynchronize(c->bank[bank].uploaded));
    return MP2VG_OK;
}
hipStream_t ctx_stream(mp2vg_ctx_t* c) { return c->stream; }
void ctx_set_launch_timing(mp2vg_ctx_t* c, bool on) { c->launch_timing = on; }
}

static int batch_decode(mp2vg_ctx_t* c);

struct PoolSet {
    std::vector<uint8_t*> chunks;
    std::vector<size_t> bytes;
    std::vector<uint64_t> vmm, fptr, tptr;
};

static void pool_set_free(PoolSet& p) {
    for (size_t i = 0; i < p.chunks.size(); i++) pool_block_free(p.chunks[i], p.bytes[i], p.vmm[i]);
    p = PoolSet();
}

static void free_held_pools(mp2vg_ctx_t* c) {
    for (PoolSet* p : c->place_held) {
        pool_set_free(*p);
        delete p;
    }
    c->place_held.clear();
}

static PoolSet pool_take(mp2vg_ctx_t* c) {
    PoolSet p;
    p.chunks.swap(c->chunks);
    p.bytes.swap(c->chunk_bytes);
    p.vmm.swap(c->chunk_vmm);
    p.fptr.swap(c->fptr);
    p.tptr.swap(c->tptr);
    return p;
}

static hipError_t pool_install(mp2vg_ctx_t* c, PoolSet& p) {
    c->chunks.swap(p.chunks);
    c->chunk_bytes.swap(p.bytes);
    c->chunk_vmm.swap(p.vmm);
    c->fptr.swap(p.fptr);
    c->tptr.swap(p.tptr);
    p = PoolSet();
    hipError_t e = hipMemcpyAsync(c->d_tab, c->fptr.data(), sizeof(uint64_t) * c->nslots, hipMemcpyHostToDevice, c->stream);
    if (e == hipSuccess)
        e = hipMemcpyAsync(c->d_tab + c->nslots, c->tptr.data(), sizeof(uint64_t) * c->nslots, hipMemcpyHostToDevice,
                           c->stream);
    if (e == hipSuccess) e = hipStreamSynchronize(c->stream);
    return e;
}

static hipError_t pool_clone(mp2vg_ctx_t* c, const PoolSet& src, PoolSet& dst) {
    for (size_t i = 0; i < src.chunks.size(); i++) {
        uint8_t* q = nullptr;
        size_t got = 0;
        uint64_t h = 0;
        hipError_t e = pool_block_alloc(c->cfg.device, src.bytes[i], &q, &got, &h);
        if (e != hipSuccess) {
            pool_set_free(dst);
            return e;
        }
        dst.chunks.push_back(q);
        dst.bytes.push_back(got);
        dst.vmm.push_back(h);
        if ((e = hipMemcpyAsync(q, src.chunks[i], src.bytes[i], hipMemcpyDeviceToDevice, c->stream)) != hipSuccess) {
            pool_set_free(dst);
            return e;
        }
    }
    std::vector<std::pair<uintptr_t, size_t>> order(src.chunks.size());
    for (size_t i = 0; i < order.size(); i++) order[i] = {(uintptr_t)src.chunks[i], i};
    std::sort(order.begin(), order.end());
    auto rebase = [&](uint64_t ptr) -> uint64_t {
        auto it = std::upper_bound(order.begin(), order.end(), std::make_pair((uintptr_t)ptr, (size_t)-1));
        const size_t i = std::prev(it)->second;
        return (uint64_t)(uintptr_t)dst.chunks[i] + (ptr - (uint64_t)(uintptr_t)src.chunks[i]);
    };
    for (uint64_t f : src.fptr) dst.fptr.push_back(rebase(f));
    for (uint64_t t : src.tptr) dst.tptr.push_back(rebase(t));
    return hipStreamSynchronize(c->stream);
}

static int env_int(const char* name, int dflt) {
    const char* e = getenv(name);
    return e && *e ? atoi(e) : dflt;
}

static int calibrate_placement(mp2vg_ctx_t* c) {
    if (c->placed) return 1;
    const int k = std::max(1, std::min(6, env_int("MP2VG_PLACE_CANDIDATES", 3)));
    size_t pool = 0;
    for (size_t b : c->chunk_bytes) pool += b;
    if (k < 2 || c->chunks.empty() || pool < ((size_t)std::max(0, env_int("MP2VG_PLACE_MIN_MB", 4096)) << 20)) return 1;
    if (c->nstreams == 1 && !env_int("MP2VG_PLACE_ONE_STREAM", 1)) return 1;
    const Bank& bk = c->bank[c->cur];
    std::vector<uint8_t> written(c->nslots, 0);
    for (const auto& w : bk.tiles.writes)
        if (w.first >= 0 && w.first < c->nslots) written[w.first] = 1;
    for (const auto& r : bk.tiles.ext_reads)
        if (r.first >= 0 && r.first < c->nslots && written[r.first]) return 1;
    c->placed = true;
    size_t free_b = 0, total_b = 0;
    if (hipMemGetInfo(&free_b, &total_b) != hipSuccess) return 1;
    HIPCHK(hipStreamSynchronize(c->stream));
    std::vector<PoolSet> cand;
    cand.push_back(pool_take(c));
    const size_t reserve = std::max(total_b / 8, (size_t)8 << 30);
    for (int i = 1; i < k && free_b >= (size_t)i * pool + reserve; i++) {
        PoolSet p;
        if (pool_clone(c, cand[0], p) != hipSuccess) {
            (void)hipGetLastError();
            break;
        }
        cand.push_back(std::move(p));
    }
    const size_t n = cand.size();
    std::vector<float> ms(2 * n, 0.f);
    int rc = MP2VG_OK;
    auto run = [&](size_t i, float* t) -> int {
        if (pool_install(c, cand[i]) != hipSuccess) {
            cand[i] = pool_take(c);
            return (int)MP2VG_E_HIP;
        }
        c->last_foot.clear();
        int r = batch_decode(c);
        if (r == MP2VG_OK && t) r = mp2vg_batch_times(c, 0, t, nullptr, 0, nullptr);
        cand[i] = pool_take(c);
        return r;
    };
    const std::vector<uint8_t> tiles0 = c->tiles_ok;
    for (int w = 0; w < 2 && rc == MP2VG_OK; w++) rc = run(0, nullptr);
    for (int r = 0; r < 2 && rc == MP2VG_OK; r++)
        for (size_t i = 0; i < n && rc == MP2VG_OK; i++) {
            if (r == 0 && i > 0) c->tiles_ok = tiles0;
            rc = run(i, &ms[r * n + i]);
        }
    size_t best = 0;
    if (rc == MP2VG_OK)
        for (size_t i = 1; i < n; i++)
            if (std::min(ms[i], ms[n + i]) < std::min(ms[best], ms[n + best])) best = i;
    size_t free_now = 0, total_now = 0;
    const bool room = hipMemGetInfo(&free_now, &total_now) == hipSuccess && free_now >= total_now / 8;
    const int hold_env = env_int("MP2VG_PLACE_HOLD", -1);
    const bool hold = hold_env < 0 ? room : hold_env != 0;
    for (size_t i = 0; i < n; i++)
        if (i != best && rc == MP2VG_OK) {
            if (hold)
                c->place_held.push_back(new PoolSet(std::move(cand[i])));
            else
                pool_set_free(cand[i]);
        }
    if (rc != MP2VG_OK) {
        for (size_t i = 1; i < n; i++) pool_set_free(cand[i]);
        best = 0;
    }
    HIPCHK(pool_install(c, cand[best]));
    c->place_ms = ms;
    c->place_kept = rc == MP2VG_OK ? (int)best : -1;
    if (getenv("MP2VG_TRACE")) {
        fprintf(stderr, "[mp2vg] placement: %zu candidate pools (others %s), batch ms (two rounds)", n,
                hold ? "held" : "freed");
        for (float m : ms) fprintf(stderr, " %.3f", m);
        fprintf(stderr, ", kept %zu\n", best);
    }
    return rc;
}

extern "C" int mp2vg_batch_decode(mp2vg_ctx_t* c) {
    if (!c) return MP2VG_E_INVALID;
    if (!c->batch_ready) {
        set_error("no batch uploaded");
        return MP2VG_E_STATE;
    }
    HIPCHK(hipSetDevice(c->cfg.device));
    const int rc = calibrate_placement(c);
    return rc == 1 ? batch_decode(c) : rc;
}

static int batch_decode(mp2vg_ctx_t* c) {
    Bank& b = c->bank[c->cur];
    const std::vector<Launch>& launches = b.launches;
    int nl = (int)launches.size();
    mp2vg_ctx::BatchEv& H = c->hist[c->seq % mp2vg_ctx::kHist];
    for (auto& e : H.b)
        if (!e) HIPCHK(hipEventCreate(&e));
    while (c->launch_timing && (int)H.l.size() < 2 * nl) {
        hipEvent_t e;
        HIPCHK(hipEventCreate(&e));
        H.l.push_back(e);
    }

    KArgs a;
    memset(&a, 0, sizeof a);
    a.pics = b.d_pics;
    a.mbs = b.d_mbs;
    a.coefs = b.d_coefs;
    a.slices = b.d_slices;
    a.sink = c->d_sink + kSinkOff;
    a.ftab = c->d_tab;
    a.ttab = c->d_tab + c->nslots;
    a.slot_bytes = c->g.slot_bytes;
    for (int i = 0; i < 3; i++) {
        a.plane_off[i] = c->g.plane_off[i];
        a.stride[i] = c->g.stride[i];
        a.ph[i] = c->g.ph[i];
    }
    int nsets = 1;
    for (const Launch& L : launches) nsets = std::max(nsets, L.set + 1);
    while ((int)c->sstreams.size() < nsets) {
        hipStream_t st;
        hipEvent_t e;
        HIPCHK(hipStreamCreateWithFlags(&st, hipStreamNonBlocking));
        HIPCHK(hipEventCreateWithFlags(&e, hipEventDisableTiming));
        c->sstreams.push_back(st);
        c->sev.push_back(e);
        c->swaited.push_back(c->export_synced);
    }
    auto stream_of = [&](int set) { return c->sstreams[set]; };
// ... 563 lines not shown
```

Baseline: 388,300.

## Recode coefficient words into a pre-scaled block-position format before dequant

Coefficient words are converted, during host validation or by a new GPU recode kernel for resident batches, into an internal format. The new word carries the block position instead of the scan index and a pre-multiplied signed level (2*mag or 2*mag+1, with sign) plus DC/first-1s flags. The dequant inner loop then drops the scan-table LDS lookup and the intra/inter branching, using a single mad24 and bit-field selects. The cost is an extra host pass (or extra kernel) per batch, a pinned staging buffer, and a new overlap check on coefficient rows. Downloaded records are converted back to the public format on the host.

```diff
diff --git a/include/mp2vg.h b/include/mp2vg.h
--- a/include/mp2vg.h
+++ b/include/mp2vg.h
@@ -245,6 +245,10 @@
                                   uint64_t ncoefs);
 int  mp2vg_last_parse_times(mp2vg_ctx_t* ctx, float ms[3]);
 
+int  mp2vg_coef_recode_model(const uint32_t* words, uint64_t n, int32_t intra, int32_t alternate_scan,
+                             const uint8_t* W, int32_t qs, uint32_t* internal, uint32_t* back, int16_t* value,
+                             uint8_t* raster);
+
 enum {
     MP2VG_VLC_MBA = 0, MP2VG_VLC_MBTYPE_I = 1, MP2VG_VLC_MBTYPE_P = 2, MP2VG_VLC_MBTYPE_B = 3,
     MP2VG_VLC_CBP = 4, MP2VG_VLC_MOTION = 5, MP2VG_VLC_DC_LUMA = 6, MP2VG_VLC_DC_CHROMA = 7,
diff --git a/tiny_mp2v_dec_amd/_lib.py b/tiny_mp2v_dec_amd/_lib.py
--- a/tiny_mp2v_dec_amd/_lib.py
+++ b/tiny_mp2v_dec_amd/_lib.py
@@ -148,7 +148,7 @@
     "mp2vg_scan_es", "mp2vg_scan_counts", "mp2vg_scan_pictures", "mp2vg_scan_display_order",
     "mp2vg_scan_gop_index", "mp2vg_scan_shards", "mp2vg_scan_stream_headers", "mp2vg_scan_free",
     "mp2vg_scan_parse_host", "mp2vg_batch_upload_es", "mp2vg_batch_record_counts",
-    "mp2vg_batch_download_records", "mp2vg_last_parse_times",
+    "mp2vg_batch_download_records", "mp2vg_last_parse_times", "mp2vg_coef_recode_model",
 ]
 
 _lib = None
@@ -239,6 +239,7 @@
         "mp2vg_batch_record_counts": ([VP, P(U64), P(U64)], ctypes.c_int),
         "mp2vg_batch_download_records": ([VP, VP, U64, VP, U64], ctypes.c_int),
         "mp2vg_last_parse_times": ([VP, P(ctypes.c_float)], ctypes.c_int),
+        "mp2vg_coef_recode_model": ([VP, U64, I32, I32, VP, I32, VP, VP, VP, VP], ctypes.c_int),
     }
     for name, (args, res) in sig.items():
         fn = getattr(L, name)
diff --git a/tiny_mp2v_dec_amd/csrc/coef_word.h b/tiny_mp2v_dec_amd/csrc/coef_word.h
--- /dev/null
+++ b/tiny_mp2v_dec_amd/csrc/coef_word.h
@@ -0,0 +1,69 @@
+#pragma once
+#include <stdint.h>
+
+#include "../../include/mp2vg.h"
+
+#if defined(__HIPCC__) || defined(__CUDACC__)
+#define MP2VG_CW_HD __host__ __device__
+#else
+#define MP2VG_CW_HD
+#endif
+
+namespace mp2vg {
+
+constexpr uint32_t kCwAsIs = 1u << 0;
+constexpr uint32_t kCwOnes = 1u << 13;
+constexpr int kCwPosShift = 1;
+constexpr int kCwKbShift = 7;
+constexpr int kCwMulShift = 14;
+
+MP2VG_CW_HD static inline uint32_t cw_block_pos(uint32_t r) { return (r >> 4) * 16u + (r & 7u) * 2u + ((r >> 3) & 1u); }
+
+MP2VG_CW_HD static inline uint32_t cw_recode(uint32_t w, bool intra, const uint8_t* raster_of_scan) {
+    const int level = (int16_t)(w & 0xffffu);
+    const int mag = level < 0 ? -level : level;
+    int m;
+    uint32_t fl = 0;
+    if (w & MP2VG_COEF_DC) {
+        m = level;
+        fl = kCwAsIs;
+    } else if (w & MP2VG_COEF_FIRST1S) {
+        m = level < 0 ? -3 : 3;
+        fl = kCwOnes;
+    } else {
+        const int a = intra ? 2 * mag : 2 * mag + 1;
+        m = level < 0 ? -a : a;
+    }
+    const uint32_t pos = cw_block_pos(raster_of_scan[(w >> 16) & 63u]);
+    return fl | (pos << kCwPosShift) | (((w >> 22) & 63u) << kCwKbShift) | ((uint32_t)m << kCwMulShift);
+}
+
+static inline uint32_t cw_public(uint32_t iw, bool intra, const uint8_t* scan_of_pos, uint32_t mbx) {
+    const int m = (int32_t)iw >> kCwMulShift;
+    const int am = m < 0 ? -m : m;
+    const uint32_t block = (iw >> kCwKbShift) & 15u;
+    uint32_t fl = MP2VG_COEF_MBX(mbx);
+    int level;
+    if (iw & kCwAsIs) {
+        level = m;
+        fl |= MP2VG_COEF_DC;
+    } else if (iw & kCwOnes) {
+        level = m < 0 ? -1 : 1;
+        fl |= MP2VG_COEF_FIRST1S;
+    } else {
+        const int a = intra ? am / 2 : (am - 1) / 2;
+        level = m < 0 ? -a : a;
+    }
+    return MP2VG_COEF_PACK(level, scan_of_pos[(iw >> kCwPosShift) & 63u], block, fl);
+}
+
+static inline int16_t cw_dequant_model(uint32_t iw, uint32_t wq) {
+    const int32_t m = (int32_t)iw >> kCwMulShift;
+    const int32_t p = (int32_t)((uint32_t)m * wq + (uint32_t)((m >> 31) & 31));
+    const int32_t val = p >> 5;
+    const int16_t t = (int16_t)val;
+    const int16_t v = (int16_t)(t < -2048 ? -2048 : (t > 2047 ? 2047 : t));
+    return (iw & kCwAsIs) ? (int16_t)m : ((iw & kCwOnes) ? t : v);
+}
+
+}
diff --git a/tiny_mp2v_dec_amd/csrc/recon.hip b/tiny_mp2v_dec_amd/csrc/recon.hip
--- a/tiny_mp2v_dec_amd/csrc/recon.hip
+++ b/tiny_mp2v_dec_amd/csrc/recon.hip
@@ -4,6 +4,7 @@
 #include <stdint.h>
 #include <stdlib.h>
 
+#include "coef_word.h"
 #include "recon_kernel.h"
 
 namespace mp2vg {
@@ -687,8 +688,8 @@
     static constexpr int NH = lds_sets(CF, C8);
     uint8_t W[4 * NH][64];
     static constexpr bool WB = C8;
-    uint8_t scan[64 * NH];
-    uint8_t Wb[WB && CF != 1 ? Fmt<CF>::NB : 0][64];
+    uint8_t gap[64 * NH];
+    uint8_t Wb[WB && CF != 1 ? Fmt<CF>::NB : 0][128];
     uint32_t kbtab[WB ? 64 : 0];
     __device__ static int bofs(int slot, int idx) { return slot * BLK + (X64 ? (idx ^ ((slot & 7) << 3)) : idx); }
 };
@@ -771,73 +772,64 @@
     return (slot & 0xff) | (pick8(S.qs8, k) << 8) | (wsel << 16) | (intra << 18) | ((uint32_t)coded << 19);
 }
 
-__device__ __forceinline__ int mul24i_asm(int a, int b) {
+__device__ __forceinline__ int mad24i_asm(int a, int b, int c) {
     int r;
-    asm("v_mul_i32_i24 %0, %1, %2" : "=v"(r) : "v"(a), "v"(b));
+    asm("v_mad_i32_i24 %0, %1, %2, %3" : "=v"(r) : "v"(a), "v"(b), "v"(c));
     return r;
 }
+__device__ __forceinline__ int cw_scale(int m, uint32_t wq) { return mad24i_asm(m, (int)wq, (m >> 31) & 31) >> 5; }
 
 template <class LT, bool INTRA_ONLY = false, int NB = 6>
 __device__ __forceinline__ void dequant_word(LT& L, int wave, uint32_t w, uint32_t qs8, bool live = true, int h = 0,
                                              int buf = 0) {
+    static_assert(kCwAsIs == 1u && kCwPosShift == 1 && kCwKbShift == 7 && kCwOnes == 1u << 13, "the masks below");
+    const int m = (int)w >> kCwMulShift;
+    const uint32_t dcm = (uint32_t)__builtin_amdgcn_sbfe((int)w, 0, 1);
     if constexpr (INTRA_ONLY) {
-        const uint32_t k = (w >> 26) & 3u, b = (w >> 22) & 15u;
+        const uint32_t k = (w >> (kCwKbShift + 4)) & 3u, b = (w >> kCwKbShift) & 15u;
         const int slot = (int)(k * NB + b);
-        const int i = (w >> 16) & 63;
-        const int level = (short)(w & 0xffff);
-        const int Wi = NB == 6 ? L.W[4 * h][i]
-                               : (LT::WB ? ((const uint8_t*)L.Wb)[(w >> 16) & 0x3ffu] : L.W[4 * h + (b < 6 ? 0 : 2)][i]);
+        const uint32_t pos2 = w & 0x7eu, pos = pos2 >> 1;
+        int Wi;
+        if constexpr (LT::WB)
+            Wi = NB == 6 ? ((const uint8_t*)L.W)[pos2] : ((const uint8_t*)L.Wb)[w & 0x7feu];
+        else
+            Wi = L.W[4 * h + (NB == 6 || b < 6 ? 0 : 2)][pos];
         uint32_t kb = 0;
-        if constexpr (LT::WB && MP2VG_I_KBTAB) kb = L.kbtab[(w >> 22) & 63u];
+        if constexpr (LT::WB && MP2VG_I_KBTAB) kb = L.kbtab[(w >> kCwKbShift) & 63u];
         const uint32_t qsk = (LT::WB && MP2VG_I_KBTAB) ? __builtin_amdgcn_ubfe(qs8, kb, 8) : pick8(qs8, (int)k);
         const uint32_t wq = __umul24((uint32_t)Wi, qsk);
-        const int p = mul24i_asm(level, (int)wq);
-        const int val = (p + ((p >> 31) & 15)) >> 4;
+        const int val = cw_scale(m, wq);
         const int v = min(max((int)(short)val, -2048), 2047);
-        short o;
-        if constexpr (LT::WB) {
-            const uint32_t dcm = (uint32_t)__builtin_amdgcn_sbfe((int)w, 30, 1);
-            uint32_t ov;
-            asm("v_bfi_b32 %0, %1, %2, %3" : "=v"(ov) : "v"(dcm), "v"(w), "v"((uint32_t)v));
-            o = (short)ov;
-        } else {
-            o = (w & MP2VG_COEF_DC) ? (short)level : (short)v;
-        }
+        uint32_t ov;
+        asm("v_bfi_b32 %0, %1, %2, %3" : "=v"(ov) : "v"(dcm), "v"((uint32_t)m), "v"((uint32_t)v));
+        const short o = (short)ov;
         if constexpr (LT::WB) {
             const uint32_t a = MP2VG_I_KBTAB
-                                   ? (uint32_t)(uintptr_t)(lds_short2_t*)L.blk[wave] + ((kb >> 8) ^ (uint32_t)L.scan[64 * h + i])
+                                   ? (uint32_t)(uintptr_t)(lds_short2_t*)L.blk[wave] + ((kb >> 8) ^ pos2)
                                    : (uint32_t)(uintptr_t)(lds_short2_t*)L.blk[wave] + ((uint32_t)slot << 7) +
-                                         ((((uint32_t)slot << 4) & 0x70u) ^ (uint32_t)L.scan[64 * h + i]);
+                                         ((((uint32_t)slot << 4) & 0x70u) ^ pos2);
             const uint32_t d = (uint32_t)(uintptr_t)(lds_short2_t*)L.res[wave];
             *(__attribute__((address_space(3))) short*)(uintptr_t)(live ? a : d) = o;
         } else {
-            short* const dst = live ? &((short*)L.blk[wave])[LT::bofs(slot, L.scan[64 * h + i])] : (short*)L.res[wave];
+            short* const dst = live ? &((short*)L.blk[wave])[LT::bofs(slot, (int)pos)] : (short*)L.res[wave];
             *dst = o;
         }
         return;
     }
-    const uint32_t e = L.dq[wave][(w >> 22) & 63u];
+    const uint32_t pos = (w >> kCwPosShift) & 63u;
+    const uint32_t e = L.dq[wave][(w >> kCwKbShift) & 63u];
     const int slot = (int)(e & 0xff);
-    const bool intra = INTRA_ONLY || ((e >> 18) & 1);
     const int qs = (int)((e >> 8) & 0xff);
-    const int i = (w >> 16) & 63;
-    const int level = (short)(w & 0xffff);
-    const bool dc = w & MP2VG_COEF_DC;
-    const bool s1 = !INTRA_ONLY && (w & MP2VG_COEF_FIRST1S);
-    const int Wi = L.W[4 * h + ((e >> 16) & 3)][i];
-    const int sign = level < 0 ? -1 : 0;
-    const int mag = level < 0 ? -level : level;
+    const int Wi = L.W[4 * h + ((e >> 16) & 3)][pos];
     const uint32_t wq = __umul24((uint32_t)Wi, (uint32_t)qs);
-    int val = intra ? (int)mul24_asm((uint32_t)mag, wq) >> 4 : (int)mul24_asm((uint32_t)(2 * mag + 1), wq) >> 5;
-    val = (val ^ sign) - sign;
+    const int val = cw_scale(m, wq);
     const int t = (short)val;
-    short v = (short)min(max(t, -2048), 2047);
-    if (!INTRA_ONLY) {
-        const short t1 = (short)((int)(3u * wq) >> 5);
-        v = s1 ? (short)((t1 ^ sign) - sign) : v;
-    }
-    v = dc ? (short)level : v;
-    ((short*)L.blk[wave * LT::NBUF + buf])[LT::bofs(slot, L.scan[64 * h + i])] = v;
+    const int v = min(max(t, -2048), 2047);
+    const uint32_t s1m = (uint32_t)__builtin_amdgcn_sbfe((int)w, 13, 1);
+    uint32_t ov;
+    asm("v_bfi_b32 %0, %1, %2, %3" : "=v"(ov) : "v"(s1m), "v"((uint32_t)t), "v"((uint32_t)v));
+    asm("v_bfi_b32 %0, %1, %2, %3" : "=v"(ov) : "v"(dcm), "v"((uint32_t)m), "v"(ov));
+    ((short*)L.blk[wave * LT::NBUF + buf])[LT::bofs(slot, (int)pos)] = (short)ov;
 }
 
 template <int NW>
@@ -1177,10 +1169,13 @@
     const int alt = pic->alternate_scan & 1;
 
     if ((uint32_t)wave % wps == 0 && (two || tid < 64)) {
-        ((uint32_t*)L.W)[64 * half + lane] = ((const uint32_t*)pic->W)[lane];
-        const int r = c_scan_raster[alt][lane];
-        const int pos = (r >> 4) * 16 + (r & 7) * 2 + ((r >> 3) & 1);
-        L.scan[64 * half + lane] = (uint8_t)(LT::WB ? 2 * pos : pos);
+        const uint32_t pos = cw_block_pos(c_scan_raster[alt][lane]);
+        if constexpr (LT::WB) {
+            if constexpr (CF == 1) ((uint8_t*)L.W)[2 * pos] = pic->W[0][lane];
+        } else {
+#pragma unroll
+            for (int k = 0; k < 4; k++) L.W[4 * half + k][pos] = pic->W[k][lane];
+        }
         if constexpr (LT::WB && MP2VG_I_KBTAB) {
             const int k = lane >> 4, bb = lane & 15;
             const uint32_t slot = (uint32_t)(k * Fmt<CF>::NB + (bb < Fmt<CF>::NB ? bb : 0));
@@ -1188,7 +1183,7 @@
         }
         if constexpr (LT::WB && CF != 1) {
 #pragma unroll
-            for (int bb = 0; bb < Fmt<CF>::NB; bb++) L.Wb[bb][lane] = pic->W[bb < 6 ? 0 : 2][lane];
+            for (int bb = 0; bb < Fmt<CF>::NB; bb++) L.Wb[bb][2 * pos] = pic->W[bb < 6 ? 0 : 2][lane];
         }
     }
     for (int i = lane; i < LT::NBUF * LT::MAXS * LT::BLK / 2; i += 64) ((uint32_t*)L.blk[wave * LT::NBUF])[i] = 0;
@@ -1401,6 +1396,40 @@
     return hipGetLastError();
 }
 
+__global__ void __launch_bounds__(64) recode_kernel(const mp2vg_picture_t* __restrict__ pics,
+                                                    const mp2vg_mb_t* __restrict__ mbs, uint32_t* __restrict__ coefs,
+                                                    uint32_t chunks, uint64_t nmbs, uint64_t ncoefs) {
+    __shared__ uint8_t raster[64];
+    const int lane = threadIdx.x;
+    const uint32_t p = blockIdx.x / chunks, ch = blockIdx.x % chunks;
+    const mp2vg_picture_t* pic = pics + p;
+    raster[lane] = c_scan_raster[pic->alternate_scan & 1][lane];
+    __syncthreads();
+    const uint32_t nm = (uint32_t)pic->mb_width * pic->mb_height, k = ch * 64u + (uint32_t)lane;
+    uint32_t off = 0, n = 0, intra = 0;
+    if (k < nm && (uint64_t)pic->mb_first + k < nmbs) {
+        const mp2vg_mb_t* m = mbs + pic->mb_first + k;
+        off = m->coef_off;
+        n = (uint64_t)off + m->ncoef <= ncoefs ? m->ncoef : 0u;
+        intra = m->flags & MP2VG_MB_INTRA;
+    }
+    for (int j = 0; j < 64; j++) {
+        const uint32_t o = (uint32_t)__shfl((int)off, j), c = (uint32_t)__shfl((int)n, j);
+        const bool in = __shfl((int)intra, j) != 0;
+        for (uint32_t i = (uint32_t)lane; i < c; i += 64u) coefs[o + i] = cw_recode(coefs[o + i], in, raster);
+    }
+}
+
+static hipError_t recode_launch(const mp2vg_picture_t* d_pics, const mp2vg_mb_t* d_mbs, uint32_t* d_coefs, int32_t npics,
+                                uint32_t mbs_per_pic, uint64_t nmbs, uint64_t ncoefs, hipStream_t stream) {
+    if (npics <= 0 || !mbs_per_pic || !ncoefs) return hipSuccess;
+    const uint32_t chunks = (mbs_per_pic + 63u) / 64u;
+    hipLaunchKernelGGL(recode_kernel, dim3((uint32_t)npics * chunks), dim3(64), 0, stream, d_pics, d_mbs, d_coefs, chunks,
+                       nmbs, ncoefs);
+    return hipGetLastError();
+}
+__attribute__((used)) static const bool recode_registered =(launch_recode = &recode_launch, true);
+
 __global__ void __launch_bounds__(256) clock_probe_kernel(unsigned long long* __restrict__ out, int iters) {
     uint32_t a = threadIdx.x, b = a * 2654435761u, c2 = a ^ 0x9e3779b9u, d = ~a;
     uint64_t t0, r0, t1, r1;
diff --git a/tiny_mp2v_dec_amd/csrc/recon_kernel.h b/tiny_mp2v_dec_amd/csrc/recon_kernel.h
--- a/tiny_mp2v_dec_amd/csrc/recon_kernel.h
+++ b/tiny_mp2v_dec_amd/csrc/recon_kernel.h
@@ -54,4 +54,9 @@
 };
 hipError_t launch_frame_copy(const FrameCopy& fc, int n, uint64_t bytes, hipStream_t stream);
 
+typedef hipError_t (*RecodeLauncher)(const mp2vg_picture_t* d_pics, const mp2vg_mb_t* d_mbs, uint32_t* d_coefs,
+                                     int32_t npics, uint32_t mbs_per_pic, uint64_t nmbs, uint64_t ncoefs,
+                                     hipStream_t stream);
+extern RecodeLauncher launch_recode;
+
 }
diff --git a/tiny_mp2v_dec_amd/csrc/runtime.cpp b/tiny_mp2v_dec_amd/csrc/runtime.cpp
--- a/tiny_mp2v_dec_amd/csrc/runtime.cpp
+++ b/tiny_mp2v_dec_amd/csrc/runtime.cpp
@@ -9,6 +9,7 @@
 #include <atomic>
 #include <thread>
 
+#include "coef_word.h"
 #include "export_kernel.h"
 #include "hipchk.h"
 #include "parse_kernel.h"
@@ -27,6 +28,7 @@
 hipError_t launch_digest(const uint64_t* ftab, const int32_t* d_slots, int n,
                          const uint64_t off[3], const int32_t stride[3], const int32_t w[3],
                          const int32_t h[3], unsigned long long* d_out, hipStream_t stream);
+RecodeLauncher launch_recode = nullptr;
 }
 
 using namespace mp2vg;
@@ -142,6 +144,8 @@
     std::vector<PoolSet*> place_held;
 
     void* h_stage = nullptr;
+    uint32_t* h_icoefs = nullptr;
+    size_t cap_icoefs = 0;
     int32_t* d_dslots = nullptr;
     unsigned long long* d_digest = nullptr;
     size_t cap_digest = 0;
@@ -292,6 +296,7 @@
     }
     if (c->export_ev) hipEventDestroy(c->export_ev);
     if (c->h_stage) hipHostFree(c->h_stage);
+    if (c->h_icoefs) hipHostFree(c->h_icoefs);
     for (auto st : c->sstreams) hipStreamSynchronize(st);
     for (auto e : c->sev) hipEventDestroy(e);
     for (auto e : c->lev) hipEventDestroy(e);
@@ -471,7 +476,7 @@
 static int plan_batch(mp2vg_ctx_t* c, const mp2vg_picture_t* pics, int32_t npics, const mp2vg_mb_t* mbs,
                       uint64_t nmbs, const uint32_t* coefs, uint64_t ncoefs, std::vector<SliceDesc>& slices,
                       std::vector<Launch>& launches, std::vector<std::vector<int32_t>>* foot = nullptr,
-                      bool trusted = false, TilePlan* tplan = nullptr) {
+                      bool trusted = false, TilePlan* tplan = nullptr, uint32_t* recoded = nullptr) {
     const int mbw = c->cfg.width / 16, mbh = c->cfg.height / 16;
     const int nb = c->g.nblocks;
     if (ncoefs + kCoefPad >= (1ull << 30)) {
@@ -513,6 +518,7 @@
         const uint64_t nm = (uint64_t)mbw * mbh;
         if ((uint64_t)P.mb_first + nm > nmbs) return "picture MB range outside the batch";
         bool uses[2] = {false, false};
+        const uint8_t* const raster = kScanRaster[P.alternate_scan & 1];
         for (uint64_t k = 0; k < nm; k++) {
             const mp2vg_mb_t& m = mbs[P.mb_first + k];
             if (m.x != k % mbw || m.y != k / mbw) return "MB records not in raster order";
@@ -521,10 +527,21 @@
             const uint32_t first = MP2VG_COEF_DC | MP2VG_COEF_FIRST1S;
             uint32_t bad = 0, blocks = 0, pos0 = 0;
             const uint32_t* w = coefs + m.coef_off;
-            for (uint32_t j = 0; j < m.ncoef; j++) {
-                bad |= (w[j] & 0x9C000000u) ^ tag;
-                blocks |= 1u << MP2VG_COEF_BLOCK(w[j]);
-                pos0 |= (w[j] & first) ? MP2VG_COEF_POS(w[j]) : 0u;
+            if (recoded) {
+                uint32_t* const iw = recoded + m.coef_off;
+                const bool intra = m.flags & MP2VG_MB_INTRA;
+                for (uint32_t j = 0; j < m.ncoef; j++) {
+                    bad |= (w[j] & 0x9C000000u) ^ tag;
+                    blocks |= 1u << MP2VG_COEF_BLOCK(w[j]);
+                    pos0 |= (w[j] & first) ? MP2VG_COEF_POS(w[j]) : 0u;
+                    iw[j] = cw_recode(w[j], intra, raster);
+                }
+            } else {
+                for (uint32_t j = 0; j < m.ncoef; j++) {
+                    bad |= (w[j] & 0x9C000000u) ^ tag;
+                    blocks |= 1u << MP2VG_COEF_BLOCK(w[j]);
+                    pos0 |= (w[j] & first) ? MP2VG_COEF_POS(w[j]) : 0u;
+                }
             }
             if (bad) return "coefficient word bits 26-28 are not the MB column mod 8 (or bit 31 is set)";
             if (pos0) return "DC or '1s' coefficient word with a nonzero scan position";
@@ -557,6 +574,23 @@
         return nullptr;
     };
     parallel_for(npics, 16, [&](int p) { err[p] = validate(p); });
+    if (!trusted && std::none_of(err.begin(), err.end(), [](const char* e) { return e != nullptr; })) {
+        std::vector<std::pair<uint64_t, uint64_t>> rows;
+        rows.reserve((size_t)npics * mbh);
+        for (int p = 0; p < npics; p++)
+            for (int y = 0; y < mbh; y++) {
+                const mp2vg_mb_t& a = mbs[pics[p].mb_first + (uint64_t)y * mbw];
+                const mp2vg_mb_t& z = mbs[pics[p].mb_first + (uint64_t)y * mbw + mbw - 1];
+                const uint64_t lo = a.coef_off, hi = (uint64_t)z.coef_off + z.ncoef;
+                if (hi > lo) rows.push_back({lo, hi});
+            }
+        std::sort(rows.begin(), rows.end());
+        for (size_t i = 1; i < rows.size(); i++)
+            if (rows[i].first < rows[i - 1].second) {
+                set_error("macroblock rows share coefficient words");
+                return MP2VG_E_INVALID;
+            }
+    }
     return plan_from_uses(c, pics, npics, uses_of.data(), err.data(), slices, launches, foot, tplan);
 }
 
@@ -777,6 +811,16 @@
     return MP2VG_OK;
 }
 
+static int recode_resident(mp2vg_ctx_t* c, Bank& b, int32_t npics, uint64_t nmbs, uint64_t ncoefs) {
+    if (!launch_recode) {
+        set_error("the reconstruct kernels are not linked into this build");
+        return MP2VG_E_STATE;
+    }
+    HIPCHK(launch_recode(b.d_pics, b.d_mbs, b.d_coefs, npics, (uint32_t)(c->cfg.width / 16) * (c->cfg.height / 16), nmbs,
+                         ncoefs, c->ustream));
+    return MP2VG_OK;
+}
+
 static int batch_upload(mp2vg_ctx_t* c, const mp2vg_picture_t* pics, int32_t npics, const mp2vg_mb_t* mbs,
                         uint64_t nmbs, const uint32_t* coefs, uint64_t ncoefs, bool pinned, bool async,
                         bool trusted = false) {
@@ -788,7 +832,19 @@
     std::vector<std::vector<int32_t>> foot;
     TilePlan tplan;
     double tp = now_ms();
-    int rc = plan_batch(c, pics, npics, mbs, nmbs, coefs, ncoefs, slices, lb, &foot, trusted, &tplan);
+    uint32_t* recoded = nullptr;
+    if (!trusted && ncoefs) {
+        if (ncoefs > c->cap_icoefs) {
+            const size_t cap = std::max({(size_t)ncoefs, c->cap_icoefs * 3 / 2, (size_t)1 << 18});
+            if (c->h_icoefs) HIPCHK(hipHostFree(c->h_icoefs));
+            c->h_icoefs = nullptr;
+            c->cap_icoefs = 0;
+            HIPCHK(hipHostMalloc((void**)&c->h_icoefs, cap * sizeof(uint32_t), hipHostMallocDefault));
+            c->cap_icoefs = cap;
+        }
+        recoded = c->h_icoefs;
+    }
+    int rc = plan_batch(c, pics, npics, mbs, nmbs, coefs, ncoefs, slices, lb, &foot, trusted, &tplan, recoded);
     if (rc != MP2VG_OK) return rc;
     tp = trace_phase("upload: plan", tp);
     const int k = (c->cur + 1) & 1;
@@ -833,7 +889,12 @@
         if (ps_bytes && (rc = upload(c, b.d_post, ps.data(), ps_bytes, false)) != MP2VG_OK) return rc;
     }
     if ((rc = upload(c, b.d_mbs, mbs, sizeof(mp2vg_mb_t) * nmbs, pinned)) != MP2VG_OK) return rc;
-    if (ncoefs && (rc = upload(c, b.d_coefs, coefs, sizeof(uint32_t) * ncoefs, pinned)) != MP2VG_OK) return rc;
+    if (recoded) {
+        if ((rc = upload(c, b.d_coefs, recoded, sizeof(uint32_t) * ncoefs, true)) != MP2VG_OK) return rc;
+    } else if (ncoefs) {
+        if ((rc = upload(c, b.d_coefs, coefs, sizeof(uint32_t) * ncoefs, pinned)) != MP2VG_OK) return rc;
+        if ((rc = recode_resident(c, b, npics, nmbs, ncoefs)) != MP2VG_OK) return rc;
+    }
     HIPCHK(hipEventRecord(b.uploaded, c->ustream));
     if (!async) HIPCHK(hipStreamSynchronize(c->ustream));
     trace_phase("upload: copy", tp);
@@ -912,6 +973,7 @@
     if ((rc = upload(c, b.d_pics, pics, sizeof(mp2vg_picture_t) * npics, false)) != MP2VG_OK) return rc;
     if ((rc = upload(c, b.d_slices, slices.data(), sizeof(SliceDesc) * slices.size(), false)) != MP2VG_OK) return rc;
     if (!ps.empty() && (rc = upload(c, b.d_post, ps.data(), sizeof(int32_t) * ps.size(), false)) != MP2VG_OK) return rc;
+    if ((rc = recode_resident(c, b, npics, nmbs, ncoefs)) != MP2VG_OK) return rc;
     HIPCHK(hipEventRecord(b.uploaded, c->ustream));
     HIPCHK(hipStreamSynchronize(c->ustream));
     b.launches = std::move(lb);
@@ -955,7 +1017,45 @@
     HIPCHK(hipSetDevice(c->cfg.device));
     HIPCHK(hipEventSynchronize(b.uploaded));
     HIPCHK(hipMemcpy(mbs, b.d_mbs, sizeof(mp2vg_mb_t) * nmbs, hipMemcpyDeviceToHost));
-    if (ncoefs) HIPCHK(hipMemcpy(coefs, b.d_coefs, sizeof(uint32_t) * ncoefs, hipMemcpyDeviceToHost));
+    if (!ncoefs) return MP2VG_OK;
+    HIPCHK(hipMemcpy(coefs, b.d_coefs, sizeof(uint32_t) * ncoefs, hipMemcpyDeviceToHost));
+    std::vector<mp2vg_picture_t> pics((size_t)b.npics);
+    HIPCHK(hipMemcpy(pics.data(), b.d_pics, sizeof(mp2vg_picture_t) * pics.size(), hipMemcpyDeviceToHost));
+    uint8_t scan_of_pos[2][64];
+    for (int alt = 0; alt < 2; alt++)
+        for (int i = 0; i < 64; i++) scan_of_pos[alt][cw_block_pos(kScanRaster[alt][i])] = (uint8_t)i;
+    const uint64_t nm = (uint64_t)(c->cfg.width / 16) * (c->cfg.height / 16);
+    for (const mp2vg_picture_t& P : pics)
+        for (uint64_t k = 0; k < nm && P.mb_first + k < nmbs; k++) {
+            const mp2vg_mb_t& m = mbs[P.mb_first + k];
+            if ((uint64_t)m.coef_off + m.ncoef > ncoefs) continue;
+            uint32_t* const w = coefs + m.coef_off;
+            for (uint32_t j = 0; j < m.ncoef; j++)
+                w[j] = cw_public(w[j], m.flags & MP2VG_MB_INTRA, scan_of_pos[P.alternate_scan & 1], m.x);
+        }
+    return MP2VG_OK;
+}
+
+extern "C" int mp2vg_coef_recode_model(const uint32_t* words, uint64_t n, int32_t intra, int32_t alternate_scan,
+                                       const uint8_t* W, int32_t qs, uint32_t* internal, uint32_t* back, int16_t* value,
+                                       uint8_t* raster) {
+    if ((!words && n) || ((value || raster) && !W)) return MP2VG_E_INVALID;
+    const uint8_t* const scan = kScanRaster[alternate_scan & 1];
+    uint8_t scan_of_pos[64], raster_of_pos[64], Wp[64] = {};
+    for (int i = 0; i < 64; i++) {
+        const uint32_t pos = cw_block_pos(scan[i]);
+        scan_of_pos[pos] = (uint8_t)i;
+        raster_of_pos[pos] = scan[i];
+        if (W) Wp[pos] = W[i];
+    }
+    for (uint64_t j = 0; j < n; j++) {
+        const uint32_t iw = cw_recode(words[j], intra != 0, scan);
+        const uint32_t pos = (iw >> kCwPosShift) & 63u;
+        if (internal) internal[j] = iw;
+        if (back) back[j] = cw_public(iw, intra != 0, scan_of_pos, (words[j] >> 26) & 7u);
+        if (value) value[j] = cw_dequant_model(iw, (uint32_t)Wp[pos] * (uint32_t)qs);
+        if (raster) raster[j] = raster_of_pos[pos];
+    }
     return MP2VG_OK;
 }
 
```

Measured after the change: 391,200 (median of 6 runs). About the same (+0.8%).
